# Blaizzy/mlx-audio-swift

Measured on NVIDIA H100. Metric: orpheus3b_tts_rtfx_batch8, higher is better.
Workload: dtype bf16

## Files before the change

### include/b200audio_internal.h

```cpp
#ifndef B200AUDIO_INTERNAL_H
#define B200AUDIO_INTERNAL_H

#include "b200audio.h"

#ifdef __cplusplus
extern "C" {
#endif

int32_t b2a_tts_create_random(int32_t device, const b2a_llama_config* cfg, float std, uint64_t seed,
                              b2a_snac* snac, b2a_tts** out);
int32_t b2a_stt_create_random(int32_t device, const b2a_whisper_config* cfg, float std, uint64_t seed, b2a_stt** out);
int32_t b2a_tts_set_bench_flags(b2a_tts* h, int32_t mask_eos, int32_t wrap_codes);
int32_t b2a_stt_set_bench_flags(b2a_stt* h, int32_t mask_eot);
int32_t b2a_tts_time_steps(b2a_tts* h, int32_t batch, int32_t ctx, int32_t iters, float* ms_per_step);
int32_t b2a_qwen3_talker_create_random(int32_t device, const b2a_qwen3_talker_config* cfg, float std, uint64_t seed, b2a_qwen3_talker** out);
int32_t b2a_qwen3_talker_set_bench_flags(b2a_qwen3_talker* h, int32_t mask_eos);

int32_t b2a_tts_debug_trace(b2a_tts* h, int32_t enable, int32_t batch, float* out);
int32_t b2a_debug_step_smem(int32_t gqa, int32_t* out);

int32_t b2a_speech_tokenizer_debug_layout(const float* w, int32_t out, int32_t k, int32_t in, int32_t stride, float* layout_out,
                                          int64_t capacity, int32_t* rows, int32_t* taps, int32_t* kpad);
int32_t b2a_speech_tokenizer_debug_stage(b2a_speech_tokenizer* h, int32_t stage, float* out, int64_t capacity, int64_t* n);
int32_t b2a_qwen3_sample_test(const float* logits, int32_t batch, int32_t vocab, float temperature, float top_p, int32_t top_k,
                              float min_p, float repetition_penalty, int32_t eos, int32_t suppress_lo, int32_t suppress_hi,
                              uint32_t* seen, int32_t track, uint64_t seed, int32_t step, int32_t* tokens_out, float* filtered_out);
int32_t b2a_implicit_conv_test(const float* w, int32_t M, int32_t taps, int32_t Cin, const float* x, int32_t B, int32_t Ttot, int32_t T,
                               int32_t dil, int32_t shift0, int32_t up, const float* bias, const float* gamma, int32_t gelu, int32_t add,
                               int32_t bias_twice_t0, const float* sa, const float* sb, int32_t Hout, int32_t fp16, float* xo, float* hl_out);
int32_t b2a_tc_gemm_epilogue_test(const void* W, const void* X, void* out, int32_t M, int32_t N, int32_t K, int32_t bn, int32_t epi,
                                  int32_t split, int32_t hilo, int32_t ctas, const float* bias, int32_t act, int32_t tile_rows,
                                  int32_t lo_rows, const float* rstd_ss, int32_t rstd_parts, float rstd_eps, int32_t stages, void* stream);
int32_t b2a_tc_gemm_test(const void* W, const void* X, void* out, int32_t M, int32_t N, int32_t K, int32_t bn, int32_t epi,
                         int32_t split, int32_t hilo, int32_t ctas, void* stream);
int32_t b2a_tc_gemm_splitk_test(const void* W, const void* X, float* h, const float* gain, void* xn, float* ss, int32_t M, int32_t N,
                                int32_t K, int32_t cluster, int32_t stages, void* stream);
int32_t b2a_mha_tc_test(const float* qkv, void* out, int32_t B, int32_t T, int32_t nh, void* stream);
int32_t b2a_conv_gemm_test(const float* w, int32_t M, int32_t K, const void* X, int32_t N, int32_t epi, const float* bias,
                           const float* alpha, const float* gamma, int32_t gelu, float* x, int32_t ldx, void* hl, int32_t ldh,
                           int32_t dual, int32_t T, int32_t Cout, int32_t stride, int32_t pad, int32_t Tin, const float* noise,
                           uint64_t seed, int32_t ctas, void* stream);
int32_t b2a_snac_unit_test(int32_t mode, int32_t C, int32_t dil, const float* x, float* y, int32_t B, int32_t T, const float* dw_w,
                           const float* dw_b, const float* a_in, const float* a_mid, const float* pw_w, const float* pw_bias,
                           const float* noise, uint64_t seed, void* hl, const float* a_next, int32_t ctas, void* stream);
int32_t b2a_snac_convt_test(const float* x, float* y, const float* alpha, const float* bias, const float* w, int32_t B, int32_t Tin,
                            int32_t stride, int32_t cout, int32_t ctas, void* stream);
int32_t b2a_snac_encode_latent_test(b2a_snac* h, const float* wave, int32_t batch, int64_t n_samples, float* z);

#ifdef __cplusplus
}
#endif
#endif
```

### mlx-audio-swift_b200/_ffi.py

```python
from __future__ import annotations

import ctypes as C
from pathlib import Path

import numpy as np

LIB_PATH = Path(__file__).resolve().parent / "lib" / "libb200audio.so"

(OK, ERR_MODEL_NOT_INITIALIZED, ERR_GENERATION_FAILED, ERR_INVALID_INPUT, ERR_AUDIO_DECODING_FAILED,
 ERR_AUDIO_ENCODING_FAILED, ERR_CANCELLED, ERR_CUDA) = range(8)
DTYPE_F32, DTYPE_BF16, DTYPE_I32 = 0, 1, 2


class AudioGenerationError(RuntimeError):
    CASES = {1: "modelNotInitialized", 2: "generationFailed", 3: "invalidInput", 4: "audioDecodingFailed",
             5: "audioEncodingFailed", 6: "cancelled", 7: "cudaError"}

    def __init__(self, code: int, message: str):
        super().__init__(f"{self.CASES.get(code, code)}: {message}")
        self.code, self.case, self.message = code, self.CASES.get(code, str(code)), message


class Tensor(C.Structure):
    _fields_ = [("name", C.c_char_p), ("dtype", C.c_int32), ("ndim", C.c_int32), ("shape", C.c_int64 * 4),
# ... 32 lines not shown
    _fields_ = [(n, C.c_int32) for n in ("input_channels", "dim", "intermediate_dim", "num_layers", "n_fft", "hop_length",
                                          "input_kernel_size", "dw_kernel_size", "adanorm_num_embeddings")]


class EncodecConfig(C.Structure):
    _fields_ = ([(n, C.c_int32) for n in ("audio_channels", "num_filters", "kernel_size", "num_residual_layers",
                                           "dilation_growth_rate", "codebook_size", "codebook_dim", "hidden_size",
                                           "num_lstm_layers", "residual_kernel_size", "use_causal_conv", "pad_mode_reflect",
                                           "norm_type", "last_kernel_size", "compress", "n_upsampling_ratios")]
                + [("upsampling_ratios", C.c_int32 * 8), ("sampling_rate", C.c_int32), ("use_conv_shortcut", C.c_int32),
                   ("trim_right_ratio", C.c_float), ("chunk_length_s", C.c_float), ("overlap", C.c_float)])


class SpeechTokenizerConfig(C.Structure):
    _fields_ = ([(n, C.c_int32) for n in ("codebook_size", "codebook_dim", "latent_dim", "decoder_dim", "hidden_size",
                                           "intermediate_size", "head_dim", "num_attention_heads", "num_key_value_heads",
                                           "num_hidden_layers", "num_quantizers", "num_semantic_quantizers")]
                + [("rms_norm_eps", C.c_float), ("rope_theta", C.c_float), ("attention_bias", C.c_int32),
                   ("num_upsample_rates", C.c_int32), ("upsample_rates", C.c_int32 * 8),
                   ("num_upsampling_ratios", C.c_int32), ("upsampling_ratios", C.c_int32 * 8),
                   ("max_batch", C.c_int32), ("max_cache_frames", C.c_int32)])


class Qwen3TalkerConfig(C.Structure):
    _fields_ = ([(n, C.c_int32) for n in ("vocab_size", "hidden_size", "intermediate_size", "num_hidden_layers", "num_attention_heads",
                                           "num_key_value_heads", "head_dim")]
                + [("rms_norm_eps", C.c_float), ("rope_theta", C.c_float)]
                + [(n, C.c_int32) for n in ("num_code_groups", "text_hidden_size", "text_vocab_size", "codec_eos_token_id", "cp_vocab_size",
                                             "cp_hidden_size", "cp_intermediate_size", "cp_num_hidden_layers", "cp_num_attention_heads",
                                             "cp_num_key_value_heads", "cp_head_dim")]
                + [("cp_rms_norm_eps", C.c_float), ("cp_rope_theta", C.c_float), ("max_batch", C.c_int32), ("max_context", C.c_int32)])


class Qwen3GenParams(C.Structure):
    _fields_ = [("max_tokens", C.c_int32), ("temperature", C.c_float), ("top_p", C.c_float), ("top_k", C.c_int32), ("min_p", C.c_float),
                ("repetition_penalty", C.c_float), ("seed", C.c_uint64)]


class WhisperConfig(C.Structure):
    _fields_ = [(n, C.c_int32) for n in ("vocab_size", "num_mel_bins", "d_model", "encoder_layers", "encoder_attention_heads",
                                          "encoder_ffn_dim", "max_source_positions", "decoder_layers", "decoder_attention_heads",
                                          "decoder_ffn_dim", "max_target_positions", "max_batch")]


class SttParams(C.Structure):
    _fields_ = [("max_tokens", C.c_int32), ("temperature", C.c_float), ("prompt_ids", C.c_void_p), ("n_prompt", C.c_int32),
                ("begin_suppress", C.c_void_p), ("n_begin_suppress", C.c_int32), ("suppress", C.c_void_p),
                ("n_suppress", C.c_int32), ("timestamp_begin", C.c_int32), ("eot", C.c_int32), ("seed", C.c_uint64)]


class SttInfo(C.Structure):
    _fields_ = [("prompt_tokens", C.c_int32), ("generation_tokens", C.c_int32), ("decode_steps", C.c_int32),
                ("encode_time", C.c_double), ("decode_time", C.c_double), ("total_time", C.c_double)]


TOKEN_CB = C.CFUNCTYPE(None, C.c_void_p, C.c_int32, C.c_int32, C.c_int32)
AUDIO_CB = C.CFUNCTYPE(None, C.c_void_p, C.c_int32, C.POINTER(C.c_float), C.c_int64, C.c_int32)
STT_DECODE_CB = C.CFUNCTYPE(C.c_int32, C.c_void_p, C.POINTER(C.c_float), C.c_int64, C.POINTER(C.c_int32), C.c_int32, C.POINTER(C.c_int32),
                            C.c_int32, C.POINTER(C.c_int32))


class SttStreamConfig(C.Structure):
    _fields_ = [("decode_interval_s", C.c_double), ("window_s", C.c_double), ("window_overlap_s", C.c_double), ("delay_ms", C.c_int32),
                ("min_agreement_passes", C.c_int32), ("max_tokens_per_pass", C.c_int32), ("sample_rate", C.c_int32)]


class SttStreamUpdate(C.Structure):
    _fields_ = [("kind", C.c_int32), ("promoted", C.c_int32), ("completed_windows", C.c_int32), ("n_confirmed", C.c_int32),
                ("n_provisional", C.c_int32), ("total_audio_s", C.c_double), ("pass_encode_time", C.c_double), ("pass_decode_time", C.c_double)]


_P = C.c_void_p
SIGNATURES = {
    "b2a_last_error": (C.c_char_p, []),
    "b2a_version": (C.c_char_p, []),
    "b2a_device_count": (C.c_int32, []),
    "b2a_launch_count": (C.c_int64, []),
    "b2a_hanning_window": (C.c_int32, [C.c_int32, C.c_int32, _P]),
    "b2a_hamming_window": (C.c_int32, [C.c_int32, C.c_int32, _P]),
    "b2a_power_to_db": (C.c_int32, [_P, C.c_int64, C.c_float, C.c_float, _P]),
    "b2a_mel_filters": (C.c_int32, [C.c_int32, C.c_int32, C.c_int32, C.c_float, C.c_float, C.c_int32, C.c_int32, _P]),
    "b2a_mel_create": (C.c_int32, [C.c_int32, C.c_int32, C.c_int32, C.c_int32, C.c_int32, C.POINTER(_P)]),
    "b2a_mel_max_frames": (C.c_int64, [_P, C.c_int64]),
    "b2a_mel_process": (C.c_int32, [_P, _P, C.c_int64, _P, C.c_int64, C.POINTER(C.c_int64)]),
    "b2a_mel_flush": (C.c_int32, [_P, _P, C.c_int64, C.POINTER(C.c_int64)]),
    "b2a_mel_reset": (C.c_int32, [_P]),
    "b2a_mel_total_frames": (C.c_int64, [_P]),
    "b2a_mel_destroy": (None, [_P]),
    "b2a_logmel_create": (C.c_int32, [C.c_int32, C.c_int32, C.c_int32, C.c_int32, C.c_int32, C.c_int32, C.POINTER(_P)]),
    "b2a_logmel_frames": (C.c_int64, [_P, C.c_int64]),
    "b2a_logmel_compute": (C.c_int32, [_P, _P, C.c_int32, C.c_int64, _P]),
    "b2a_logmel_compute_dev": (C.c_int32, [_P, _P, C.c_int32, C.c_int64, _P, _P]),
    "b2a_logmel_destroy": (None, [_P]),
    "b2a_snac_create": (C.c_int32, [C.c_int32, C.POINTER(SnacConfig), C.POINTER(Tensor), C.c_int32, C.POINTER(_P)]),
    "b2a_snac_hop_length": (C.c_int64, [_P]),
    "b2a_snac_decode": (C.c_int32, [_P, C.POINTER(_P), C.c_int32, C.c_int64, C.POINTER(_P), C.c_int32, C.c_uint64, _P]),
    "b2a_snac_decode_dev": (C.c_int32, [_P, C.POINTER(_P), C.c_int32, C.c_int64, C.POINTER(_P), C.c_int32, C.c_uint64, _P, _P]),
    "b2a_snac_quantize": (C.c_int32, [_P, _P, C.c_int32, C.c_int64, C.POINTER(_P), _P]),
    "b2a_snac_encoded_length": (C.c_int64, [_P, C.c_int64]),
    "b2a_snac_encode": (C.c_int32, [_P, _P, C.c_int32, C.c_int64, C.POINTER(_P)]),
    "b2a_snac_encode_dev": (C.c_int32, [_P, _P, C.c_int32, C.c_int64, C.POINTER(_P), _P]),
    "b2a_snac_encode_latent_test": (C.c_int32, [_P, _P, C.c_int32, C.c_int64, _P]),
    "b2a_snac_destroy": (None, [_P]),
    "b2a_tts_create": (C.c_int32, [C.c_int32, C.POINTER(LlamaConfig), C.POINTER(Tensor), C.c_int32, _P, C.POINTER(_P)]),
    "b2a_tts_debug_trace": (C.c_int32, [_P, C.c_int32, C.c_int32, _P]),
    "b2a_debug_step_smem": (C.c_int32, [C.c_int32, C.POINTER(C.c_int32)]),
    "b2a_tts_create_random": (C.c_int32, [C.c_int32, C.POINTER(LlamaConfig), C.c_float, C.c_uint64, _P, C.POINTER(_P)]),
    "b2a_tts_stream": (C.c_void_p, [_P]),
    "b2a_tts_set_bench_flags": (C.c_int32, [_P, C.c_int32, C.c_int32]),
    "b2a_stt_set_bench_flags": (C.c_int32, [_P, C.c_int32]),
    "b2a_tts_time_steps": (C.c_int32, [_P, C.c_int32, C.c_int32, C.c_int32, C.POINTER(C.c_float)]),
    "b2a_snac_stream": (C.c_void_p, [_P]),
    "b2a_tts_prepare_input_ids": (C.c_int32, [C.POINTER(_P), _P, C.c_int32, _P, C.POINTER(C.c_int32)]),
    "b2a_tts_prepare_input_ids_ref": (C.c_int32, [C.POINTER(_P), _P, C.c_int32, _P, C.c_int32, _P, C.c_int32, _P, C.POINTER(C.c_int32)]),
    "b2a_tts_forward_logits": (C.c_int32, [_P, _P, C.c_int32, C.c_int32, C.c_int32, _P]),
    "b2a_tts_generate": (C.c_int32, [_P, _P, C.c_int32, C.c_int32, C.POINTER(GenParams), _P, _P, _P, C.c_int64, _P,
                                     C.POINTER(GenInfo), TOKEN_CB, _P]),
    "b2a_tts_generate_stream": (C.c_int32, [_P, _P, C.c_int32, C.c_int32, C.POINTER(GenParams), C.c_int32, C.c_int32, _P, _P,
                                            C.POINTER(GenInfo), TOKEN_CB, AUDIO_CB, _P]),
    "b2a_tts_generate_dev": (C.c_int32, [_P, _P, C.c_int32, C.c_int32, C.POINTER(GenParams), _P, C.c_int64, _P,
                                         C.POINTER(GenInfo)]),
    "b2a_tts_cancel": (C.c_int32, [_P]),
    "b2a_tts_parse_output": (C.c_int32, [_P, C.c_int32, C.c_int32, _P, _P]),
    "b2a_tts_deinterleave": (C.c_int32, [_P, C.c_int32, _P, _P, _P, C.POINTER(C.c_int32)]),
    "b2a_tts_interleave": (C.c_int32, [_P, _P, _P, C.c_int32, _P]),
    "b2a_tts_destroy": (None, [_P]),
    "b2a_vocos_create": (C.c_int32, [C.c_int32, C.POINTER(VocosConfig), C.POINTER(Tensor), C.c_int32, C.POINTER(_P)]),
    "b2a_vocos_output_length": (C.c_int64, [_P, C.c_int32]),
    "b2a_vocos_stream": (C.c_void_p, [_P]),
    "b2a_vocos_decode": (C.c_int32, [_P, _P, C.c_int32, C.c_int32, _P]),
    "b2a_vocos_decode_dev": (C.c_int32, [_P, _P, C.c_int32, C.c_int32, _P, _P]),
    "b2a_vocos_decode_cond": (C.c_int32, [_P, _P, _P, C.c_int32, C.c_int32, _P]),
    "b2a_vocos_destroy": (None, [_P]),
    "b2a_speech_tokenizer_create": (C.c_int32, [C.c_int32, C.POINTER(SpeechTokenizerConfig), C.POINTER(Tensor), C.c_int32, C.POINTER(_P)]),
    "b2a_speech_tokenizer_total_upsample": (C.c_int32, [_P]),
    "b2a_speech_tokenizer_stream": (C.c_void_p, [_P]),
    "b2a_speech_tokenizer_reset": (C.c_int32, [_P]),
    "b2a_speech_tokenizer_streaming_step": (C.c_int32, [_P, _P, C.c_int32, C.c_int32, C.c_int32, _P]),
    "b2a_speech_tokenizer_streaming_step_dev": (C.c_int32, [_P, _P, C.c_int32, C.c_int32, C.c_int32, _P, _P]),
    "b2a_speech_tokenizer_streaming_decode": (C.c_int32, [_P, _P, C.c_int32, C.c_int32, C.c_int32, C.c_int32, _P]),
    "b2a_speech_tokenizer_chunked_decode": (C.c_int32, [_P, _P, C.c_int32, C.c_int32, C.c_int32, C.c_int32, C.c_int32, _P]),
    "b2a_speech_tokenizer_destroy": (None, [_P]),
    "b2a_weights_sanitize_speech_tokenizer": (C.c_int32, [_P]),
    "b2a_speech_tokenizer_config_from_json": (C.c_int32, [C.c_char_p, C.c_int32, C.c_int32, C.POINTER(SpeechTokenizerConfig), C.POINTER(C.c_int32)]),
    "b2a_speech_tokenizer_create_from_directory": (C.c_int32, [C.c_char_p, C.c_int32, C.c_int32, C.c_int32, C.POINTER(_P), C.POINTER(C.c_int32)]),
    "b2a_qwen3_sample_test": (C.c_int32, [_P, C.c_int32, C.c_int32, C.c_float, C.c_float, C.c_int32, C.c_float, C.c_float, C.c_int32, C.c_int32,
                                         C.c_int32, _P, C.c_int32, C.c_uint64, C.c_int32, _P, _P]),
    "b2a_implicit_conv_test": (C.c_int32, [_P, C.c_int32, C.c_int32, C.c_int32, _P, C.c_int32, C.c_int32, C.c_int32, C.c_int32, C.c_int32, C.c_int32,
                                          _P, _P, C.c_int32, C.c_int32, C.c_int32, _P, _P, C.c_int32, C.c_int32, _P, _P]),
    "b2a_tc_gemm_test": (C.c_int32, [_P, _P, _P] + [C.c_int32] * 8 + [_P]),
    "b2a_tc_gemm_epilogue_test": (C.c_int32, [_P, _P, _P] + [C.c_int32] * 8 + [_P, C.c_int32, C.c_int32, C.c_int32, _P, C.c_int32,
                                                                             C.c_float, C.c_int32, _P]),
    "b2a_tc_gemm_splitk_test": (C.c_int32, [_P, _P, _P, _P, _P, _P] + [C.c_int32] * 5 + [_P]),
    "b2a_mha_tc_test": (C.c_int32, [_P, _P, C.c_int32, C.c_int32, C.c_int32, _P]),
    "b2a_conv_gemm_test": (C.c_int32, [_P, C.c_int32, C.c_int32, _P, C.c_int32, C.c_int32, _P, _P, _P, C.c_int32, _P, C.c_int32, _P,
                                       C.c_int32] + [C.c_int32] * 6 + [_P, C.c_uint64, C.c_int32, _P]),
    "b2a_snac_unit_test": (C.c_int32, [C.c_int32] * 3 + [_P, _P, C.c_int32, C.c_int32] + [_P] * 6 + [_P, C.c_uint64, _P, _P, C.c_int32, _P]),
    "b2a_snac_convt_test": (C.c_int32, [_P] * 5 + [C.c_int32] * 5 + [_P]),
    "b2a_speech_tokenizer_debug_stage": (C.c_int32, [_P, C.c_int32, _P, C.c_int64, _P]),
    "b2a_speech_tokenizer_debug_layout": (C.c_int32, [_P, C.c_int32, C.c_int32, C.c_int32, C.c_int32, _P, C.c_int64, _P, _P, _P]),
    "b2a_encodec_create": (C.c_int32, [C.c_int32, C.POINTER(EncodecConfig), C.POINTER(Tensor), C.c_int32, C.POINTER(_P)]),
    "b2a_encodec_output_length": (C.c_int64, [_P, C.c_int32, C.c_int32]),
    "b2a_encodec_num_codebooks": (C.c_int32, [_P]),
    "b2a_encodec_stream": (C.c_void_p, [_P]),
    "b2a_encodec_decode": (C.c_int32, [_P, _P, C.c_int32, C.c_int32, C.c_int32, C.c_int32, _P, _P]),
    "b2a_encodec_decode_dev": (C.c_int32, [_P, _P, C.c_int32, C.c_int32, C.c_int32, C.c_int32, _P, _P, _P]),
    "b2a_encodec_destroy": (None, [_P]),
    "b2a_weights_load": (C.c_int32, [C.c_char_p, C.POINTER(_P)]),
    "b2a_weights_count": (C.c_int32, [_P]),
    "b2a_weights_get": (C.c_int32, [_P, C.c_int32, C.POINTER(Tensor)]),
    "b2a_weights_sanitize_whisper": (C.c_int32, [_P, C.POINTER(C.c_int32)]),
    "b2a_weights_sanitize_llama": (C.c_int32, [_P, C.c_int32, C.c_int32, C.c_int32]),
    "b2a_weights_sanitize_llama_config": (C.c_int32, [_P, C.c_char_p]),
    "b2a_weights_dequantize": (C.c_int32, [_P, C.c_int32, C.c_int32]),
    "b2a_weights_free": (None, [_P]),
    "b2a_tts_config_from_json": (C.c_int32, [C.c_char_p, C.c_int32, C.c_int32, C.POINTER(LlamaConfig), C.POINTER(C.c_int32), C.POINTER(C.c_int32)]),
    "b2a_tts_create_from_directory": (C.c_int32, [C.c_char_p, C.c_int32, C.c_int32, C.c_int32, _P, C.POINTER(_P)]),
    "b2a_stt_create": (C.c_int32, [C.c_int32, C.POINTER(WhisperConfig), C.POINTER(Tensor), C.c_int32, C.POINTER(_P)]),
    "b2a_stt_create_random": (C.c_int32, [C.c_int32, C.POINTER(WhisperConfig), C.c_float, C.c_uint64, C.POINTER(_P)]),
    "b2a_stt_stream": (C.c_void_p, [_P]),
    "b2a_stt_encode": (C.c_int32, [_P, _P, C.c_int32, C.c_int64, _P]),
    "b2a_stt_decoder_logits": (C.c_int32, [_P, _P, C.c_int32, C.c_int32, _P]),
    "b2a_stt_transcribe": (C.c_int32, [_P, _P, C.c_int32, C.c_int64, C.POINTER(SttParams), _P, _P, C.POINTER(SttInfo)]),
    "b2a_stt_transcribe_dev": (C.c_int32, [_P, _P, C.c_int32, C.c_int64, C.POINTER(SttParams), _P, _P, C.POINTER(SttInfo)]),
    "b2a_stt_transcribe_long": (C.c_int32, [_P, _P, C.c_int64, C.POINTER(SttParams), C.c_int32, _P, _P, _P, C.POINTER(C.c_int32), C.POINTER(SttInfo)]),
    "b2a_qwen3_talker_create": (C.c_int32, [C.c_int32, C.POINTER(Qwen3TalkerConfig), C.POINTER(Tensor), C.c_int32, C.POINTER(_P)]),
    "b2a_qwen3_talker_create_random": (C.c_int32, [C.c_int32, C.POINTER(Qwen3TalkerConfig), C.c_float, C.c_uint64, C.POINTER(_P)]),
    "b2a_qwen3_talker_set_bench_flags": (C.c_int32, [_P, C.c_int32]),
    "b2a_qwen3_talker_stream": (C.c_void_p, [_P]),
    "b2a_qwen3_talker_embed_text": (C.c_int32, [_P, _P, C.c_int32, _P]),
    "b2a_qwen3_talker_embed_codec": (C.c_int32, [_P, _P, C.c_int32, _P]),
    "b2a_qwen3_talker_forward": (C.c_int32, [_P, _P, C.c_int32, C.c_int32, _P, _P]),
    "b2a_qwen3_talker_generate": (C.c_int32, [_P, _P, C.c_int32, C.c_int32, _P, _P, C.c_int32, _P, C.POINTER(Qwen3GenParams), _P, _P,
                                              C.POINTER(GenInfo), _P, _P]),
    "b2a_qwen3_talker_config_from_json": (C.c_int32, [C.c_char_p, C.c_int32, C.c_int32, C.POINTER(Qwen3TalkerConfig)]),
    "b2a_weights_sanitize_qwen3_talker": (C.c_int32, [_P, C.c_char_p]),
    "b2a_qwen3_talker_create_from_directory": (C.c_int32, [C.c_char_p, C.c_int32, C.c_int32, C.c_int32, C.POINTER(_P)]),
    "b2a_qwen3_talker_cancel": (C.c_int32, [_P]),
    "b2a_qwen3_talker_destroy": (None, [_P]),
    "b2a_stt_session_create": (C.c_int32, [_P, C.POINTER(SttParams), C.POINTER(SttStreamConfig), C.POINTER(_P)]),
    "b2a_stt_session_create_with_decoder": (C.c_int32, [STT_DECODE_CB, _P, C.POINTER(SttStreamConfig), C.POINTER(_P)]),
    "b2a_stt_session_feed": (C.c_int32, [_P, _P, C.c_int64, C.c_double, C.POINTER(SttStreamUpdate)]),
    "b2a_stt_session_stop": (C.c_int32, [_P, C.c_double, C.POINTER(SttStreamUpdate)]),
    "b2a_stt_session_tokens": (C.c_int32, [_P, C.c_int32, C.c_int32, _P, C.c_int32, C.POINTER(C.c_int32)]),
    "b2a_stt_session_destroy": (None, [_P]),
    "b2a_stt_cancel": (C.c_int32, [_P]),
    "b2a_stt_destroy": (None, [_P]),
}

_lib = None


def lib() -> C.CDLL:
    global _lib
    if _lib is None:
        if not LIB_PATH.exists():
            raise ImportError(f"{LIB_PATH} is missing: build it with `python -c 'import __graft_entry__ as g; g.build()'`"
                              " -- there is no CPU fallback")
        _lib = C.CDLL(str(LIB_PATH))
        for name, (res, args) in SIGNATURES.items():
            fn = getattr(_lib, name)
            fn.restype, fn.argtypes = res, args
    return _lib


def check(status: int) -> None:
    if status != OK:
        raise AudioGenerationError(status, lib().b2a_last_error().decode("utf-8", "replace"))


def ptr(a) -> C.c_void_p:
    if a is None:
        return C.c_void_p(None)
    if isinstance(a, np.ndarray):
        assert a.flags["C_CONTIGUOUS"]
        return C.c_void_p(a.ctypes.data)
    return C.c_void_p(a.data_ptr())


def make_tensor_table(weights: dict):
    import torch
    arr = (Tensor * len(weights))()
    keep = []
    for i, (name, w) in enumerate(weights.items()):
        if isinstance(w, torch.Tensor):
            w = w.detach().contiguous().cpu()
            if w.dtype == torch.bfloat16:
                dt = DTYPE_BF16
            elif w.dtype == torch.float32:
                dt = DTYPE_F32
            else:
                w = w.to(torch.float32); dt = DTYPE_F32
            data, shape = w.data_ptr(), tuple(w.shape)
        else:
            w = np.ascontiguousarray(w)
            if w.dtype == np.int32:
                dt = DTYPE_I32
            else:
                if w.dtype != np.float32:
                    w = w.astype(np.float32)
                dt = DTYPE_F32
            data, shape = w.ctypes.data, w.shape
        assert len(shape) <= 4, name
        nm = name.encode()
        keep += [w, nm]
        arr[i].name, arr[i].dtype, arr[i].ndim, arr[i].data = nm, dt, len(shape), data
        for j, s in enumerate(shape):
            arr[i].shape[j] = s
    return arr, keep
```

### mlx-audio-swift_b200/csrc/llama.cu

```cuda
#include "common.cuh"
#include <cooperative_groups.h>
#include "tc_gemm.cuh"
#include "qwen3_sampler.cuh"

#include <algorithm>
#include <cstdlib>
#include <cstring>
#include <chrono>
#include <cmath>

namespace b2a {

typedef __nv_bfloat16 bf16;

constexpr int TOK_START_OF_HUMAN = 128259, TOK_END_OF_HUMAN = 128260, TOK_END_OF_TEXT = 128009;
constexpr int TOK_START_OF_SPEECH = 128257, TOK_END_OF_SPEECH = 128258, TOK_PAD = 128263;
constexpr int TOK_AUDIO_OFFSET = 128266;
constexpr int TOK_AUDIO_START = 128261, TOK_AUDIO_END = 128262;

__device__ __forceinline__ float bf16_round(float x) { return __bfloat162float(__float2bfloat16_rn(x)); }
__device__ __forceinline__ float bf_lo(unsigned u) { return __uint_as_float(u << 16); }
__device__ __forceinline__ float bf_hi(unsigned u) { return __uint_as_float(u & 0xffff0000u); }

__device__ __forceinline__ uint4 ldg_stream(const uint4* p) {
// ... 14 lines not shown
        x[(long long)b * H + i] = __bfloat162float(embed[(long long)tok * H + i]);
        y[(long long)b * H + i] = 0.f;
    }
}

__global__ void ext_embed_kernel(const float* __restrict__ src, float* __restrict__ x, float* __restrict__ y, int H) {
    const int b = blockIdx.x;
    pdl_trigger();
    pdl_wait();
    for (int i = threadIdx.x; i < H; i += blockDim.x) {
        x[(long long)b * H + i] = src[(long long)b * H + i];
        y[(long long)b * H + i] = 0.f;
    }
}

__global__ void finalize_norm_kernel(const float* __restrict__ x, const float* __restrict__ w, const float* __restrict__ ss, int parts,
                                     float* __restrict__ out, int H, float eps) {
    const int b = blockIdx.x;
    pdl_trigger();
    pdl_wait();
    float t = 0.f;
    for (int p = 0; p < parts; ++p) t += ss[p * 8 + b];
    const float r = rsqrtf(t / (float)H + eps);
    for (int i = threadIdx.x; i < H; i += blockDim.x) out[(long long)b * H + i] = x[(long long)b * H + i] * r * w[i];
}

constexpr int LO_ROW = 8;

constexpr int RN_THREADS = 1024, RN_MAXV = 8;
__global__ void __launch_bounds__(RN_THREADS)
add_rmsnorm_kernel(float* __restrict__ x, float* __restrict__ delta, const float* __restrict__ w,
                   bf16* __restrict__ xn, int H, float eps, float* __restrict__ trace, float* __restrict__ zero_ptr,
                   int zero_n, int half, float* __restrict__ normed = nullptr, float* __restrict__ ss_out = nullptr,
                   int ss_parts = 0) {
    __shared__ float red[RN_THREADS / 32];
    const int b = blockIdx.x, tid = threadIdx.x;
    pdl_trigger();
    pdl_wait();
    float* xr = x + (long long)b * H;
    float v[RN_MAXV];
    float ss = 0.f;
#pragma unroll
    for (int j = 0; j < RN_MAXV; ++j) {
        const int i = tid + j * RN_THREADS;
        float val = 0.f;
        if (i < H) {
            val = xr[i];
            if (delta) { val += delta[(long long)b * H + i]; xr[i] = val; delta[(long long)b * H + i] = 0.f; }
            if (trace) trace[(long long)b * H + i] = val;
        }
        v[j] = val;
        ss += val * val;
    }
    ss = warp_sum(ss);
    if ((tid & 31) == 0) red[tid >> 5] = ss;
    __syncthreads();
    float tot = 0.f;
#pragma unroll
    for (int i = 0; i < RN_THREADS / 32; ++i) tot += red[i];
    const float r = ss_out ? 1.0f : rsqrtf(tot / (float)H + eps);
    if (ss_out && tid < ss_parts) ss_out[tid * 8 + b] = tid == 0 ? tot : 0.f;
#pragma unroll
    for (int j = 0; j < RN_MAXV; ++j) {
        const int i = tid + j * RN_THREADS;
        if (i < H) {
            const float o = v[j] * r * w[i];
            tc::store_hilo(xn, H, b, i, o, half);
            if (normed) normed[(long long)b * H + i] = o;
        }
    }
    if (zero_ptr)
        for (int i = tid; i < zero_n; i += RN_THREADS) zero_ptr[(long long)b * zero_n + i] = 0.f;
}

constexpr int GV_MAX_THREADS = 256;
enum : int { GV_F32 = 0, GV_SWIGLU = 1, GV_F32_ATOMIC = 2 };

template <int NB, int ROWS, int EPI>
__global__ void __launch_bounds__(GV_MAX_THREADS)
gemv_bf16_kernel(const bf16* __restrict__ W, const bf16* __restrict__ xin, float* __restrict__ y,
                 bf16* __restrict__ act, int N, int K) {
    extern __shared__ uint4 sx[];
    pdl_trigger();
    pdl_wait();
    const int K8 = K >> 3;
    const int Kc8 = K8 / gridDim.y, kbase = blockIdx.y * Kc8;
    for (int i = threadIdx.x; i < 2 * NB * Kc8; i += blockDim.x) {
        const int r = i / Kc8, k = i - r * Kc8;
        const int grow = r < NB ? r : LO_ROW + (r - NB);
        sx[i] = reinterpret_cast<const uint4*>(xin)[(long long)grow * K8 + kbase + k];
    }
    __syncthreads();
    const int warp = threadIdx.x >> 5, lane = threadIdx.x & 31;
    const int row0 = (blockIdx.x * (blockDim.x >> 5) + warp) * ROWS;
    if (row0 >= N) return;
    const uint4* Wr[ROWS];
#pragma unroll
    for (int r = 0; r < ROWS; ++r)
        Wr[r] = reinterpret_cast<const uint4*>(W) + (long long)min(row0 + r, N - 1) * K8 + kbase;

    float acc[ROWS][2 * NB];
#pragma unroll
    for (int r = 0; r < ROWS; ++r)
#pragma unroll
        for (int b = 0; b < 2 * NB; ++b) acc[r][b] = 0.f;

    for (int k8 = lane; k8 < Kc8; k8 += 32) {
        float wf[ROWS][8];
#pragma unroll
        for (int r = 0; r < ROWS; ++r) {
            const uint4 wv = ldg_stream(Wr[r] + k8);
            wf[r][0] = bf_lo(wv.x); wf[r][1] = bf_hi(wv.x); wf[r][2] = bf_lo(wv.y); wf[r][3] = bf_hi(wv.y);
            wf[r][4] = bf_lo(wv.z); wf[r][5] = bf_hi(wv.z); wf[r][6] = bf_lo(wv.w); wf[r][7] = bf_hi(wv.w);
        }
#pragma unroll
        for (int b = 0; b < 2 * NB; ++b) {
            const uint4 xv = sx[b * Kc8 + k8];
            const float xf[8] = {bf_lo(xv.x), bf_hi(xv.x), bf_lo(xv.y), bf_hi(xv.y),
                                 bf_lo(xv.z), bf_hi(xv.z), bf_lo(xv.w), bf_hi(xv.w)};
#pragma unroll
            for (int r = 0; r < ROWS; ++r)
#pragma unroll
                for (int j = 0; j < 8; ++j) acc[r][b] = fmaf(wf[r][j], xf[j], acc[r][b]);
        }
    }
#pragma unroll
    for (int r = 0; r < ROWS; ++r)
#pragma unroll
        for (int b = 0; b < NB; ++b) acc[r][b] = warp_sum(acc[r][b] + acc[r][NB + b]);
    if (lane == 0) {
        if (EPI == GV_F32 || EPI == GV_F32_ATOMIC) {
#pragma unroll
            for (int r = 0; r < ROWS; ++r)
                if (row0 + r < N)
#pragma unroll
                    for (int b = 0; b < NB; ++b) {
                        if (EPI == GV_F32) y[(long long)b * N + row0 + r] = acc[r][b];
                        else atomicAdd(&y[(long long)b * N + row0 + r], acc[r][b]);
                    }
        } else {
#pragma unroll
            for (int r = 0; r < ROWS; r += 2)
                if (row0 + r + 1 < N)
#pragma unroll
                    for (int b = 0; b < NB; ++b) {
                        const float g = acc[r][b], u = acc[r + 1][b];
                        tc::store_hilo(act, N / 2, b, (row0 + r) / 2, g / (1.0f + __expf(-g)) * u, LO_ROW);
                    }
        }
    }
}

constexpr int HD = 128, AT_THREADS = 256, MAXG = 8, AT_CAP = 64;
constexpr int AT_SLOTS = 3;
constexpr size_t attn_smem_bytes(int G) {
    return ((size_t)AT_SLOTS * AT_CAP * HD + (size_t)G * HD + 2 * HD + (size_t)G * HD + 2 * MAXG) * sizeof(float) + 64;
}
static_assert((AT_THREADS / 32) * MAXG * HD <= AT_CAP * HD, "the warp-partial outputs must fit in one ring slot");

struct AttnArgs {
    const float* qkv;
    const int* pos;
    const float* freqs;
    float* kcache;
    float* vcache;
    bf16* out;
    int nq, nkv, max_ctx;
    float scale;
    const float* qnorm;
    const float* knorm;
    float qk_eps;
    int zero_qkv;
};

template <int G>
__global__ void __cluster_dims__(1, 1, 2) __launch_bounds__(AT_THREADS)
attn_decode_cluster_kernel(const __grid_constant__ AttnArgs a) {
    namespace cgr = cooperative_groups;
    cgr::cluster_group cluster = cgr::this_cluster();
    const int rank = (int)cluster.block_rank();
    extern __shared__ __align__(16) uint8_t at_smem[];
    float* sKV = reinterpret_cast<float*>(at_smem);
    float* wpo = sKV;
    float* sq = sKV + (size_t)AT_SLOTS * AT_CAP * HD;
    float* snew = sq + G * HD;
    float* xo = snew + 2 * HD;
    float* xml = xo + G * HD;
    uint64_t* bars = reinterpret_cast<uint64_t*>(xml + 2 * MAXG);
    __shared__ float red_m[AT_THREADS / 32][MAXG], red_l[AT_THREADS / 32][MAXG];

    const int h = blockIdx.x, b = blockIdx.y, tid = threadIdx.x;
    pdl_trigger();
    const int p = a.pos[b];
    if (!(p >= 0 && p < a.max_ctx)) { pdl_wait(); return; }
    const int nch = p / AT_CAP + 1;
    const int n_my = nch > rank ? (nch - rank + 1) / 2 : 0;
    const bool owner = ((nch - 1) & 1) == rank;
    const int qkv_ld = (a.nq + 2 * a.nkv) * HD;
    const float* row = a.qkv + (long long)b * qkv_ld;
    float* kc = a.kcache + (((long long)b * a.nkv + h) * a.max_ctx) * HD;
    float* vc = a.vcache + (((long long)b * a.nkv + h) * a.max_ctx) * HD;
    const int n_mat = 2 * n_my;
    auto issue = [&](int j) {
        const int slot = j % AT_SLOTS, c = rank + 2 * (j >> 1);
        const int n_load = (c < nch - 1) ? AT_CAP : p - c * AT_CAP;
        if (n_load > 0) {
            const uint32_t bytes = (uint32_t)n_load * HD * 4;
            tc::mbar_arrive_expect_tx(&bars[slot], bytes);
            asm volatile("cp.async.bulk.shared::cluster.global.mbarrier::complete_tx::bytes [%0], [%1], %2, [%3];"
                         ::"r"(tc::smem_u32(sKV + (size_t)slot * AT_CAP * HD)), "l"(((j & 1) ? vc : kc) + (long long)c * AT_CAP * HD), "r"(bytes),
                           "r"(tc::smem_u32(&bars[slot])) : "memory");
        } else {
            tc::mbar_arrive(&bars[slot]);
        }
    };
    if (tid == 0) {
        for (int i = 0; i < AT_SLOTS; ++i) tc::mbar_init(&bars[i], 1);
        tc::fence_barrier_init();
        asm volatile("fence.proxy.async.shared::cta;" ::: "memory");
        for (int j = 0; j < min(n_mat, AT_SLOTS); ++j) issue(j);
    }
    float sn = 0.f, cs = 1.f;
    if (tid < HD / 2) sincosf((float)p / a.freqs[tid], &sn, &cs);
    pdl_wait();
    const float* qsrc = row + (long long)h * G * HD;
    const float* ksrc = row + (a.nq + h) * HD;
    if (a.qnorm) {
        for (int vec = tid >> 5; vec < G + 1; vec += AT_THREADS / 32) {
            const float* src = vec < G ? qsrc + vec * HD : ksrc;
            const float* w = vec < G ? a.qnorm : a.knorm;
            const float4 x = reinterpret_cast<const float4*>(src)[tid & 31];
            const float ss = warp_sum(x.x * x.x + x.y * x.y + x.z * x.z + x.w * x.w);
            const float r = rsqrtf(ss * (1.0f / HD) + a.qk_eps);
            const float4 g4 = reinterpret_cast<const float4*>(w)[tid & 31];
            reinterpret_cast<float4*>(vec < G ? sq + vec * HD : snew)[tid & 31] =
                make_float4(x.x * r * g4.x, x.y * r * g4.y, x.z * r * g4.z, x.w * r * g4.w);
        }
        __syncthreads();
        qsrc = sq;
        ksrc = snew;
    }
    if (tid < HD / 2) {
        const int d = tid;
        _Pragma("unroll") for (int g = 0; g < G; ++g) {
            const float* q = qsrc + g * HD;
            const float x1 = q[d], x2 = q[d + HD / 2];
            sq[g * HD + d] = x1 * cs - x2 * sn;
            sq[g * HD + d + HD / 2] = x2 * cs + x1 * sn;
        }
        const float* k = ksrc;
        const float x1 = k[d], x2 = k[d + HD / 2];
        const float k1 = x1 * cs - x2 * sn, k2 = x2 * cs + x1 * sn;
        if (owner) { kc[(long long)p * HD + d] = k1; kc[(long long)p * HD + d + HD / 2] = k2; }
        snew[d] = k1;
        snew[d + HD / 2] = k2;
    } else if (tid >= 128) {
        const int d = tid - 128;
        const float v = row[(a.nq + a.nkv + h) * HD + d];
        if (owner) vc[(long long)p * HD + d] = v;
        snew[HD + d] = v;
    }
    __syncthreads();

    const int lane = tid & 31, warp = tid >> 5;
    const int kslot = warp * 8 + (lane >> 2), part = lane & 3;
    float m_run[G], l_run[G];
    float4 o4[G];
    _Pragma("unroll") for (int g = 0; g < G; ++g) { m_run[g] = -INFINITY; l_run[g] = 0.f; o4[g] = make_float4(0.f, 0.f, 0.f, 0.f); }

    for (int i = 0; i < n_my; ++i) {
        const int jk = 2 * i, jv = 2 * i + 1, c = rank + 2 * i;
        float* sK = sKV + (size_t)(jk % AT_SLOTS) * AT_CAP * HD;
        float* sV = sKV + (size_t)(jv % AT_SLOTS) * AT_CAP * HD;
        const int t0 = c * AT_CAP, nk = min(AT_CAP, p + 1 - t0);
        tc::mbar_wait(&bars[jk % AT_SLOTS], (uint32_t)((jk / AT_SLOTS) & 1));
        if (c == nch - 1) {
            if (tid < HD) sK[(p - t0) * HD + tid] = snew[tid];
            __syncthreads();
        }
        float sacc[G];
        _Pragma("unroll") for (int g = 0; g < G; ++g) sacc[g] = 0.f;
        if (kslot < nk) {
            const float4* kr = reinterpret_cast<const float4*>(sK + kslot * HD);
#pragma unroll
            for (int j = 0; j < 8; ++j) {
                const int d4 = part + 4 * ((j + kslot) & 7);
                const float4 kf = kr[d4];
                _Pragma("unroll") for (int g = 0; g < G; ++g) {
                    const float4 qf = reinterpret_cast<const float4*>(sq + g * HD)[d4];
                    sacc[g] = fmaf(qf.x, kf.x, sacc[g]); sacc[g] = fmaf(qf.y, kf.y, sacc[g]);
                    sacc[g] = fmaf(qf.z, kf.z, sacc[g]); sacc[g] = fmaf(qf.w, kf.w, sacc[g]);
                }
            }
        }
        if (jk + AT_SLOTS < n_mat) {
            __syncthreads();
            if (tid == 0) issue(jk + AT_SLOTS);
        }
        float pw[G];
        _Pragma("unroll") for (int g = 0; g < G; ++g) {
            float v = sacc[g];
            v += __shfl_xor_sync(0xffffffffu, v, 1);
            v += __shfl_xor_sync(0xffffffffu, v, 2);
            const float sv = kslot < nk ? v * a.scale : -INFINITY;
            float m = sv;
            m = fmaxf(m, __shfl_xor_sync(0xffffffffu, m, 4));
            m = fmaxf(m, __shfl_xor_sync(0xffffffffu, m, 8));
            m = fmaxf(m, __shfl_xor_sync(0xffffffffu, m, 16));
            const float m_new = fmaxf(m_run[g], m);
            const float rescale = (m_run[g] == -INFINITY) ? 0.f : __expf(m_run[g] - m_new);
            const float e = (sv == -INFINITY) ? 0.f : __expf(sv - m_new);
            float l = part == 0 ? e : 0.f;
            l = warp_sum(l);
            l_run[g] = l_run[g] * rescale + l;
            m_run[g] = m_new;
            o4[g].x *= rescale; o4[g].y *= rescale; o4[g].z *= rescale; o4[g].w *= rescale;
            pw[g] = e;
        }
        tc::mbar_wait(&bars[jv % AT_SLOTS], (uint32_t)((jv / AT_SLOTS) & 1));
        if (c == nch - 1) {
            if (tid >= HD) sV[(p - t0) * HD + tid - HD] = snew[tid];
            __syncthreads();
        }
#pragma unroll
        for (int kk = 0; kk < 8; ++kk) {
            const int t = warp * 8 + kk;
            if (t < nk) {
                const float4 v = reinterpret_cast<const float4*>(sV + t * HD)[lane];
                _Pragma("unroll") for (int g = 0; g < G; ++g) {
                    const float pk = __shfl_sync(0xffffffffu, pw[g], kk * 4);
                    o4[g].x = fmaf(pk, v.x, o4[g].x); o4[g].y = fmaf(pk, v.y, o4[g].y);
                    o4[g].z = fmaf(pk, v.z, o4[g].z); o4[g].w = fmaf(pk, v.w, o4[g].w);
                }
            }
        }
        if (jv + AT_SLOTS < n_mat) {
            __syncthreads();
            if (tid == 0) issue(jv + AT_SLOTS);
        }
    }
    __syncthreads();
    _Pragma("unroll") for (int g = 0; g < G; ++g) {
        reinterpret_cast<float4*>(wpo + (warp * G + g) * HD)[lane] = o4[g];
        if (lane == 0) { red_m[warp][g] = m_run[g]; red_l[warp][g] = l_run[g]; }
    }
    __syncthreads();
    float Ms[G], Ls[G], Os[G];
    if (tid < HD) {
        _Pragma("unroll") for (int g = 0; g < G; ++g) {
            float M = red_m[0][g];
#pragma unroll
            for (int w = 1; w < AT_THREADS / 32; ++w) M = fmaxf(M, red_m[w][g]);
            float L = 0.f, O = 0.f;
#pragma unroll
            for (int w = 0; w < AT_THREADS / 32; ++w) {
                const float sc_w = red_m[w][g] == -INFINITY ? 0.f : __expf(red_m[w][g] - M);
                L = fmaf(red_l[w][g], sc_w, L);
                O = fmaf(wpo[(w * G + g) * HD + tid], sc_w, O);
            }
            Ms[g] = M; Ls[g] = L; Os[g] = O;
        }
        if (rank == 1) {
            float* rxo = cluster.map_shared_rank(xo, 0);
            float* rxml = cluster.map_shared_rank(xml, 0);
            _Pragma("unroll") for (int g = 0; g < G; ++g) {
                rxo[g * HD + tid] = Os[g];
                if (tid == 0) { rxml[g] = Ms[g]; rxml[MAXG + g] = Ls[g]; }
            }
        }
    }
    cluster.sync();
    if (a.zero_qkv && rank == 0) {
        float* wrow = const_cast<float*>(row);
        for (int i = tid; i < G * HD; i += AT_THREADS) wrow[(long long)h * G * HD + i] = 0.f;
        if (tid < HD) { wrow[(a.nq + h) * HD + tid] = 0.f; wrow[(a.nq + a.nkv + h) * HD + tid] = 0.f; }
    }
    if (rank == 0 && tid < HD) {
        _Pragma("unroll") for (int g = 0; g < G; ++g) {
            const float M1 = xml[g], L1 = xml[MAXG + g], O1 = xo[g * HD + tid];
            const float M = fmaxf(Ms[g], M1);
            const float w0 = Ms[g] == -INFINITY ? 0.f : __expf(Ms[g] - M), w1 = M1 == -INFINITY ? 0.f : __expf(M1 - M);
            const float L = Ls[g] * w0 + L1 * w1, O = Os[g] * w0 + O1 * w1;
            tc::store_hilo(a.out, (long long)a.nq * HD, b, (h * G + g) * HD + tid, O / L, LO_ROW);
        }
    }
}

constexpr int PF_HALF = 64;
constexpr int PA_QT = 32, PA_THREADS = 256, PA_MAXL = 128;

__global__ void embed_rows_kernel(const int* __restrict__ ids, const bf16* __restrict__ embed, float* __restrict__ x,
                                  int H, int V) {
    const int t = blockIdx.x;
    int tok = ids[t];
    tok = min(max(tok, 0), V - 1);
    for (int i = threadIdx.x; i < H; i += blockDim.x) x[(long long)t * H + i] = __bfloat162float(embed[(long long)tok * H + i]);
}

__global__ void rope_table_kernel(const float* __restrict__ freqs, float2* __restrict__ tab, int L) {
    const int i = blockIdx.x * blockDim.x + threadIdx.x;
    if (i >= L * (HD / 2)) return;
    const int p = i / (HD / 2), d = i - p * (HD / 2);
    float s, c;
    sincosf((float)p / freqs[d], &s, &c);
    tab[i] = make_float2(c, s);
}

struct PrefillAttnArgs {
    const float* qkv;
    const float2* rope;
    float* kcache;
    float* vcache;
    bf16* out;
    int nq, nkv, max_ctx, L;
    float scale;
};

template <int G>
__global__ void __launch_bounds__(PA_THREADS)
prefill_attn_kernel(PrefillAttnArgs a) {
    extern __shared__ __align__(16) uint8_t pa_smem[];
    const int h = blockIdx.x, b = blockIdx.y, q0 = blockIdx.z * PA_QT;
    const int nqt = min(PA_QT, a.L - q0), kmax = q0 + nqt;
    float* sK = reinterpret_cast<float*>(pa_smem);
    float* sV = sK + (size_t)a.L * HD;
    float* sQ = sV + (size_t)a.L * HD;
    const int tid = threadIdx.x, lane = tid & 31, warp = tid >> 5;
    const int ld = (a.nq + 2 * a.nkv) * HD;
    const float* base = a.qkv + (long long)b * a.L * ld;
    float* kc = a.kcache + (((long long)b * a.nkv + h) * a.max_ctx) * HD;
    float* vc = a.vcache + (((long long)b * a.nkv + h) * a.max_ctx) * HD;

    for (int i = tid; i < kmax * (HD / 2); i += PA_THREADS) {
        const int t = i / (HD / 2), d = i - t * (HD / 2);
        const float2 cs = a.rope[t * (HD / 2) + d];
        const float* k = base + (long long)t * ld + (a.nq + h) * HD;
        const float x1 = k[d], x2 = k[d + HD / 2];
        const float k1 = x1 * cs.x - x2 * cs.y, k2 = x2 * cs.x + x1 * cs.y;
        sK[t * HD + d] = k1; sK[t * HD + d + HD / 2] = k2;
        if (t >= q0) { kc[(long long)t * HD + d] = k1; kc[(long long)t * HD + d + HD / 2] = k2; }
    }
    for (int i = tid; i < kmax * HD; i += PA_THREADS) {
        const int t = i / HD, d = i - t * HD;
        const float v = base[(long long)t * ld + (a.nq + a.nkv + h) * HD + d];
        sV[i] = v;
        if (t >= q0) vc[(long long)t * HD + d] = v;
    }
    for (int i = tid; i < G * nqt * (HD / 2); i += PA_THREADS) {
        const int g = i / (nqt * (HD / 2)), r = i - g * nqt * (HD / 2), qi = r / (HD / 2), d = r - qi * (HD / 2);
        const float2 cs = a.rope[(q0 + qi) * (HD / 2) + d];
        const float* q = base + (long long)(q0 + qi) * ld + (h * G + g) * HD;
        const float x1 = q[d], x2 = q[d + HD / 2];
        sQ[(g * PA_QT + qi) * HD + d] = x1 * cs.x - x2 * cs.y;
        sQ[(g * PA_QT + qi) * HD + d + HD / 2] = x2 * cs.x + x1 * cs.y;
    }
    __syncthreads();

    constexpr int KJ = PA_MAXL / 32;
    for (int r = warp; r < G * nqt; r += PA_THREADS / 32) {
        const int g = r / nqt, qi = r - g * nqt, qpos = q0 + qi;
        const float4* q4 = reinterpret_cast<const float4*>(sQ + (g * PA_QT + qi) * HD);
        float sc[KJ];
        float mx = -INFINITY;
#pragma unroll
        for (int j = 0; j < KJ; ++j) {
            const int t = j * 32 + lane;
            float acc = -INFINITY;
            if (t <= qpos) {
                const float4* k4 = reinterpret_cast<const float4*>(sK + t * HD);
                acc = 0.f;
#pragma unroll 8
                for (int i = 0; i < HD / 4; ++i) {
                    const int d4 = (i + lane) & (HD / 4 - 1);
                    const float4 kf = k4[d4], qf = q4[d4];
                    acc = fmaf(qf.x, kf.x, acc); acc = fmaf(qf.y, kf.y, acc);
                    acc = fmaf(qf.z, kf.z, acc); acc = fmaf(qf.w, kf.w, acc);
                }
                acc *= a.scale;
            }
            sc[j] = acc;
            mx = fmaxf(mx, acc);
        }
        for (int o = 16; o; o >>= 1) mx = fmaxf(mx, __shfl_xor_sync(0xffffffffu, mx, o));
        float sum = 0.f;
#pragma unroll
        for (int j = 0; j < KJ; ++j) { sc[j] = sc[j] == -INFINITY ? 0.f : __expf(sc[j] - mx); sum += sc[j]; }
        sum = warp_sum(sum);
        float4 o = make_float4(0.f, 0.f, 0.f, 0.f);
#pragma unroll
        for (int j = 0; j < KJ; ++j) {
            if (j * 32 > qpos) break;
            for (int l = 0; l < 32; ++l) {
                const int t = j * 32 + l;
                if (t > qpos) break;
                const float p = __shfl_sync(0xffffffffu, sc[j], l);
                const float4 v = reinterpret_cast<const float4*>(sV + t * HD)[lane];
                o.x = fmaf(p, v.x, o.x); o.y = fmaf(p, v.y, o.y); o.z = fmaf(p, v.z, o.z); o.w = fmaf(p, v.w, o.w);
            }
        }
        const float inv = 1.0f / sum;
        const int tok = b * a.L + qpos;
        const long long col = (long long)(h * G + g) * HD + lane * 4;
        const long long ldo = (long long)a.nq * HD;
        tc::store_hilo(a.out, ldo, tok, col + 0, o.x * inv, PF_HALF);
        tc::store_hilo(a.out, ldo, tok, col + 1, o.y * inv, PF_HALF);
        tc::store_hilo(a.out, ldo, tok, col + 2, o.z * inv, PF_HALF);
        tc::store_hilo(a.out, ldo, tok, col + 3, o.w * inv, PF_HALF);
    }
}

__global__ void gather_last_kernel(const float* __restrict__ xp, const float* __restrict__ yp, float* __restrict__ x,
                                   float* __restrict__ y, int* __restrict__ pos, int L, int H) {
    const int b = blockIdx.x;
    const long long src = ((long long)b * L + L - 1) * H;
    for (int i = threadIdx.x; i < H; i += blockDim.x) {
        x[(long long)b * H + i] = xp[src + i];
        y[(long long)b * H + i] = yp[src + i];
    }
    if (threadIdx.x == 0) pos[b] = L - 1;
}

constexpr int SM_THREADS = 1024, SM_WARPS = SM_THREADS / 32, SM_MAX_ATTEMPTS = 12;

struct SampleArgs {
    float* logits;
    float* probs;
    int* tokens;
    int* pos;
    int* recent;
    int* recent_n;
    int* out_tokens;
    int* n_gen;
    int* done;
    int* n_active;
    const int* forced;
    int V, R, max_tokens;
    float temperature, top_p, rep_penalty;
    unsigned long long seed;
// ... 92 lines not shown
                return l * inv_t - __logf(-__logf(u));
            };
            float z = 0.f, gv = -INFINITY;
            int gi = 0x7fffffff;
            for (int i = i0 + t; i < i1; i += SM_THREADS) {
                const float l = lg[i];
                z += __expf((l - mx) * inv_t);
                const float k = l == -INFINITY ? -INFINITY : gumbel_key(i, l, 0);
                if (k > gv) { gv = k; gi = i; }
            }
            exchange(gv, gi, z);
            const float Z = z;
            int cand = gi;
            bool accepted = a.top_p >= 1.0f;
            for (int att = 0; !accepted; ++att) {
                const float lc = lg[cand];
                float gm = 0.f, dv = -INFINITY;
                int di = 0x7fffffff;
                for (int i = i0 + t; i < i1; i += SM_THREADS) { const float l = lg[i]; if (l > lc) gm += __expf((l - mx) * inv_t); }
                exchange(dv, di, gm);
                if (gm < a.top_p * Z) { accepted = true; break; }
                if (att + 1 >= SM_MAX_ATTEMPTS) { cand = tok_final; break; }
                gv = -INFINITY; gi = 0x7fffffff;
                float ds = 0.f;
                for (int i = i0 + t; i < i1; i += SM_THREADS) {
                    const float l = lg[i];
                    const float k = l == -INFINITY ? -INFINITY : gumbel_key(i, l, att + 1);
                    if (k > gv) { gv = k; gi = i; }
                }
                exchange(gv, gi, ds);
                cand = gi;
            }
            if (cand >= 0 && cand < a.V) tok_final = cand;
        }
    } else {
        tok_final = a.forced[b];
    }

    if (rank == 0 && t == 0) {
        const int tok = tok_final;
        a.tokens[b] = tok;
        a.pos[b] += 1;
        const int rn = a.recent_n[b];
        if (a.R > 0) {
            if (rn < a.R) a.recent[b * a.R + rn] = tok;
            else {
                for (int j = 1; j < a.R; ++j) a.recent[b * a.R + j - 1] = a.recent[b * a.R + j];
                a.recent[b * a.R + a.R - 1] = tok;
            }
            a.recent_n[b] = rn + 1;
        }
        if (a.forced == nullptr && !a.done[b]) {
            if (tok == TOK_END_OF_SPEECH) {
                a.done[b] = 1;
                atomicSub(a.n_active, 1);
            } else {
                const int n = a.n_gen[b];
                if (n < a.max_tokens) a.out_tokens[b * a.max_tokens + n] = tok;
                a.n_gen[b] = n + 1;
                if (n + 1 >= a.max_tokens) { a.done[b] = 1; atomicSub(a.n_active, 1); }
            }
        }
    }
}

__global__ void prefill_advance_kernel(const int* __restrict__ ids, int L, int* tokens, int* pos, int B) {
    const int b = threadIdx.x;
    pdl_wait();
    if (b >= B) return;
    const int p = pos[b] + 1;
    pos[b] = p;
    if (p < L) tokens[b] = ids[b * L + p];
}

__global__ void init_rows_kernel(const int* __restrict__ ids, int L, int B, int R, int* tokens, int* pos, int* recent,
                                 int* recent_n, int* n_gen, int* done, int* n_active, int start_pos) {
    const int b = threadIdx.x;
    if (b == 0) *n_active = B;
    if (b >= B) return;
    tokens[b] = ids[b * L];
    pos[b] = start_pos;
    n_gen[b] = 0;
    done[b] = 0;
    const int n = min(R, L);
    for (int j = 0; j < n; ++j) recent[b * R + j] = ids[b * L + L - n + j];
    recent_n[b] = n;
}

__global__ void random_bf16_kernel(bf16* __restrict__ w, long long n, float std, unsigned long long seed) {
    for (long long i = (long long)blockIdx.x * blockDim.x + threadIdx.x; i < n; i += (long long)gridDim.x * blockDim.x) {
        unsigned long long z = seed + 0x9E3779B97F4A7C15ull * (unsigned long long)(i + 1);
        z = (z ^ (z >> 30)) * 0xBF58476D1CE4E5B9ull;
        z = (z ^ (z >> 27)) * 0x94D049BB133111EBull;
        z ^= z >> 31;
        const float u1 = ((unsigned)(z >> 40) + 1.0f) * (1.0f / 16777217.0f);
        const float u2 = (unsigned)((z >> 8) & 0xFFFFFF) * (1.0f / 16777216.0f);
        w[i] = __float2bfloat16_rn(std * sqrtf(-2.0f * __logf(u1)) * cospif(2.0f * u2));
    }
}
__global__ void fill_f32_kernel(float* p, int n, float v) {
    const int i = blockIdx.x * blockDim.x + threadIdx.x;
    if (i < n) p[i] = v;
}

static std::vector<float> llama3_freqs(const b2a_llama_config& c) {
    const int d = c.head_dim;
    std::vector<float> f(d / 2);
    const float low_wl = c.rope_old_context_len / c.rope_low_freq_factor;
    const float high_wl = c.rope_old_context_len / c.rope_high_freq_factor;
    for (int i = 0; i < d / 2; ++i) {
        float fr = powf(c.rope_theta, (float)(2 * i) / (float)d);
        const float wl = 2.0f * (float)M_PI * fr;
        const float base = fr;
        if (wl > low_wl) fr = fr * c.rope_factor;
        const bool med = wl > high_wl && wl < low_wl;
        if (med) {
            const float smooth = (c.rope_old_context_len / wl - c.rope_low_freq_factor) /
                                 (c.rope_high_freq_factor - c.rope_low_freq_factor);
            fr = base / ((1.0f - smooth) / c.rope_factor + smooth);
        }
        f[i] = fr;
    }
    return f;
}

struct LayerW {
    DBuf<bf16> wqkv, wo, wgu, wdown;
    DBuf<float> ln1, ln2;
    DBuf<float> qnorm, knorm;
};

struct StackSpec {
    std::string prefix = "model.";
    bool qk_norm = false;
    bool has_embed = true;
    std::string head;
    bool has_head = true;
};

}

using namespace b2a;

struct b2a_tts {
    int device;
    b2a_llama_config cfg;
    b2a_snac* snac;
    cudaStream_t stream = nullptr;
    std::vector<LayerW> layers;
    DBuf<bf16> embed, lm_head_w;
    const bf16* lm_head = nullptr;
    DBuf<float> final_ln, freqs;
    DBuf<float> kcache, vcache;
    DBuf<float> x, y, qkv, logits, probs;
    DBuf<bf16> xn, attn, act;
    DBuf<float> sk_ws;
    DBuf<unsigned> sk_cnt;
    int sk_slots = 0;
    bool use_tc = true;
    int num_sms = 132;
    std::vector<CUtensorMap> tm_qkv, tm_o, tm_gu, tm_down;
    static int pick_tile_rows(int M, int sms) {
        if (cdiv(M, tc::BM) * 4 >= sms * 3) return tc::BM;
        return std::max(8, std::min(tc::BM, cdiv(cdiv(M, sms), 8) * 8));
    }
    int lm_tile_rows = 128, head_rows_now = 0;
    std::vector<CUtensorMap> tm_gu_dec;
    int gu_tile_rows = 0;
    CUtensorMap tm_lm{}, tmx_xn{}, tmx_attn{}, tmx_act{};
    DBuf<float> xp, yp, qkvp;
    DBuf<bf16> xnp, attnp, actp;
    DBuf<float2> rope_tab;
    CUtensorMap tmp_xn{}, tmp_attn{}, tmp_act{};
    int pf_tokens_cap = 0;
    bool use_batched_prefill = true;
    DBuf<int> tokens, pos, recent, recent_n, out_tokens, n_gen, done, n_active, ids, forced;
    HBuf<int> h_flag;
    cudaEvent_t ev_poll[2] = {nullptr, nullptr};
    bool fused = false;
    static constexpr int fused_cluster = 5;
    static constexpr int gemm_stages = 6, splitk_stages = 5;
    int fused_parts = 0;
    DBuf<float> ss_a, ss_b;
    StackSpec spec;
    const float* x_ext = nullptr;
    float* normed_out = nullptr;
    std::atomic<int> cancel{0};
    int bench_mask_eos = 0, bench_wrap_codes = 0;
    int nb_pad = 0;
    bool trace_on = false;
    DBuf<float> trace;
    cudaGraphExec_t g_step = nullptr, g_prefill = nullptr;
    SampleArgs g_args{};
    int g_nb = 0;
    DBuf<int> d_codes[3];
    DBuf<float> d_wave;

    ~b2a_tts() {
        if (g_step) cudaGraphExecDestroy(g_step);
        if (g_prefill) cudaGraphExecDestroy(g_prefill);
        for (auto& e : ev_poll) if (e) cudaEventDestroy(e);
        if (stream) cudaStreamDestroy(stream);
    }

    static void upload_bf16(const TensorTable& tt, const std::string& name, int64_t expect, DBuf<bf16>& dst, size_t offset_elems,
                            size_t total_elems) {
        const b2a_tensor& t = tt.get(name);
        B2A_CHECK(t.dtype == B2A_DTYPE_BF16 || t.dtype == B2A_DTYPE_F32, B2A_ERR_MODEL_NOT_INITIALIZED, "tensor must be bf16 or f32: " + name);
        B2A_CHECK(TensorTable::numel(t) == expect, B2A_ERR_MODEL_NOT_INITIALIZED, "bad shape for tensor: " + name);
        dst.alloc(total_elems);
        if (t.dtype == B2A_DTYPE_BF16) {
            B2A_CUDA(cudaMemcpy(dst.p + offset_elems, t.data, expect * sizeof(bf16), cudaMemcpyHostToDevice));
        } else {
            std::vector<bf16> tmp((size_t)expect);
            const float* src = (const float*)t.data;
            for (int64_t i = 0; i < expect; ++i) tmp[i] = __float2bfloat16_rn(src[i]);
            B2A_CUDA(cudaMemcpy(dst.p + offset_elems, tmp.data(), expect * sizeof(bf16), cudaMemcpyHostToDevice));
        }
    }

    template <int G>
    static void attn_cluster_attr() {
        B2A_CUDA(cudaFuncSetAttribute(attn_decode_cluster_kernel<G>, cudaFuncAttributeMaxDynamicSharedMemorySize, (int)attn_smem_bytes(G)));
        B2A_CUDA(cudaFuncSetAttribute(attn_decode_cluster_kernel<G>, cudaFuncAttributePreferredSharedMemoryCarveout, cudaSharedmemCarveoutMaxShared));
    }
    void attn_launch(const AttnArgs& aa, int B, cudaStream_t s) {
        const int G = aa.nq / aa.nkv;
        const size_t sm = attn_smem_bytes(G);
        const dim3 g3(aa.nkv, B, 2);
        switch (G) {
            case 1: launch_pdl(attn_decode_cluster_kernel<1>, g3, dim3(AT_THREADS), sm, s, aa); break;
            case 2: launch_pdl(attn_decode_cluster_kernel<2>, g3, dim3(AT_THREADS), sm, s, aa); break;
            case 3: launch_pdl(attn_decode_cluster_kernel<3>, g3, dim3(AT_THREADS), sm, s, aa); break;
            case 4: launch_pdl(attn_decode_cluster_kernel<4>, g3, dim3(AT_THREADS), sm, s, aa); break;
            case 6: launch_pdl(attn_decode_cluster_kernel<6>, g3, dim3(AT_THREADS), sm, s, aa); break;
            default: launch_pdl(attn_decode_cluster_kernel<8>, g3, dim3(AT_THREADS), sm, s, aa); break;
        }
    }

    void check_config() {
        const b2a_llama_config& c = cfg;
        B2A_CHECK(c.head_dim == HD, B2A_ERR_INVALID_INPUT, "llama: head_dim must be 128");
        B2A_CHECK(c.hidden_size % 8 == 0 && c.intermediate_size % 8 == 0, B2A_ERR_INVALID_INPUT, "llama: sizes must be multiples of 8");
        {
            const int g = c.num_key_value_heads > 0 && c.num_attention_heads % c.num_key_value_heads == 0
                              ? c.num_attention_heads / c.num_key_value_heads : 0;
            B2A_CHECK(g == 1 || g == 2 || g == 3 || g == 4 || g == 6 || g == 8, B2A_ERR_INVALID_INPUT,
                      "llama: unsupported GQA ratio (q heads per kv head must be 1, 2, 3, 4, 6 or 8)");
        }
        B2A_CHECK(c.max_batch >= 1 && c.max_batch <= 8, B2A_ERR_INVALID_INPUT, "llama: max_batch must be in 1..8");
        B2A_CHECK(c.max_context >= 8, B2A_ERR_INVALID_INPUT, "llama: max_context too small");
        require_device(device);
        B2A_CUDA(cudaStreamCreateWithFlags(&stream, cudaStreamNonBlocking));
    }

    void alloc_state() {
        const b2a_llama_config& c = cfg;
        const int H = c.hidden_size, I = c.intermediate_size, nq = c.num_attention_heads, nkv = c.num_key_value_heads;
        const int NQ = nq * HD, NKV = nkv * HD;
        B2A_CHECK(H <= RN_THREADS * RN_MAXV, B2A_ERR_INVALID_INPUT, "llama: hidden_size above 8192 is not supported");
        std::vector<float> fr = llama3_freqs(c);
        freqs.upload(fr.data(), fr.size());
        const size_t kv = (size_t)c.num_hidden_layers * c.max_batch * nkv * c.max_context * HD;
        kcache.alloc(kv);
        vcache.alloc(kv);
        B2A_CUDA(cudaMemset(kcache.p, 0, kv * sizeof(float)));
        B2A_CUDA(cudaMemset(vcache.p, 0, kv * sizeof(float)));
        const int B = 8, R16 = 16;
        x.alloc((size_t)B * H); y.alloc((size_t)B * H); qkv.alloc((size_t)B * (NQ + 2 * NKV));
        logits.alloc((size_t)B * c.vocab_size); probs.alloc((size_t)B * c.vocab_size);
        xn.alloc((size_t)R16 * H); attn.alloc((size_t)R16 * NQ); act.alloc((size_t)R16 * I);
        B2A_CUDA(cudaMemset(xn.p, 0, (size_t)R16 * H * sizeof(bf16)));
        B2A_CUDA(cudaMemset(attn.p, 0, (size_t)R16 * NQ * sizeof(bf16)));
        B2A_CUDA(cudaMemset(act.p, 0, (size_t)R16 * I * sizeof(bf16)));
        B2A_CUDA(cudaMemset(x.p, 0, (size_t)B * H * sizeof(float)));
        B2A_CUDA(cudaMemset(y.p, 0, (size_t)B * H * sizeof(float)));
        B2A_CUDA(cudaMemset(qkv.p, 0, (size_t)B * (NQ + 2 * NKV) * sizeof(float)));
        tokens.alloc(B); pos.alloc(B); recent.alloc(B * 64); recent_n.alloc(B); n_gen.alloc(B); done.alloc(B);
        n_active.alloc(1); forced.alloc(B);
        B2A_CUDA(cudaMemset(tokens.p, 0, B * sizeof(int)));
        B2A_CUDA(cudaMemset(pos.p, 0, B * sizeof(int)));
        h_flag.alloc(16);
        gemv_attrs<1>(); gemv_attrs<2>(); gemv_attrs<4>(); gemv_attrs<8>();
        attn_cluster_attr<1>(); attn_cluster_attr<2>(); attn_cluster_attr<3>(); attn_cluster_attr<4>(); attn_cluster_attr<6>(); attn_cluster_attr<8>();
        const char* env = getenv("B2A_GEMM");
        use_tc = !(env && std::string(env) == "simt") && H % tc::BK == 0 && NQ % tc::BK == 0 && I % tc::BK == 0;
        fused_parts = H / tc::BM;
        fused = use_tc && H % tc::BM == 0 && fused_parts <= 64;
        ss_a.alloc((size_t)64 * 8); ss_b.alloc((size_t)64 * 8);
        B2A_CUDA(cudaMemset(ss_a.p, 0, 64 * 8 * sizeof(float)));
        B2A_CUDA(cudaMemset(ss_b.p, 0, 64 * 8 * sizeof(float)));
        B2A_CUDA(cudaDeviceGetAttribute(&num_sms, cudaDevAttrMultiProcessorCount, device));
        {
            const int ops[3][2] = {{NQ + 2 * NKV, H}, {H, NQ}, {H, I}};
            int mt_max = 0;
            for (const auto& op : ops) {
                const int mt = cdiv(op[0], tc::BM), kb = op[1] / tc::BK;
                if (kb == 0) continue;
                const int ctas = (int)std::min<long long>(num_sms, (long long)mt * kb);
                sk_slots = std::max(sk_slots, tc::stream_k_slots(mt, kb, ctas));
                mt_max = std::max(mt_max, mt);
            }
            sk_ws.alloc((size_t)std::max(1, mt_max) * std::max(1, sk_slots) * 16 * tc::BM);
            sk_cnt.alloc((size_t)std::max(1, mt_max));
            B2A_CUDA(cudaMemset(sk_cnt.p, 0, (size_t)std::max(1, mt_max) * sizeof(unsigned)));
        }
        const char* envp = getenv("B2A_PREFILL");
        use_batched_prefill = !(envp && std::string(envp) == "step");
        if (use_tc) {
            tc::set_attributes();
            for (auto& L : layers) {
                tm_qkv.push_back(tc::make_tmap_bf16(L.wqkv.p, NQ + 2 * NKV, H, tc::BM));
                tm_o.push_back(tc::make_tmap_bf16(L.wo.p, H, NQ, tc::BM));
                tm_gu.push_back(tc::make_tmap_bf16(L.wgu.p, 2 * I, H, tc::BM));
                {
                    gu_tile_rows = pick_tile_rows(2 * I, num_sms);
                    tm_gu_dec.push_back(tc::make_tmap_bf16(L.wgu.p, 2 * I, H, gu_tile_rows));
                }
                tm_down.push_back(tc::make_tmap_bf16(L.wdown.p, H, I, tc::BM));
            }
            lm_tile_rows = pick_tile_rows(c.vocab_size, num_sms);
            if (lm_head) tm_lm = tc::make_tmap_bf16(lm_head, c.vocab_size, H, lm_tile_rows);
            tmx_xn = tc::make_tmap_bf16(xn.p, R16, H, 16);
            tmx_attn = tc::make_tmap_bf16(attn.p, R16, NQ, 16);
            tmx_act = tc::make_tmap_bf16(act.p, R16, I, 16);
        }
        B2A_CUDA(cudaDeviceSynchronize());
    }

    b2a_tts(int dev, const b2a_llama_config& c, const TensorTable& tt, b2a_snac* sn, const StackSpec& sp = StackSpec())
        : device(dev), cfg(c), snac(sn), spec(sp) {
        check_config();
        const int H = c.hidden_size, I = c.intermediate_size, nq = c.num_attention_heads, nkv = c.num_key_value_heads;
        const int NQ = nq * HD, NKV = nkv * HD;
        if (sp.has_embed) upload_bf16(tt, sp.prefix + "embed_tokens.weight", (int64_t)c.vocab_size * H, embed, 0, (size_t)c.vocab_size * H);
        if (sp.has_head) {
            if (sp.head.empty() && c.tie_word_embeddings) {
                B2A_CHECK(sp.has_embed, B2A_ERR_MODEL_NOT_INITIALIZED, "a tied head needs the embedding");
                lm_head = embed.p;
            } else {
                upload_bf16(tt, sp.head.empty() ? std::string("lm_head.weight") : sp.head, (int64_t)c.vocab_size * H, lm_head_w, 0, (size_t)c.vocab_size * H);
                lm_head = lm_head_w.p;
            }
        }
        layers.resize(c.num_hidden_layers);
        std::vector<bf16> tmp;
        for (int l = 0; l < c.num_hidden_layers; ++l) {
            const std::string p = sp.prefix + "layers." + std::to_string(l) + ".";
            if (sp.qk_norm) {
                std::vector<float> qn = tt.f32(p + "self_attn.q_norm.weight", HD), kn = tt.f32(p + "self_attn.k_norm.weight", HD);
                layers[l].qnorm.upload(qn.data(), HD);
                layers[l].knorm.upload(kn.data(), HD);
            }
            LayerW& L = layers[l];
            const size_t qkv_n = (size_t)(NQ + 2 * NKV) * H;
            upload_bf16(tt, p + "self_attn.q_proj.weight", (int64_t)NQ * H, L.wqkv, 0, qkv_n);
            upload_bf16(tt, p + "self_attn.k_proj.weight", (int64_t)NKV * H, L.wqkv, (size_t)NQ * H, qkv_n);
            upload_bf16(tt, p + "self_attn.v_proj.weight", (int64_t)NKV * H, L.wqkv, (size_t)(NQ + NKV) * H, qkv_n);
            upload_bf16(tt, p + "self_attn.o_proj.weight", (int64_t)H * NQ, L.wo, 0, (size_t)H * NQ);
            upload_bf16(tt, p + "mlp.down_proj.weight", (int64_t)H * I, L.wdown, 0, (size_t)H * I);
            const b2a_tensor& tg = tt.get(p + "mlp.gate_proj.weight");
            const b2a_tensor& tu = tt.get(p + "mlp.up_proj.weight");
            B2A_CHECK(tg.dtype == tu.dtype && (tg.dtype == B2A_DTYPE_BF16 || tg.dtype == B2A_DTYPE_F32) &&
                          TensorTable::numel(tg) == (int64_t)I * H && TensorTable::numel(tu) == (int64_t)I * H,
                      B2A_ERR_MODEL_NOT_INITIALIZED, "bad gate/up projection: " + p);
            tmp.resize((size_t)2 * I * H);
            for (int n = 0; n < I; ++n) {
                if (tg.dtype == B2A_DTYPE_BF16) {
                    memcpy(&tmp[(size_t)(2 * n) * H], (const bf16*)tg.data + (size_t)n * H, H * sizeof(bf16));
                    memcpy(&tmp[(size_t)(2 * n + 1) * H], (const bf16*)tu.data + (size_t)n * H, H * sizeof(bf16));
                } else {
                    for (int k = 0; k < H; ++k) {
                        tmp[(size_t)(2 * n) * H + k] = __float2bfloat16_rn(((const float*)tg.data)[(size_t)n * H + k]);
                        tmp[(size_t)(2 * n + 1) * H + k] = __float2bfloat16_rn(((const float*)tu.data)[(size_t)n * H + k]);
                    }
                }
            }
            L.wgu.alloc(tmp.size());
            B2A_CUDA(cudaMemcpy(L.wgu.p, tmp.data(), tmp.size() * sizeof(bf16), cudaMemcpyHostToDevice));
            std::vector<float> g1 = tt.f32(p + "input_layernorm.weight", H), g2 = tt.f32(p + "post_attention_layernorm.weight", H);
            L.ln1.upload(g1.data(), H);
            L.ln2.upload(g2.data(), H);
        }
        std::vector<float> gf = tt.f32(sp.prefix + "norm.weight", H);
        final_ln.upload(gf.data(), H);
        alloc_state();
    }

    b2a_tts(int dev, const b2a_llama_config& c, float std, unsigned long long seed, b2a_snac* sn, const StackSpec& sp = StackSpec())
        : device(dev), cfg(c), snac(sn), spec(sp) {
        check_config();
        const int H = c.hidden_size, I = c.intermediate_size, nq = c.num_attention_heads, nkv = c.num_key_value_heads;
        const int NQ = nq * HD, NKV = nkv * HD;
        unsigned long long sd = seed * 1000003ull + 17;
        auto rnd = [&](DBuf<bf16>& d, size_t n) {
            d.alloc(n);
            random_bf16_kernel<<<132 * 8, 256, 0, stream>>>(d.p, (long long)n, std, sd++);
            count_launch();
        };
        auto ones = [&](DBuf<float>& d, int n) {
            d.alloc(n);
            fill_f32_kernel<<<cdiv(n, 256), 256, 0, stream>>>(d.p, n, 1.0f);
            count_launch();
        };
        if (sp.has_embed) rnd(embed, (size_t)c.vocab_size * H);
        if (sp.has_head) {
            if (sp.head.empty() && c.tie_word_embeddings && sp.has_embed) lm_head = embed.p;
            else { rnd(lm_head_w, (size_t)c.vocab_size * H); lm_head = lm_head_w.p; }
        }
        layers.resize(c.num_hidden_layers);
        for (auto& L : layers) {
            if (sp.qk_norm) { ones(L.qnorm, HD); ones(L.knorm, HD); }
            rnd(L.wqkv, (size_t)(NQ + 2 * NKV) * H);
            rnd(L.wo, (size_t)H * NQ);
            rnd(L.wgu, (size_t)2 * I * H);
            rnd(L.wdown, (size_t)H * I);
            ones(L.ln1, H);
            ones(L.ln2, H);
        }
        ones(final_ln, H);
        B2A_CUDA(cudaStreamSynchronize(stream));
        B2A_CUDA(cudaGetLastError());
        alloc_state();
    }

    template <int NB, int ROWS, int EPI>
    void gemv_launch(const bf16* W, const bf16* xin, float* yout, bf16* actout, int N, int K, int warps, int ksplit,
                     cudaStream_t s) {
        const size_t sm = (size_t)2 * NB * (K / ksplit) * sizeof(bf16);
        dim3 grid(cdiv(N, warps * ROWS), ksplit);
        launch_pdl(gemv_bf16_kernel<NB, ROWS, EPI>, grid, dim3(warps * 32), sm, s, W, xin, yout, actout, N, K);
    }
    template <int NB, int ROWS, int EPI>
    static void gemv_attr() {
        B2A_CUDA(cudaFuncSetAttribute(gemv_bf16_kernel<NB, ROWS, EPI>, cudaFuncAttributeMaxDynamicSharedMemorySize, 200 * 1024));
    }
    template <int NB>
    static void gemv_attrs() {
        gemv_attr<NB, 2, GV_F32>(); gemv_attr<NB, 2, GV_SWIGLU>(); gemv_attr<NB, 2, GV_F32_ATOMIC>();
    }
    enum { OP_QKV, OP_O, OP_GU, OP_DOWN, OP_LM };
    template <int NB>
    void gemv_op(int op, const bf16* W, const bf16* xin, float* yout, bf16* actout, int N, int K, cudaStream_t s) {
        const bool split = (K / 8) % 2 == 0 && (size_t)2 * NB * K * sizeof(bf16) > 96 * 1024;
        switch (op) {
            case OP_GU: gemv_launch<NB, 2, GV_SWIGLU>(W, xin, yout, actout, N, K, 8, 1, s); break;
            case OP_DOWN:
            case OP_O:
                if (split) gemv_launch<NB, 2, GV_F32_ATOMIC>(W, xin, yout, actout, N, K, 4, 2, s);
                else gemv_launch<NB, 2, GV_F32>(W, xin, yout, actout, N, K, 4, 1, s);
                break;
            default: gemv_launch<NB, 2, GV_F32>(W, xin, yout, actout, N, K, 8, 1, s); break;
        }
    }
    void gemv_nb(int op, const bf16* W, const bf16* xin, float* yout, bf16* actout, int N, int K, cudaStream_t s) {
        B2A_CHECK((size_t)2 * nb_pad * K * sizeof(bf16) <= 200 * 1024 * ((op == OP_DOWN || op == OP_O) ? 2 : 1),
                  B2A_ERR_INVALID_INPUT, "llama: layer too wide for the shared-memory activation tile");
        switch (nb_pad) {
            case 1: gemv_op<1>(op, W, xin, yout, actout, N, K, s); break;
            case 2: gemv_op<2>(op, W, xin, yout, actout, N, K, s); break;
            case 4: gemv_op<4>(op, W, xin, yout, actout, N, K, s); break;
            default: gemv_op<8>(op, W, xin, yout, actout, N, K, s); break;
        }
    }

    void tc_gemm(const CUtensorMap& tmW, const CUtensorMap& tmX, int op, float* yout, bf16* actout, int B, int M, int K,
                 cudaStream_t s, const float* rstd_ss = nullptr) {
        tc::Args a{};
        a.rstd_ss = rstd_ss; a.rstd_parts = fused_parts; a.rstd_inv_h = 1.0f / (float)cfg.hidden_size; a.rstd_eps = cfg.rms_norm_eps;
        a.out_f32 = yout; a.out_bf16 = actout; a.M = M; a.N = B; a.K = K;
        a.m_tiles = cdiv(M, tc::BM); a.k_blocks = K / tc::BK;
        a.stages = gemm_stages;
        a.hilo = 1;
        int ctas = num_sms;
        if (op == OP_GU) {
            a.ldo = M / 2; a.epi_full = tc::EPI_SWIGLU; a.epi_partial = -1; a.lo_rows = LO_ROW;
            a.tile_rows = gu_tile_rows; a.m_tiles = cdiv(M, gu_tile_rows);
            ctas = std::min(num_sms, a.m_tiles);
        } else if (op == OP_LM) {
            a.ldo = M; a.epi_full = tc::EPI_STORE; a.epi_partial = -1; a.lo_rows = 0;
            a.tile_rows = head_rows_now > 0 ? head_rows_now : lm_tile_rows; a.m_tiles = cdiv(M, a.tile_rows);
            ctas = std::min(num_sms, a.m_tiles);
        } else {
            a.ldo = M; a.epi_full = tc::EPI_STORE; a.epi_partial = tc::EPI_PARTIAL; a.lo_rows = 0;
            ctas = (int)std::min<long long>(num_sms, (long long)a.m_tiles * a.k_blocks);
            a.part_ws = sk_ws.p; a.part_cnt = sk_cnt.p; a.part_slots = sk_slots;
        }
        tc::launch<16>(tmW, tmX, a, ctas, 1, s);
    }

    void gemm(int op, int layer, int B, cudaStream_t s) {
        const int H = cfg.hidden_size, I = cfg.intermediate_size, NQ = cfg.num_attention_heads * HD,
                  NKV = cfg.num_key_value_heads * HD;
        LayerW* L = layer >= 0 ? &layers[layer] : nullptr;
        switch (op) {
            case OP_QKV:
                if (use_tc) tc_gemm(tm_qkv[layer], tmx_xn, op, qkv.p, nullptr, B, NQ + 2 * NKV, H, s);
                else gemv_nb(op, L->wqkv.p, xn.p, qkv.p, nullptr, NQ + 2 * NKV, H, s);
                break;
            case OP_O:
                if (use_tc) tc_gemm(tm_o[layer], tmx_attn, op, y.p, nullptr, B, H, NQ, s);
                else gemv_nb(op, L->wo.p, attn.p, y.p, nullptr, H, NQ, s);
                break;
            case OP_GU:
                if (use_tc) tc_gemm(tm_gu_dec[layer], tmx_xn, op, nullptr, act.p, B, 2 * I, H, s);
                else gemv_nb(op, L->wgu.p, xn.p, nullptr, act.p, 2 * I, H, s);
                break;
            case OP_DOWN:
                if (use_tc) tc_gemm(tm_down[layer], tmx_act, op, y.p, nullptr, B, H, I, s);
                else gemv_nb(op, L->wdown.p, act.p, y.p, nullptr, H, I, s);
                break;
            default:
                if (use_tc) tc_gemm(tm_lm, tmx_xn, op, logits.p, nullptr, B, cfg.vocab_size, H, s);
                else gemv_nb(op, lm_head, xn.p, logits.p, nullptr, cfg.vocab_size, H, s);
                break;
        }
    }

    void splitk_gemm(const CUtensorMap& tmW, const CUtensorMap& tmX, int M, int K, const float* gain, float* ss, int B, cudaStream_t s) {
        tc::SplitArgs a{};
        a.M = M; a.N = B; a.K = K; a.k_blocks = K / tc::BK; a.stages = splitk_stages;
        a.h = x.p; a.gain = gain; a.xn = xn.p; a.ss = ss;
        a.rstd_ss = nullptr; a.rstd_parts = 0; a.rstd_inv_h = 0.f; a.rstd_eps = 0.f;
        tc::launch_splitk(tmW, tmX, a, cdiv(M, tc::BM), std::max(1, std::min(fused_cluster, a.k_blocks)), s);
    }
    void run_layers_fused(int B, cudaStream_t s) {
        const int H = cfg.hidden_size, I = cfg.intermediate_size, nq = cfg.num_attention_heads, nkv = cfg.num_key_value_heads;
        const int NQ = nq * HD, NKV = nkv * HD, L = cfg.num_hidden_layers;
        if (x_ext) launch_pdl(ext_embed_kernel, dim3(B), dim3(256), 0, s, x_ext, x.p, y.p, H);
        else launch_pdl(embed_kernel, dim3(B), dim3(256), 0, s, tokens.p, embed.p, x.p, y.p, H, cfg.vocab_size);
        launch_pdl(add_rmsnorm_kernel, dim3(B), dim3(RN_THREADS), 0, s, x.p, (float*)nullptr, layers[0].ln1.p, xn.p, H, cfg.rms_norm_eps,
                   (float*)nullptr, (float*)nullptr, 0, LO_ROW, (float*)nullptr, ss_b.p, fused_parts);
        const size_t kv_layer = (size_t)cfg.max_batch * nkv * cfg.max_context * HD;
        for (int l = 0; l < L; ++l) {
            LayerW& Lw = layers[l];
            tc_gemm(tm_qkv[l], tmx_xn, OP_QKV, qkv.p, nullptr, B, NQ + 2 * NKV, H, s, ss_b.p);
            AttnArgs aa{qkv.p, pos.p, freqs.p, kcache.p + l * kv_layer, vcache.p + l * kv_layer, attn.p, nq, nkv, cfg.max_context,
                        1.0f / sqrtf((float)HD), spec.qk_norm ? Lw.qnorm.p : nullptr, spec.qk_norm ? Lw.knorm.p : nullptr, cfg.rms_norm_eps, 1};
            attn_launch(aa, B, s);
            splitk_gemm(tm_o[l], tmx_attn, H, NQ, Lw.ln2.p, ss_a.p, B, s);
            tc_gemm(tm_gu_dec[l], tmx_xn, OP_GU, nullptr, act.p, B, 2 * I, H, s, ss_a.p);
            splitk_gemm(tm_down[l], tmx_act, H, I, l + 1 < L ? layers[l + 1].ln1.p : final_ln.p, ss_b.p, B, s);
        }
    }
    int launches_layers_fused() const { return 2 + cfg.num_hidden_layers * 5; }

    void run_layers(int B, cudaStream_t s) {
        if (fused && !trace_on) { run_layers_fused(B, s); return; }
        const int H = cfg.hidden_size, nq = cfg.num_attention_heads, nkv = cfg.num_key_value_heads;
        const int QKV_N = (nq + 2 * nkv) * HD, G = nq / nkv;
        if (x_ext) launch_pdl(ext_embed_kernel, dim3(B), dim3(256), 0, s, x_ext, x.p, y.p, H);
        else launch_pdl(embed_kernel, dim3(B), dim3(256), 0, s, tokens.p, embed.p, x.p, y.p, H, cfg.vocab_size);
        const size_t kv_layer = (size_t)cfg.max_batch * nkv * cfg.max_context * HD;
        for (int l = 0; l < cfg.num_hidden_layers; ++l) {
            LayerW& L = layers[l];
            launch_pdl(add_rmsnorm_kernel, dim3(B), dim3(RN_THREADS), 0, s, x.p, l == 0 ? (float*)nullptr : y.p, L.ln1.p, xn.p, H,
                       cfg.rms_norm_eps, trace_on ? trace.p + (size_t)(2 * l) * 8 * H : (float*)nullptr, (float*)nullptr, 0, LO_ROW,
                       (float*)nullptr, (float*)nullptr, 0);
            gemm(OP_QKV, l, B, s);
            AttnArgs aa{qkv.p, pos.p, freqs.p, kcache.p + l * kv_layer, vcache.p + l * kv_layer, attn.p, nq, nkv, cfg.max_context,
                        1.0f / sqrtf((float)HD), spec.qk_norm ? L.qnorm.p : nullptr, spec.qk_norm ? L.knorm.p : nullptr, cfg.rms_norm_eps, 0};
            attn_launch(aa, B, s);
            gemm(OP_O, l, B, s);
            launch_pdl(add_rmsnorm_kernel, dim3(B), dim3(RN_THREADS), 0, s, x.p, y.p, L.ln2.p, xn.p, H, cfg.rms_norm_eps,
                       trace_on ? trace.p + (size_t)(2 * l + 1) * 8 * H : (float*)nullptr, qkv.p, QKV_N, LO_ROW, (float*)nullptr, (float*)nullptr, 0);
            gemm(OP_GU, l, B, s);
            gemm(OP_DOWN, l, B, s);
        }
        (void)G;
    }

    void run_final_norm(int B, cudaStream_t s) {
        if (fused && !trace_on) {
            if (normed_out)
                launch_pdl(finalize_norm_kernel, dim3(B), dim3(256), 0, s, (const float*)x.p, (const float*)final_ln.p, (const float*)ss_b.p, fused_parts,
                           normed_out, cfg.hidden_size, cfg.rms_norm_eps);
            return;
        }
        launch_pdl(add_rmsnorm_kernel, dim3(B), dim3(RN_THREADS), 0, s, x.p, y.p, final_ln.p, xn.p, cfg.hidden_size, cfg.rms_norm_eps,
                   trace_on ? trace.p + (size_t)(2 * cfg.num_hidden_layers) * 8 * cfg.hidden_size : (float*)nullptr, (float*)nullptr, 0, LO_ROW,
                   normed_out, (float*)nullptr, 0);
    }
    void run_lm_head(int B, cudaStream_t s) {
        run_final_norm(B, s);
        if (fused && !trace_on) tc_gemm(tm_lm, tmx_xn, OP_LM, logits.p, nullptr, B, cfg.vocab_size, cfg.hidden_size, s, ss_b.p);
        else gemm(OP_LM, -1, B, s);
    }
    void run_lm_head_after_prefill(int B, cudaStream_t s) {
        launch_pdl(add_rmsnorm_kernel, dim3(B), dim3(RN_THREADS), 0, s, x.p, y.p, final_ln.p, xn.p, cfg.hidden_size, cfg.rms_norm_eps,
                   (float*)nullptr, (float*)nullptr, 0, LO_ROW, (float*)nullptr, (float*)nullptr, 0);
        gemm(OP_LM, -1, B, s);
    }
    void run_head(const CUtensorMap& tmW, const bf16* W, int M, float* logits_out, int B, cudaStream_t s, int tile_rows = 0) {
        head_rows_now = tile_rows;
        if (use_tc) tc_gemm(tmW, tmx_xn, OP_LM, logits_out, nullptr, B, M, cfg.hidden_size, s, (fused && !trace_on) ? ss_b.p : nullptr);
        else gemv_nb(OP_LM, W, xn.p, logits_out, nullptr, M, cfg.hidden_size, s);
        head_rows_now = 0;
    }

    template <int G>
    static void pattn_attr() {
        B2A_CUDA(cudaFuncSetAttribute(prefill_attn_kernel<G>, cudaFuncAttributeMaxDynamicSharedMemorySize, 220 * 1024));
    }
    size_t pattn_smem(int L) const {
        const int G = cfg.num_attention_heads / cfg.num_key_value_heads;
        return ((size_t)2 * L * HD + (size_t)G * PA_QT * HD) * sizeof(float);
    }
    bool can_batch_prefill(int L) const {
        return use_tc && use_batched_prefill && spec.has_embed && !spec.qk_norm && L >= 2 && L <= PA_MAXL && pattn_smem(L) <= 220 * 1024;
    }

    void pf_gemm(const CUtensorMap& tmW, const CUtensorMap& tmX, int epi, float* yout, bf16* actout, int T, int M, int K,
                 cudaStream_t s) {
        tc::Args a{};
        a.out_f32 = yout; a.out_bf16 = actout; a.M = M; a.N = T; a.K = K;
        a.m_tiles = cdiv(M, tc::BM); a.k_blocks = K / tc::BK;
        a.stages = tc::Smem<128>::max_stages(); a.hilo = 1; a.epi_full = epi; a.epi_partial = -1;
        a.ldo = epi == tc::EPI_SWIGLU ? M / 2 : M;
        a.lo_rows = epi == tc::EPI_SWIGLU ? PF_HALF : 0;
        const int n_tiles = cdiv(T, PF_HALF);
        const int ctas = std::max(1, std::min(a.m_tiles, num_sms / n_tiles));
        tc::launch<128>(tmW, tmX, a, ctas, n_tiles, s);
    }

    void prefill_batched(int B, int L, cudaStream_t s) {
        const int H = cfg.hidden_size, I = cfg.intermediate_size, nq = cfg.num_attention_heads, nkv = cfg.num_key_value_heads;
        const int NQ = nq * HD, QKV_N = (nq + 2 * nkv) * HD, T = B * L, G = nq / nkv;
        const int n_tiles = cdiv(T, PF_HALF), Tp = n_tiles * PF_HALF;
        if (Tp > pf_tokens_cap) {
            xp.alloc((size_t)Tp * H); yp.alloc((size_t)Tp * H); qkvp.alloc((size_t)Tp * QKV_N);
            xnp.alloc((size_t)2 * Tp * H); attnp.alloc((size_t)2 * Tp * NQ); actp.alloc((size_t)2 * Tp * I);
            pf_tokens_cap = Tp;
            tmp_xn = tc::make_tmap_bf16(xnp.p, 2 * Tp, H, 128);
            tmp_attn = tc::make_tmap_bf16(attnp.p, 2 * Tp, NQ, 128);
            tmp_act = tc::make_tmap_bf16(actp.p, 2 * Tp, I, 128);
            pattn_attr<1>(); pattn_attr<2>(); pattn_attr<3>(); pattn_attr<4>(); pattn_attr<6>(); pattn_attr<8>();
        }
        rope_tab.alloc((size_t)PA_MAXL * (HD / 2));
        B2A_CUDA(cudaMemsetAsync(xnp.p, 0, (size_t)2 * pf_tokens_cap * H * sizeof(bf16), s));
        B2A_CUDA(cudaMemsetAsync(attnp.p, 0, (size_t)2 * pf_tokens_cap * NQ * sizeof(bf16), s));
        B2A_CUDA(cudaMemsetAsync(actp.p, 0, (size_t)2 * pf_tokens_cap * I * sizeof(bf16), s));
        embed_rows_kernel<<<T, 256, 0, s>>>(ids.p, embed.p, xp.p, H, cfg.vocab_size);
        rope_table_kernel<<<cdiv(L * (HD / 2), 256), 256, 0, s>>>(freqs.p, rope_tab.p, L);
        count_launch(2);
        const size_t kv_layer = (size_t)cfg.max_batch * nkv * cfg.max_context * HD;
        for (int l = 0; l < cfg.num_hidden_layers; ++l) {
            LayerW& Lw = layers[l];
            launch_pdl(add_rmsnorm_kernel, dim3(T), dim3(RN_THREADS), 0, s, xp.p, l == 0 ? (float*)nullptr : yp.p, Lw.ln1.p, xnp.p, H,
                       cfg.rms_norm_eps, (float*)nullptr, (float*)nullptr, 0, PF_HALF, (float*)nullptr, (float*)nullptr, 0);
            pf_gemm(tm_qkv[l], tmp_xn, tc::EPI_STORE, qkvp.p, nullptr, T, QKV_N, H, s);
            PrefillAttnArgs pa{qkvp.p, rope_tab.p, kcache.p + l * kv_layer, vcache.p + l * kv_layer, attnp.p, nq, nkv,
                               cfg.max_context, L, 1.0f / sqrtf((float)HD)};
            const dim3 grid(nkv, B, cdiv(L, PA_QT));
            const size_t sm = pattn_smem(L);
            switch (G) {
                case 1: prefill_attn_kernel<1><<<grid, PA_THREADS, sm, s>>>(pa); break;
                case 2: prefill_attn_kernel<2><<<grid, PA_THREADS, sm, s>>>(pa); break;
                case 3: prefill_attn_kernel<3><<<grid, PA_THREADS, sm, s>>>(pa); break;
                case 4: prefill_attn_kernel<4><<<grid, PA_THREADS, sm, s>>>(pa); break;
                case 6: prefill_attn_kernel<6><<<grid, PA_THREADS, sm, s>>>(pa); break;
                default: prefill_attn_kernel<8><<<grid, PA_THREADS, sm, s>>>(pa); break;
            }
            count_launch();
            pf_gemm(tm_o[l], tmp_attn, tc::EPI_STORE, yp.p, nullptr, T, H, NQ, s);
            launch_pdl(add_rmsnorm_kernel, dim3(T), dim3(RN_THREADS), 0, s, xp.p, yp.p, Lw.ln2.p, xnp.p, H, cfg.rms_norm_eps,
                       (float*)nullptr, (float*)nullptr, 0, PF_HALF, (float*)nullptr, (float*)nullptr, 0);
            pf_gemm(tm_gu[l], tmp_xn, tc::EPI_SWIGLU, nullptr, actp.p, T, 2 * I, H, s);
            pf_gemm(tm_down[l], tmp_act, tc::EPI_STORE, yp.p, nullptr, T, H, I, s);
        }
        gather_last_kernel<<<B, 256, 0, s>>>(xp.p, yp.p, x.p, y.p, pos.p, L, H);
        count_launch();
        B2A_CUDA(cudaGetLastError());
    }

    void set_batch(int B) {
        nb_pad = B <= 1 ? 1 : B <= 2 ? 2 : B <= 4 ? 4 : 8;
    }

    void drop_graphs() {
        if (g_step) { cudaGraphExecDestroy(g_step); g_step = nullptr; }
        if (g_prefill) { cudaGraphExecDestroy(g_prefill); g_prefill = nullptr; }
    }

    static bool same_args(const SampleArgs& a, const SampleArgs& b) {
        return a.V == b.V && a.R == b.R && a.max_tokens == b.max_tokens && a.temperature == b.temperature &&
               a.top_p == b.top_p && a.rep_penalty == b.rep_penalty && a.seed == b.seed && a.mask_eos == b.mask_eos &&
               a.out_tokens == b.out_tokens;
    }

    void capture(int B, const SampleArgs& sa, int L) {
        if (g_step && g_nb == B && same_args(sa, g_args) && g_L == L) return;
        drop_graphs();
        cudaGraph_t g;
        B2A_CUDA(cudaStreamBeginCapture(stream, cudaStreamCaptureModeThreadLocal));
        run_layers(B, stream);
        run_lm_head(B, stream);
        launch_pdl(sample_kernel, dim3(B * SM_CLUSTER), dim3(SM_THREADS), 0, stream, sa);
        B2A_CUDA(cudaStreamEndCapture(stream, &g));
        B2A_CUDA(cudaGraphInstantiate(&g_step, g, 0));
        cudaGraphDestroy(g);
        B2A_CUDA(cudaStreamBeginCapture(stream, cudaStreamCaptureModeThreadLocal));
        run_layers(B, stream);
        launch_pdl(prefill_advance_kernel, dim3(1), dim3(32), 0, stream, ids.p, L, tokens.p, pos.p, B);
        B2A_CUDA(cudaStreamEndCapture(stream, &g));
        B2A_CUDA(cudaGraphInstantiate(&g_prefill, g, 0));
        cudaGraphDestroy(g);
        g_nb = B; g_args = sa; g_L = L;
        launches_step = fused ? launches_layers_fused() + 1 + 1 : 1 + cfg.num_hidden_layers * 7 + 2 + 1;
        launches_prefill = fused ? launches_layers_fused() + 1 : 1 + cfg.num_hidden_layers * 7 + 1;
    }
    int g_L = 0, launches_step = 0, launches_prefill = 0;
};

static std::vector<int> parse_row(const int* row, int n, int crop_after) {
    std::vector<int> r;
    for (int j = crop_after + 1; j < n; ++j)
        if (row[j] != TOK_END_OF_SPEECH) r.push_back(row[j]);
    r.resize((r.size() / 7) * 7);
    for (auto& t : r) t -= TOK_AUDIO_OFFSET;
    return r;
}

static void deinterleave(const int* cl, int n, std::vector<int>& l1, std::vector<int>& l2, std::vector<int>& l3) {
    const int groups = (n + 1) / 7;
    for (int i = 0; i < groups; ++i) {
        const int b = 7 * i;
        l1.push_back(cl[b]);
        l2.push_back(cl[b + 1] - 4096);
        l3.push_back(cl[b + 2] - 2 * 4096);
        l3.push_back(cl[b + 3] - 3 * 4096);
        l2.push_back(cl[b + 4] - 4 * 4096);
        l3.push_back(cl[b + 5] - 5 * 4096);
        l3.push_back(cl[b + 6] - 6 * 4096);
    }
}

static double now_s() {
    return std::chrono::duration<double>(std::chrono::steady_clock::now().time_since_epoch()).count();
}

struct StreamSpec {
    int frames_per_chunk = 0;
    int left_context = 0;
    b2a_audio_cb on_audio = nullptr;
};

static void tts_generate_impl(b2a_tts* h, const int32_t* input_ids, bool ids_on_device, int32_t B, int32_t L,
                              const b2a_gen_params* gp, int32_t* tokens_out, int32_t* n_tokens_out, float* wave_out,
                              bool wave_on_device, int64_t wave_cap, int64_t* wave_len, b2a_gen_info* info,
                              b2a_token_cb on_token, void* user, const StreamSpec& ss = StreamSpec()) {
    B2A_CHECK(h && input_ids && gp, B2A_ERR_INVALID_INPUT, "tts generate: null argument");
    B2A_CHECK(B >= 1 && B <= h->cfg.max_batch, B2A_ERR_INVALID_INPUT, "tts generate: batch exceeds max_batch");
    B2A_CHECK(L >= 1, B2A_ERR_INVALID_INPUT, "tts generate: empty prompt");
    B2A_CHECK(gp->max_tokens >= 1, B2A_ERR_INVALID_INPUT, "tts generate: max_tokens must be positive");
    B2A_CHECK(L + gp->max_tokens <= h->cfg.max_context, B2A_ERR_INVALID_INPUT, "tts generate: prompt + max_tokens exceeds max_context");
    B2A_CHECK(gp->repetition_context_size >= 0 && gp->repetition_context_size <= 64, B2A_ERR_INVALID_INPUT,
              "tts generate: repetition_context_size must be in 0..64");
    B2A_CHECK(gp->temperature >= 0.f && gp->top_p > 0.f, B2A_ERR_INVALID_INPUT, "tts generate: bad sampling parameters");
    if (wave_out) B2A_CHECK(h->snac, B2A_ERR_MODEL_NOT_INITIALIZED, "SNAC model not loaded");
    B2A_CUDA(cudaSetDevice(h->device));
    cudaStream_t s = h->stream;
    h->cancel.store(0);
    h->set_batch(B);
    if (h->trace_on) { h->trace_on = false; h->drop_graphs(); }
    const int MT = gp->max_tokens, R = std::max(1, gp->repetition_context_size);
    h->ids.alloc((size_t)B * L);
    h->out_tokens.alloc((size_t)B * MT);
    h->recent.alloc((size_t)8 * R);
    B2A_CUDA(cudaMemcpyAsync(h->ids.p, input_ids, (size_t)B * L * sizeof(int),
                             ids_on_device ? cudaMemcpyDeviceToDevice : cudaMemcpyHostToDevice, s));
    SampleArgs sa{};
    sa.logits = h->logits.p; sa.probs = h->probs.p; sa.tokens = h->tokens.p; sa.pos = h->pos.p; sa.recent = h->recent.p;
    sa.recent_n = h->recent_n.p; sa.out_tokens = h->out_tokens.p; sa.n_gen = h->n_gen.p; sa.done = h->done.p;
    sa.n_active = h->n_active.p; sa.forced = nullptr; sa.V = h->cfg.vocab_size; sa.R = gp->repetition_context_size > 0 ? R : 0;
    sa.max_tokens = MT; sa.temperature = gp->temperature; sa.top_p = gp->top_p;
    sa.rep_penalty = gp->repetition_context_size > 0 ? gp->repetition_penalty : 1.0f;
    sa.seed = gp->seed; sa.mask_eos = h->bench_mask_eos;
    if (sa.R == 0) { sa.R = 1; }
    h->capture(B, sa, L);

    const double t0 = now_s();
    init_rows_kernel<<<1, 32, 0, s>>>(h->ids.p, L, B, gp->repetition_context_size > 0 ? R : 0, h->tokens.p, h->pos.p, h->recent.p,
                                      h->recent_n.p, h->n_gen.p, h->done.p, h->n_active.p, 0);
    count_launch();
    int steps = 0;
    if (h->can_batch_prefill(L)) {
        h->prefill_batched(B, L, s);
        h->run_lm_head_after_prefill(B, s);
        launch_pdl(sample_kernel, dim3(B * SM_CLUSTER), dim3(SM_THREADS), 0, s, sa);
        steps = 1;
    } else {
        for (int p = 0; p < L - 1; ++p) {
            B2A_CUDA(cudaGraphLaunch(h->g_prefill, s));
            count_launch(h->launches_prefill);
        }
    }
    B2A_CUDA(cudaStreamSynchronize(s));
    const double t1 = now_s();
    bool cancelled = false;
    int streamed = 0;
    std::vector<int> h_tok;
    const bool streaming = ss.frames_per_chunk > 0 && ss.on_audio;
    if (streaming) B2A_CHECK(h->snac && !ids_on_device, B2A_ERR_MODEL_NOT_INITIALIZED, "SNAC model not loaded");
    std::vector<int> emitted(B, 0), s_prompt, s_tok, s_ng(B);
    std::vector<float> s_wave;
    double codec_stream_t = 0;
    if (streaming) { s_prompt.assign(input_ids, input_ids + (size_t)B * L); s_tok.resize((size_t)B * MT); }
    auto emit_audio = [&](bool final_call) {
        const double c0 = now_s();
        B2A_CUDA(cudaMemcpy(s_ng.data(), h->n_gen.p, B * sizeof(int), cudaMemcpyDeviceToHost));
        B2A_CUDA(cudaMemcpy(s_tok.data(), h->out_tokens.p, (size_t)B * MT * sizeof(int), cudaMemcpyDeviceToHost));
        const int64_t hop = b2a_snac_hop_length(h->snac);
        for (int b = 0; b < B; ++b) {
            const int ng = std::min(s_ng[b], MT);
            std::vector<int> all(s_prompt.begin() + (size_t)b * L, s_prompt.begin() + (size_t)(b + 1) * L);
            all.insert(all.end(), s_tok.begin() + (size_t)b * MT, s_tok.begin() + (size_t)b * MT + ng);
            int last = -1;
            for (int j = 0; j < (int)all.size(); ++j) if (all[j] == TOK_START_OF_SPEECH) last = j;
            std::vector<int> cl = parse_row(all.data(), (int)all.size(), last);
            if (h->bench_wrap_codes)
                for (size_t i = 0; i < cl.size(); ++i) cl[i] = ((cl[i] % 4096) + 4096) % 4096 + 4096 * (int)(i % 7);
            const int total = (int)cl.size() / 7;
            while (total - emitted[b] >= ss.frames_per_chunk || (final_call && total > emitted[b])) {
                const int f1 = final_call ? total : emitted[b] + ss.frames_per_chunk;
                const int f0 = std::max(0, emitted[b] - ss.left_context);
                std::vector<int> l1, l2, l3;
                deinterleave(cl.data() + (size_t)f0 * 7, (f1 - f0) * 7, l1, l2, l3);
                const int F = f1 - f0;
                h->d_codes[0].upload(l1.data(), l1.size(), s);
                h->d_codes[1].upload(l2.data(), l2.size(), s);
                h->d_codes[2].upload(l3.data(), l3.size(), s);
                const int64_t T = 4ll * F, wl = T * hop;
                h->d_wave.alloc((size_t)wl);
                const int* dc[3] = {h->d_codes[0].p, h->d_codes[1].p, h->d_codes[2].p};
                B2A_CUDA(cudaStreamSynchronize(s));
                const int32_t st = b2a_snac_decode_dev(h->snac, dc, 1, T, nullptr, 0, gp->seed + (uint64_t)b, h->d_wave.p, s);
                B2A_CHECK(st == B2A_OK, B2A_ERR_AUDIO_DECODING_FAILED, std::string("SNAC decode failed: ") + b2a_last_error());
                const int64_t skip = (int64_t)(emitted[b] - f0) * 4 * hop, n_new = wl - skip;
                s_wave.resize((size_t)n_new);
                B2A_CUDA(cudaMemcpyAsync(s_wave.data(), h->d_wave.p + skip, (size_t)n_new * sizeof(float), cudaMemcpyDeviceToHost, s));
                B2A_CUDA(cudaStreamSynchronize(s));
                emitted[b] = f1;
                ss.on_audio(user, b, s_wave.data(), n_new, (final_call && f1 == total) ? 1 : 0);
            }
        }
        codec_stream_t += now_s() - c0;
    };
    auto stream_tokens = [&]() {
        h_tok.resize((size_t)B * MT);
        std::vector<int> ng(B);
        B2A_CUDA(cudaMemcpy(ng.data(), h->n_gen.p, B * sizeof(int), cudaMemcpyDeviceToHost));
        B2A_CUDA(cudaMemcpy(h_tok.data(), h->out_tokens.p, (size_t)B * MT * sizeof(int), cudaMemcpyDeviceToHost));
        for (int b = 0; b < B; ++b)
            if (ng[b] > streamed) on_token(user, b, streamed, h_tok[(size_t)b * MT + streamed]);
        ++streamed;
    };
    if (steps == 1) {
        if (on_token) stream_tokens();
        B2A_CUDA(cudaMemcpyAsync(h->h_flag.p, h->n_active.p, sizeof(int), cudaMemcpyDeviceToHost, s));
        B2A_CUDA(cudaStreamSynchronize(s));
    }
    const bool pipelined = !on_token && !streaming;
// ... 101 lines not shown
        info->codec_time = codec_t + codec_stream_t;
        size_t fr = 0, tot = 0;
        cudaMemGetInfo(&fr, &tot);
        info->peak_memory_gb = (double)(tot - fr) / 1e9;
    }
}

extern "C" {

int32_t b2a_tts_generate_stream(b2a_tts* h, const int32_t* input_ids, int32_t B, int32_t L, const b2a_gen_params* gp,
                                int32_t frames_per_chunk, int32_t left_context_frames, int32_t* tokens_out, int32_t* n_tokens_out,
                                b2a_gen_info* info, b2a_token_cb on_token, b2a_audio_cb on_audio, void* user) {
    return guarded([&] {
        B2A_CHECK(on_audio && frames_per_chunk >= 1 && left_context_frames >= 0, B2A_ERR_INVALID_INPUT,
                  "b2a_tts_generate_stream: needs on_audio, frames_per_chunk >= 1, left_context_frames >= 0");
        StreamSpec ss;
        ss.frames_per_chunk = frames_per_chunk; ss.left_context = left_context_frames; ss.on_audio = on_audio;
        tts_generate_impl(h, input_ids, false, B, L, gp, tokens_out, n_tokens_out, nullptr, false, 0, nullptr, info, on_token, user, ss);
    });
}

int32_t b2a_tts_create(int32_t device, const b2a_llama_config* cfg, const b2a_tensor* tensors, int32_t n, b2a_snac* snac,
                       b2a_tts** out) {
    return guarded([&] {
        B2A_CHECK(out, B2A_ERR_INVALID_INPUT, "b2a_tts_create: null out");
        *out = nullptr;
        B2A_CHECK(cfg && tensors && n > 0, B2A_ERR_MODEL_NOT_INITIALIZED, "b2a_tts_create: missing config or weights");
        TensorTable tt(tensors, n);
        *out = new b2a_tts(device, *cfg, tt, snac);
    });
}

int32_t b2a_tts_create_random(int32_t device, const b2a_llama_config* cfg, float std, uint64_t seed, b2a_snac* snac,
                              b2a_tts** out) {
    return guarded([&] {
        B2A_CHECK(out, B2A_ERR_INVALID_INPUT, "b2a_tts_create_random: null out");
        *out = nullptr;
        B2A_CHECK(cfg && std > 0.f, B2A_ERR_MODEL_NOT_INITIALIZED, "b2a_tts_create_random: missing config");
        *out = new b2a_tts(device, *cfg, std, seed, snac);
    });
}

void* b2a_tts_stream(b2a_tts* h) { return h ? (void*)h->stream : nullptr; }

int32_t b2a_tts_time_steps(b2a_tts* h, int32_t B, int32_t ctx, int32_t iters, float* ms_per_step) {
    return guarded([&] {
        B2A_CHECK(h && ms_per_step && iters > 0, B2A_ERR_INVALID_INPUT, "b2a_tts_time_steps: bad argument");
        B2A_CHECK(B >= 1 && B <= h->cfg.max_batch && ctx >= 0 && ctx + iters < h->cfg.max_context, B2A_ERR_INVALID_INPUT,
                  "b2a_tts_time_steps: batch / context out of range");
        B2A_CUDA(cudaSetDevice(h->device));
        cudaStream_t s = h->stream;
        h->set_batch(B);
        const int MT = iters + 8;
        h->ids.alloc((size_t)B * 1);
        h->out_tokens.alloc((size_t)B * MT);
        h->recent.alloc(8);
        SampleArgs sa{};
        sa.logits = h->logits.p; sa.probs = h->probs.p; sa.tokens = h->tokens.p; sa.pos = h->pos.p; sa.recent = h->recent.p;
        sa.recent_n = h->recent_n.p; sa.out_tokens = h->out_tokens.p; sa.n_gen = h->n_gen.p; sa.done = h->done.p;
        sa.n_active = h->n_active.p; sa.forced = nullptr; sa.V = h->cfg.vocab_size; sa.R = 1; sa.max_tokens = MT;
        sa.temperature = 0.f; sa.top_p = 1.f; sa.rep_penalty = 1.f; sa.seed = 0; sa.mask_eos = 1;
        h->capture(B, sa, 1);
        B2A_CUDA(cudaMemsetAsync(h->ids.p, 0, (size_t)B * sizeof(int), s));
        init_rows_kernel<<<1, 32, 0, s>>>(h->ids.p, 1, B, 0, h->tokens.p, h->pos.p, h->recent.p, h->recent_n.p, h->n_gen.p,
                                          h->done.p, h->n_active.p, ctx);
        count_launch();
        cudaEvent_t e0, e1;
        B2A_CUDA(cudaEventCreate(&e0));
        B2A_CUDA(cudaEventCreate(&e1));
        B2A_CUDA(cudaGraphLaunch(h->g_step, s));
        B2A_CUDA(cudaEventRecord(e0, s));
        for (int i = 0; i < iters - 1; ++i) B2A_CUDA(cudaGraphLaunch(h->g_step, s));
        B2A_CUDA(cudaEventRecord(e1, s));
        B2A_CUDA(cudaStreamSynchronize(s));
        count_launch(h->launches_step * iters);
        float ms = 0.f;
        B2A_CUDA(cudaEventElapsedTime(&ms, e0, e1));
        cudaEventDestroy(e0);
        cudaEventDestroy(e1);
        *ms_per_step = ms / (float)std::max(1, iters - 1);
    });
}

int32_t b2a_tts_prepare_input_ids(const int32_t* const* prompt_ids, const int32_t* lens, int32_t batch, int32_t* out,
                                  int32_t* out_len) {
    return guarded([&] {
        B2A_CHECK(prompt_ids && lens && out_len && batch > 0, B2A_ERR_INVALID_INPUT, "b2a_tts_prepare_input_ids: null argument");
        int mx = 0;
        for (int b = 0; b < batch; ++b) mx = std::max(mx, lens[b]);
        *out_len = mx + 3;
        if (!out) return;
        for (int b = 0; b < batch; ++b) {
            int32_t* r = out + (size_t)b * (mx + 3);
            int j = 0;
            for (; j < mx - lens[b]; ++j) r[j] = TOK_PAD;
            r[j++] = TOK_START_OF_HUMAN;
            for (int i = 0; i < lens[b]; ++i) r[j++] = prompt_ids[b][i];
            r[j++] = TOK_END_OF_TEXT;
            r[j++] = TOK_END_OF_HUMAN;
        }
    });
}

int32_t b2a_tts_prepare_input_ids_ref(const int32_t* const* prompt_ids, const int32_t* lens, int32_t batch, const int32_t* ref_text_ids,
                                      int32_t ref_text_len, const int32_t* ref_code_list, int32_t ref_code_len, int32_t* out,
                                      int32_t* out_len) {
    return guarded([&] {
        B2A_CHECK(prompt_ids && lens && out_len && batch > 0 && ref_text_len >= 0 && ref_code_len >= 0 && (ref_text_ids || ref_text_len == 0) &&
                      (ref_code_list || ref_code_len == 0),
                  B2A_ERR_INVALID_INPUT, "b2a_tts_prepare_input_ids_ref: null argument");
        B2A_CHECK(ref_code_len % 7 == 0, B2A_ERR_INVALID_INPUT, "b2a_tts_prepare_input_ids_ref: ref_code_len must be a multiple of 7");
        for (int i = 0; i < ref_code_len; ++i)
            B2A_CHECK(ref_code_list[i] >= 0 && ref_code_list[i] < 7 * 4096, B2A_ERR_INVALID_INPUT,
                      "b2a_tts_prepare_input_ids_ref: reference code out of range [0, 7 * 4096)");
        int mx = 0;
        for (int b = 0; b < batch; ++b) {
            B2A_CHECK(lens[b] >= 0 && (prompt_ids[b] || lens[b] == 0), B2A_ERR_INVALID_INPUT, "b2a_tts_prepare_input_ids_ref: bad prompt");
            mx = std::max(mx, lens[b]);
        }
        const int ref = 1 + ref_text_len + 2 + 2 + ref_code_len + 2;
        *out_len = mx + ref + 3;
        if (!out) return;
        for (int b = 0; b < batch; ++b) {
            int32_t* r = out + (size_t)b * (mx + ref + 3);
            int j = 0;
            for (; j < mx - lens[b]; ++j) r[j] = TOK_PAD;
            r[j++] = TOK_START_OF_HUMAN;
            for (int i = 0; i < ref_text_len; ++i) r[j++] = ref_text_ids[i];
            r[j++] = TOK_END_OF_TEXT;
            r[j++] = TOK_END_OF_HUMAN;
            r[j++] = TOK_AUDIO_START;
            r[j++] = TOK_START_OF_SPEECH;
            for (int i = 0; i < ref_code_len; ++i) r[j++] = ref_code_list[i] + TOK_AUDIO_OFFSET;
            r[j++] = TOK_END_OF_SPEECH;
            r[j++] = TOK_AUDIO_END;
            r[j++] = TOK_START_OF_HUMAN;
            for (int i = 0; i < lens[b]; ++i) r[j++] = prompt_ids[b][i];
            r[j++] = TOK_END_OF_TEXT;
            r[j++] = TOK_END_OF_HUMAN;
        }
    });
}

int32_t b2a_debug_step_smem(int32_t gqa, int32_t* out) {
    return guarded([&] {
        B2A_CHECK(out && (gqa == 1 || gqa == 2 || gqa == 3 || gqa == 4 || gqa == 6 || gqa == 8), B2A_ERR_INVALID_INPUT,
                  "b2a_debug_step_smem: q heads per kv head must be 1, 2, 3, 4, 6 or 8");
        out[0] = (int32_t)tc::Smem<16>::bytes(b2a_tts::gemm_stages);
        out[1] = (int32_t)tc::SmemSplit::bytes(b2a_tts::splitk_stages, b2a_tts::fused_cluster);
        out[2] = (int32_t)attn_smem_bytes(gqa);
    });
}

int32_t b2a_tts_debug_trace(b2a_tts* h, int32_t enable, int32_t batch, float* out) {
    return guarded([&] {
        B2A_CHECK(h, B2A_ERR_INVALID_INPUT, "b2a_tts_debug_trace: null handle");
        B2A_CUDA(cudaSetDevice(h->device));
        const int H = h->cfg.hidden_size, n = 2 * h->cfg.num_hidden_layers + 1;
        if (out) {
            B2A_CHECK(h->trace.p && batch >= 1 && batch <= 8, B2A_ERR_INVALID_INPUT, "b2a_tts_debug_trace: nothing traced");
            B2A_CUDA(cudaStreamSynchronize(h->stream));
            for (int i = 0; i < n; ++i)
                B2A_CUDA(cudaMemcpy(out + (size_t)i * batch * H, h->trace.p + (size_t)i * 8 * H, (size_t)batch * H * sizeof(float),
                                    cudaMemcpyDeviceToHost));
        }
        h->trace_on = enable != 0;
        if (h->trace_on) { h->trace.alloc((size_t)n * 8 * H); h->drop_graphs(); }
    });
}

int32_t b2a_tts_forward_logits(b2a_tts* h, const int32_t* ids, int32_t B, int32_t L, int32_t reset_cache, float* logits_out) {
    return guarded([&] {
        B2A_CHECK(h && ids && logits_out, B2A_ERR_INVALID_INPUT, "b2a_tts_forward_logits: null argument");
        B2A_CHECK(B >= 1 && B <= h->cfg.max_batch && L >= 1, B2A_ERR_INVALID_INPUT, "b2a_tts_forward_logits: bad batch / length");
        B2A_CUDA(cudaSetDevice(h->device));
        cudaStream_t s = h->stream;
        h->set_batch(B);
        h->drop_graphs();
        std::vector<int> hp(8, 0);
        if (!reset_cache) B2A_CUDA(cudaMemcpy(hp.data(), h->pos.p, 8 * sizeof(int), cudaMemcpyDeviceToHost));
        const int start = reset_cache ? 0 : hp[0];
        B2A_CHECK(start + L <= h->cfg.max_context, B2A_ERR_INVALID_INPUT, "b2a_tts_forward_logits: context overflow");
        h->ids.alloc((size_t)B * L);
        B2A_CUDA(cudaMemcpyAsync(h->ids.p, ids, (size_t)B * L * sizeof(int), cudaMemcpyHostToDevice, s));
        const int V = h->cfg.vocab_size;
        std::vector<int> tk(8, 0), ps(8, -1);
        for (int p = 0; p < L; ++p) {
            for (int b = 0; b < B; ++b) { tk[b] = ids[(size_t)b * L + p]; ps[b] = start + p; }
            B2A_CUDA(cudaMemcpyAsync(h->tokens.p, tk.data(), 8 * sizeof(int), cudaMemcpyHostToDevice, s));
            B2A_CUDA(cudaMemcpyAsync(h->pos.p, ps.data(), 8 * sizeof(int), cudaMemcpyHostToDevice, s));
            h->run_layers(B, s);
            h->run_lm_head(B, s);
            for (int b = 0; b < B; ++b)
                B2A_CUDA(cudaMemcpyAsync(logits_out + ((size_t)b * L + p) * V, h->logits.p + (size_t)b * V, V * sizeof(float),
                                         cudaMemcpyDeviceToHost, s));
            B2A_CUDA(cudaStreamSynchronize(s));
        }
        for (int b = 0; b < B; ++b) ps[b] = start + L;
        B2A_CUDA(cudaMemcpy(h->pos.p, ps.data(), 8 * sizeof(int), cudaMemcpyHostToDevice));
        B2A_CUDA(cudaGetLastError());
    });
}

int32_t b2a_tts_generate(b2a_tts* h, const int32_t* input_ids, int32_t B, int32_t L, const b2a_gen_params* gp,
                         int32_t* tokens_out, int32_t* n_tokens_out, float* wave_out, int64_t wave_cap, int64_t* wave_len,
                         b2a_gen_info* info, b2a_token_cb on_token, void* user) {
    return guarded([&] {
        tts_generate_impl(h, input_ids, false, B, L, gp, tokens_out, n_tokens_out, wave_out, false, wave_cap, wave_len, info,
                          on_token, user);
    });
}

int32_t b2a_tts_generate_dev(b2a_tts* h, const int32_t* d_input_ids, int32_t B, int32_t L, const b2a_gen_params* gp,
                             float* d_wave_out, int64_t wave_cap, int64_t* wave_len, b2a_gen_info* info) {
    return guarded([&] {
        tts_generate_impl(h, d_input_ids, true, B, L, gp, nullptr, nullptr, d_wave_out, true, wave_cap, wave_len, info, nullptr,
                          nullptr);
    });
}

int32_t b2a_tts_set_bench_flags(b2a_tts* h, int32_t mask_eos, int32_t wrap_codes) {
    if (!h) return B2A_ERR_INVALID_INPUT;
    h->bench_mask_eos = mask_eos != 0;
    h->bench_wrap_codes = wrap_codes != 0;
    return B2A_OK;
}

int32_t b2a_tts_cancel(b2a_tts* h) {
    if (!h) return B2A_ERR_INVALID_INPUT;
    h->cancel.store(1);
    return B2A_OK;
}

int32_t b2a_tts_parse_output(const int32_t* tokens, int32_t batch, int32_t n, int32_t* code_lists_out, int32_t* code_lens) {
    return guarded([&] {
        B2A_CHECK(tokens && code_lists_out && code_lens && batch > 0 && n >= 0, B2A_ERR_INVALID_INPUT, "b2a_tts_parse_output: bad argument");
        int last = -1;
        for (int i = 0; i < batch; ++i)
            for (int j = 0; j < n; ++j)
                if (tokens[(size_t)i * n + j] == TOK_START_OF_SPEECH) last = j;
        for (int i = 0; i < batch; ++i) {
            std::vector<int> r = parse_row(tokens + (size_t)i * n, n, last);
            code_lens[i] = (int)r.size();
            memcpy(code_lists_out + (size_t)i * n, r.data(), r.size() * sizeof(int));
        }
    });
}

int32_t b2a_tts_deinterleave(const int32_t* code_list, int32_t n, int32_t* c0, int32_t* c1, int32_t* c2, int32_t* n_frames) {
    return guarded([&] {
        B2A_CHECK(code_list && c0 && c1 && c2 && n_frames && n >= 0, B2A_ERR_INVALID_INPUT, "b2a_tts_deinterleave: bad argument");
        const int groups = (n + 1) / 7;
        B2A_CHECK(groups * 7 <= n, B2A_ERR_INVALID_INPUT, "b2a_tts_deinterleave: code list must hold whole 7-token frames");
        std::vector<int> l1, l2, l3;
        deinterleave(code_list, n, l1, l2, l3);
        memcpy(c0, l1.data(), l1.size() * sizeof(int));
        memcpy(c1, l2.data(), l2.size() * sizeof(int));
        memcpy(c2, l3.data(), l3.size() * sizeof(int));
        *n_frames = groups;
    });
}

int32_t b2a_tts_interleave(const int32_t* c0, const int32_t* c1, const int32_t* c2, int32_t n_frames, int32_t* cl) {
    return guarded([&] {
        B2A_CHECK(c0 && c1 && c2 && cl && n_frames >= 0, B2A_ERR_INVALID_INPUT, "b2a_tts_interleave: bad argument");
        for (int i = 0; i < n_frames; ++i) {
            int32_t* o = cl + 7 * i;
            o[0] = c0[i];
            o[1] = c1[2 * i] + 4096;
            o[2] = c2[4 * i] + 2 * 4096;
            o[3] = c2[4 * i + 1] + 3 * 4096;
            o[4] = c1[2 * i + 1] + 4 * 4096;
            o[5] = c2[4 * i + 2] + 5 * 4096;
            o[6] = c2[4 * i + 3] + 6 * 4096;
        }
    });
}

void b2a_tts_destroy(b2a_tts* h) { delete h; }

}

namespace b2a {

__global__ void q3_gather_kernel(const bf16* __restrict__ table, int rows, const int* __restrict__ ids, int id_stride, int id_col,
                                 float* __restrict__ dst, int H, int* pos, int pos_value) {
    const int b = blockIdx.x;
    if (!pos) pdl_trigger();
    pdl_wait();
    int t = ids[b * id_stride + id_col];
    t = min(max(t, 0), rows - 1);
    for (int i = threadIdx.x; i < H; i += blockDim.x) dst[(long long)b * H + i] = __bfloat162float(table[(long long)t * H + i]);
    if (pos && threadIdx.x == 0) pos[b] = pos_value;
}
__global__ void q3_copy_rows_kernel(const float* __restrict__ src, long long src_stride, float* __restrict__ dst, int H, int* pos, int pos_value) {
    const int b = blockIdx.x;
    if (!(pos && pos_value >= 0)) pdl_trigger();
    pdl_wait();
    for (int i = threadIdx.x; i < H; i += blockDim.x) dst[(long long)b * H + i] = src[(long long)b * src_stride + i];
    if (pos && pos_value >= 0 && threadIdx.x == 0) pos[b] = pos_value;
}
__global__ void q3_linear_kernel(const bf16* __restrict__ W, const float* __restrict__ bias, const float* __restrict__ x, float* __restrict__ y,
                                 int O, int K, int silu) {
    const int o = blockIdx.x * (blockDim.x >> 5) + (threadIdx.x >> 5), t = blockIdx.y, lane = threadIdx.x & 31;
    if (o >= O) return;
    float acc = 0.f;
// ... 428 lines not shown
```

### mlx-audio-swift_b200/csrc/tc_gemm.cu

```cuda
#define B2A_TC_GEMM_IMPL
#include "common.cuh"
#include "tc_gemm.cuh"

namespace b2a {
namespace tc {

typedef CUresult (*EncodeTiledFn)(CUtensorMap*, CUtensorMapDataType, cuuint32_t, void*, const cuuint64_t*, const cuuint64_t*,
                                  const cuuint32_t*, const cuuint32_t*, CUtensorMapInterleave, CUtensorMapSwizzle,
                                  CUtensorMapL2promotion, CUtensorMapFloatOOBfill);

static EncodeTiledFn encode_fn() {
    static EncodeTiledFn fn = nullptr;
    if (!fn) {
        void* p = nullptr;
        cudaDriverEntryPointQueryResult q;
        B2A_CUDA(cudaGetDriverEntryPoint("cuTensorMapEncodeTiled", &p, cudaEnableDefault, &q));
        B2A_CHECK(p && q == cudaDriverEntryPointSuccess, B2A_ERR_CUDA, "cuTensorMapEncodeTiled is not available in this driver");
        fn = (EncodeTiledFn)p;
    }
    return fn;
}

static CUtensorMapDataType type16(int f16) { return f16 ? CU_TENSOR_MAP_DATA_TYPE_FLOAT16 : CU_TENSOR_MAP_DATA_TYPE_BFLOAT16; }

CUtensorMap make_tmap_bf16(const void* base, long long rows, long long cols, int box_rows, int f16) {
    B2A_CHECK(cols % 8 == 0 && ((uintptr_t)base & 15) == 0, B2A_ERR_INVALID_INPUT, "TMA: tensor must be 16-byte aligned with cols % 8 == 0");
    CUtensorMap m;
    const cuuint64_t dims[2] = {(cuuint64_t)cols, (cuuint64_t)rows};
    const cuuint64_t strides[1] = {(cuuint64_t)cols * 2};
    const cuuint32_t box[2] = {(cuuint32_t)BK, (cuuint32_t)box_rows};
    const cuuint32_t estr[2] = {1, 1};
    const CUresult r = encode_fn()(&m, type16(f16), 2, const_cast<void*>(base), dims, strides, box, estr,
                                   CU_TENSOR_MAP_INTERLEAVE_NONE, CU_TENSOR_MAP_SWIZZLE_128B, CU_TENSOR_MAP_L2_PROMOTION_L2_256B,
                                   CU_TENSOR_MAP_FLOAT_OOB_FILL_NONE);
    B2A_CHECK(r == CUDA_SUCCESS, B2A_ERR_CUDA, "cuTensorMapEncodeTiled failed (" + std::to_string((int)r) + ")");
    return m;
}

CUtensorMap make_tmap_f16_3d(const void* base, long long d0, long long d1, long long d2, int b0, int b1) {
    B2A_CHECK(b0 * 2 == 128 && d0 % 8 == 0 && ((uintptr_t)base & 15) == 0, B2A_ERR_INVALID_INPUT, "TMA: bad 3-D fp16 tensor");
    CUtensorMap m;
    const cuuint64_t dims[3] = {(cuuint64_t)d0, (cuuint64_t)d1, (cuuint64_t)d2};
    const cuuint64_t strides[2] = {(cuuint64_t)d0 * 2, (cuuint64_t)d0 * (cuuint64_t)d1 * 2};
    const cuuint32_t box[3] = {(cuuint32_t)b0, (cuuint32_t)b1, 1};
    const cuuint32_t estr[3] = {1, 1, 1};
    const CUresult r = encode_fn()(&m, CU_TENSOR_MAP_DATA_TYPE_FLOAT16, 3, const_cast<void*>(base), dims, strides, box, estr,
                                   CU_TENSOR_MAP_INTERLEAVE_NONE, CU_TENSOR_MAP_SWIZZLE_128B, CU_TENSOR_MAP_L2_PROMOTION_L2_256B,
                                   CU_TENSOR_MAP_FLOAT_OOB_FILL_NONE);
    B2A_CHECK(r == CUDA_SUCCESS, B2A_ERR_CUDA, "cuTensorMapEncodeTiled (3-D fp16) failed (" + std::to_string((int)r) + ")");
    return m;
}

CUtensorMap make_tmap_planes(const void* base, int C, long long Ttot, int B, int box_frames, int f16) {
    B2A_CHECK(C % 8 == 0 && ((uintptr_t)base & 15) == 0 && Ttot >= 1 && B >= 1, B2A_ERR_INVALID_INPUT,
              "TMA: activation planes must be 16-byte aligned with channels % 8 == 0");
    CUtensorMap m;
    const cuuint64_t dims[4] = {(cuuint64_t)C, (cuuint64_t)Ttot, (cuuint64_t)B, 2};
    const cuuint64_t strides[3] = {(cuuint64_t)C * 2, (cuuint64_t)Ttot * C * 2, (cuuint64_t)B * Ttot * C * 2};
    const cuuint32_t box[4] = {(cuuint32_t)BK, (cuuint32_t)box_frames, 1, 2};
    const cuuint32_t estr[4] = {1, 1, 1, 1};
    const CUresult r = encode_fn()(&m, type16(f16), 4, const_cast<void*>(base), dims, strides, box, estr,
                                   CU_TENSOR_MAP_INTERLEAVE_NONE, CU_TENSOR_MAP_SWIZZLE_128B, CU_TENSOR_MAP_L2_PROMOTION_L2_256B,
                                   CU_TENSOR_MAP_FLOAT_OOB_FILL_NONE);
    B2A_CHECK(r == CUDA_SUCCESS, B2A_ERR_CUDA, "cuTensorMapEncodeTiled (rank 4) failed (" + std::to_string((int)r) + ")");
    return m;
}

template <int BN>
void launch(const CUtensorMap& tmA, const CUtensorMap& tmB, const Args& a, int ctas, int n_tiles, cudaStream_t s) {
    B2A_CHECK(a.stages >= 1 && a.stages <= Smem<BN>::max_stages(), B2A_ERR_INVALID_INPUT, "tc_gemm: ring depth does not fit in shared memory");
    B2A_CHECK(a.epi_partial < 0 || (a.part_ws && a.part_cnt && a.part_slots >= stream_k_slots(a.m_tiles, a.k_blocks, ctas)),
              B2A_ERR_INVALID_INPUT, "tc_gemm: stream-K workspace missing or too small");
    launch_pdl(tc_gemm_kernel<BN>, dim3(ctas, n_tiles), dim3(Cfg<BN>::NTHREADS), Smem<BN>::bytes(a.stages), s, tmA, tmB, a);
}
template void launch<16>(const CUtensorMap&, const CUtensorMap&, const Args&, int, int, cudaStream_t);
template void launch<32>(const CUtensorMap&, const CUtensorMap&, const Args&, int, int, cudaStream_t);
template void launch<128>(const CUtensorMap&, const CUtensorMap&, const Args&, int, int, cudaStream_t);

void launch_splitk(const CUtensorMap& tmA, const CUtensorMap& tmB, const SplitArgs& a, int m_tiles, int cluster, cudaStream_t s) {
    B2A_CHECK(SmemSplit::bytes(a.stages, cluster) <= 227 * 1024, B2A_ERR_INVALID_INPUT, "tc_gemm: split-K ring does not fit in shared memory");
    cudaLaunchConfig_t cfg{};
    cfg.gridDim = dim3((unsigned)(m_tiles * cluster)); cfg.blockDim = dim3(THREADS);
    cfg.dynamicSmemBytes = SmemSplit::bytes(a.stages, cluster); cfg.stream = s;
    cudaLaunchAttribute at[2];
    at[0].id = cudaLaunchAttributeProgrammaticStreamSerialization;
    at[0].val.programmaticStreamSerializationAllowed = pdl_enabled() ? 1 : 0;
    at[1].id = cudaLaunchAttributeClusterDimension;
    at[1].val.clusterDim.x = (unsigned)cluster; at[1].val.clusterDim.y = 1; at[1].val.clusterDim.z = 1;
    cfg.attrs = at; cfg.numAttrs = 2;
    B2A_CUDA(cudaLaunchKernelEx(&cfg, tc_gemm_splitk_kernel, tmA, tmB, a));
    count_launch();
}

void set_attributes() {
    B2A_CUDA(cudaFuncSetAttribute(tc_gemm_splitk_kernel, cudaFuncAttributeMaxDynamicSharedMemorySize, 227 * 1024));
    B2A_CUDA(cudaFuncSetAttribute(tc_gemm_kernel<16>, cudaFuncAttributeMaxDynamicSharedMemorySize, 227 * 1024));
    B2A_CUDA(cudaFuncSetAttribute(tc_gemm_splitk_kernel, cudaFuncAttributePreferredSharedMemoryCarveout, cudaSharedmemCarveoutMaxShared));
    B2A_CUDA(cudaFuncSetAttribute(tc_gemm_kernel<16>, cudaFuncAttributePreferredSharedMemoryCarveout, cudaSharedmemCarveoutMaxShared));
    B2A_CUDA(cudaFuncSetAttribute(tc_gemm_kernel<32>, cudaFuncAttributeMaxDynamicSharedMemorySize, 227 * 1024));
    B2A_CUDA(cudaFuncSetAttribute(tc_gemm_kernel<128>, cudaFuncAttributeMaxDynamicSharedMemorySize, 227 * 1024));
}

}
}


extern "C" int32_t b2a_tc_gemm_epilogue_test(const void* W, const void* X, void* out, int32_t M, int32_t N, int32_t K, int32_t bn,
                                             int32_t epi, int32_t split, int32_t hilo, int32_t ctas, const float* bias, int32_t act,
                                             int32_t tile_rows, int32_t lo_rows, const float* rstd_ss, int32_t rstd_parts,
                                             float rstd_eps, int32_t stages, void* stream) {
    using namespace b2a;
    using namespace b2a::tc;
    return guarded([&] {
        B2A_CHECK(W && X && out && (bn == 16 || bn == 32 || bn == 128) && K % BK == 0 && M > 0 && N > 0 && ctas > 0, B2A_ERR_INVALID_INPUT,
                  "b2a_tc_gemm_epilogue_test: bad argument");
        B2A_CHECK(epi == EPI_STORE || epi == EPI_SWIGLU || epi == EPI_STORE_BF16 || epi == EPI_ADD, B2A_ERR_INVALID_INPUT,
                  "b2a_tc_gemm_epilogue_test: unknown epilogue");
        B2A_CHECK(act == ACT_NONE || act == ACT_GELU, B2A_ERR_INVALID_INPUT, "b2a_tc_gemm_epilogue_test: unknown activation");
        B2A_CHECK(!split || epi == EPI_STORE || epi == EPI_ADD, B2A_ERR_INVALID_INPUT,
                  "b2a_tc_gemm_epilogue_test: stream-K partial tiles are summed into fp32 outputs only");
        B2A_CHECK(!split || act == ACT_NONE, B2A_ERR_INVALID_INPUT, "b2a_tc_gemm_epilogue_test: GELU of a partial K range is not the GELU of the sum");
        B2A_CHECK(!split || tile_rows == 0, B2A_ERR_INVALID_INPUT, "b2a_tc_gemm_epilogue_test: tile_rows is a whole-tile option");
        B2A_CHECK(tile_rows == 0 || (tile_rows % 8 == 0 && tile_rows >= 8 && tile_rows <= BM), B2A_ERR_INVALID_INPUT,
                  "b2a_tc_gemm_epilogue_test: tile_rows must be a multiple of 8 in [8, 128]");
        B2A_CHECK(!lo_rows || (hilo && (epi == EPI_SWIGLU || epi == EPI_STORE_BF16)), B2A_ERR_INVALID_INPUT,
                  "b2a_tc_gemm_epilogue_test: hi/lo outputs need hi/lo inputs and a bf16 epilogue");
        B2A_CHECK(epi != EPI_SWIGLU || M % 2 == 0, B2A_ERR_INVALID_INPUT, "b2a_tc_gemm_epilogue_test: SwiGLU needs (gate, up) row pairs");
        B2A_CHECK(!rstd_ss || (bn == 16 && hilo && N <= 8 && rstd_parts >= 1), B2A_ERR_INVALID_INPUT,
                  "b2a_tc_gemm_epilogue_test: the fused RMSNorm scale is a BN = 16 hi/lo option");
        require_device(0);
        set_attributes();
        const int n_tiles = hilo ? cdiv(N, bn / 2) : cdiv(N, bn);
        B2A_CHECK(n_tiles <= 65535, B2A_ERR_INVALID_INPUT, "b2a_tc_gemm_epilogue_test: too many tokens");
        const int x_rows = hilo ? n_tiles * bn : N;
        const int TR = tile_rows > 0 ? tile_rows : BM;
        CUtensorMap ta = make_tmap_bf16(W, M, K, TR), tb = make_tmap_bf16(X, x_rows, K, bn);
        Args a{};
        a.out_f32 = (float*)out; a.out_bf16 = (__nv_bfloat16*)out; a.M = M; a.N = N; a.K = K;
        a.ldo = epi == EPI_SWIGLU ? M / 2 : M;
        a.tile_rows = tile_rows; a.m_tiles = cdiv(M, TR); a.k_blocks = K / BK;
        const int max_st = bn == 16 ? Smem<16>::max_stages() : bn == 32 ? Smem<32>::max_stages() : Smem<128>::max_stages();
        a.stages = stages > 0 ? stages : max_st;
        a.epi_full = epi; a.epi_partial = split ? EPI_PARTIAL : -1; a.hilo = hilo;
        a.bias = bias; a.act = act;
        a.lo_rows = lo_rows ? bn / 2 : 0;
        a.rstd_ss = rstd_ss; a.rstd_parts = rstd_parts; a.rstd_inv_h = 1.0f / (float)K; a.rstd_eps = rstd_eps;
        DBuf<float> ws;
        DBuf<unsigned> cnt;
        if (split) {
            a.part_slots = stream_k_slots(a.m_tiles, a.k_blocks, ctas);
            ws.alloc((size_t)n_tiles * a.m_tiles * a.part_slots * bn * BM);
            cnt.alloc((size_t)n_tiles * a.m_tiles);
            B2A_CUDA(cudaMemset(cnt.p, 0, (size_t)n_tiles * a.m_tiles * sizeof(unsigned)));
            a.part_ws = ws.p; a.part_cnt = cnt.p;
        }
        if (bn == 16) launch<16>(ta, tb, a, ctas, n_tiles, (cudaStream_t)stream);
        else if (bn == 32) launch<32>(ta, tb, a, ctas, n_tiles, (cudaStream_t)stream);
        else launch<128>(ta, tb, a, ctas, n_tiles, (cudaStream_t)stream);
        B2A_CUDA(cudaGetLastError());
        B2A_CUDA(cudaStreamSynchronize((cudaStream_t)stream));
    });
}

extern "C" int32_t b2a_tc_gemm_test(const void* W, const void* X, void* out, int32_t M, int32_t N, int32_t K, int32_t bn,
                                    int32_t epi, int32_t split, int32_t hilo, int32_t ctas, void* stream) {
    const int32_t lo_rows = hilo && (epi == b2a::tc::EPI_SWIGLU || epi == b2a::tc::EPI_STORE_BF16);
    return b2a_tc_gemm_epilogue_test(W, X, out, M, N, K, bn, epi, split, hilo, ctas, nullptr, b2a::tc::ACT_NONE, 0, lo_rows, nullptr, 0,
                                     0.f, 0, stream);
}

extern "C" int32_t b2a_tc_gemm_splitk_test(const void* W, const void* X, float* h, const float* gain, void* xn, float* ss, int32_t M,
                                           int32_t N, int32_t K, int32_t cluster, int32_t stages, void* stream) {
    using namespace b2a;
    using namespace b2a::tc;
    return guarded([&] {
        B2A_CHECK(W && X && h && gain && xn && ss && M > 0 && M % 8 == 0 && K > 0 && K % BK == 0 && N >= 1 && N <= 8 && stages >= 1,
                  B2A_ERR_INVALID_INPUT, "b2a_tc_gemm_splitk_test: bad argument");
        B2A_CHECK(cluster >= 1 && cluster <= SPLIT_MAX_CLUSTER && cluster <= K / BK, B2A_ERR_INVALID_INPUT,
                  "b2a_tc_gemm_splitk_test: cluster must be in [1, min(8, K / 64)]");
        require_device(0);
        set_attributes();
        CUtensorMap ta = make_tmap_bf16(W, M, K, BM), tb = make_tmap_bf16(X, 16, K, 16);
        SplitArgs a{};
        a.M = M; a.N = N; a.K = K; a.k_blocks = K / BK; a.stages = stages;
        a.h = h; a.gain = gain; a.xn = (__nv_bfloat16*)xn; a.ss = ss;
        launch_splitk(ta, tb, a, cdiv(M, BM), cluster, (cudaStream_t)stream);
        B2A_CUDA(cudaGetLastError());
        B2A_CUDA(cudaStreamSynchronize((cudaStream_t)stream));
    });
}
```

### mlx-audio-swift_b200/csrc/tc_gemm.cuh

```cuda
#pragma once
#include <cuda.h>
#include <cuda_bf16.h>
#include <cuda_runtime.h>
#include <stdint.h>

namespace b2a {
namespace tc {

constexpr int BM = 128, BK = 64, UMMA_K = 16;
constexpr int THREADS = 160;
enum : int { EPI_STORE = 0, EPI_PARTIAL = 1, EPI_SWIGLU = 2, EPI_STORE_BF16 = 3, EPI_ADD = 4 };
enum : int { ACT_NONE = 0, ACT_GELU = 1 };

struct Args {
    float* out_f32;
    __nv_bfloat16* out_bf16;
    int M, N, K;
    int ldo;
    int m_tiles, k_blocks;
    int stages;
    int epi_full;
    int epi_partial;
    int hilo;
    const float* bias;
    int act;
    int tile_rows;
    const float* rstd_ss;
    int rstd_parts;
    float rstd_inv_h, rstd_eps;
    int lo_rows;
    float* part_ws;
    unsigned* part_cnt;
    int part_slots;
};

__host__ __device__ __forceinline__ int stream_k_owner(long long u, long long units, int ctas) {
    return (int)(((u + 1) * ctas + units - 1) / units) - 1;
}
inline int stream_k_slots(int m_tiles, int k_blocks, int ctas) {
    const long long units = (long long)m_tiles * k_blocks;
    int n = 1;
    for (int mt = 0; mt < m_tiles; ++mt)
        n = n > stream_k_owner((long long)(mt + 1) * k_blocks - 1, units, ctas) - stream_k_owner((long long)mt * k_blocks, units, ctas) + 1
                ? n : stream_k_owner((long long)(mt + 1) * k_blocks - 1, units, ctas) - stream_k_owner((long long)mt * k_blocks, units, ctas) + 1;
    return n;
}

__device__ __forceinline__ uint32_t smem_u32(const void* p) { return (uint32_t)__cvta_generic_to_shared(p); }

__device__ __forceinline__ void mbar_init(uint64_t* bar, uint32_t count) {
    asm volatile("mbarrier.init.shared::cta.b64 [%0], %1;" ::"r"(smem_u32(bar)), "r"(count));
}
__device__ __forceinline__ void fence_barrier_init() { asm volatile("fence.mbarrier_init.release.cluster;" ::: "memory"); }
__device__ __forceinline__ void mbar_arrive_expect_tx(uint64_t* bar, uint32_t bytes) {
    asm volatile("mbarrier.arrive.expect_tx.shared::cta.b64 _, [%0], %1;" ::"r"(smem_u32(bar)), "r"(bytes) : "memory");
}
__device__ __forceinline__ void mbar_arrive(uint64_t* bar) {
    asm volatile("mbarrier.arrive.shared::cta.b64 _, [%0];" ::"r"(smem_u32(bar)) : "memory");
}
__device__ __forceinline__ bool mbar_try_wait(uint64_t* bar, uint32_t parity) {
    uint32_t ok;
    asm volatile(
        "{\n\t"
        ".reg .pred p;\n\t"
        "mbarrier.try_wait.parity.shared::cta.b64 p, [%1], %2;\n\t"
        "selp.u32 %0, 1, 0, p;\n\t"
        "}\n"
        : "=r"(ok)
        : "r"(smem_u32(bar)), "r"(parity)
        : "memory");
    return ok != 0;
}
__device__ __forceinline__ void mbar_wait(uint64_t* bar, uint32_t parity) {
    for (uint32_t spins = 0; !mbar_try_wait(bar, parity); ++spins)
        if (spins > (1u << 28)) __trap();
}
__device__ __forceinline__ void tma_load_2d(void* dst, const CUtensorMap* map, uint64_t* bar, int c0, int c1) {
    asm volatile(
        "cp.async.bulk.tensor.2d.shared::cluster.global.tile.mbarrier::complete_tx::bytes [%0], [%1, {%3, %4}], [%2];"
        ::"r"(smem_u32(dst)), "l"(map), "r"(smem_u32(bar)), "r"(c0), "r"(c1)
        : "memory");
}
__device__ __forceinline__ void tma_prefetch_desc(const CUtensorMap* map) {
    asm volatile("prefetch.tensormap [%0];" ::"l"(map) : "memory");
}
__device__ __forceinline__ void wg_fence() { asm volatile("wgmma.fence.sync.aligned;" ::: "memory"); }
__device__ __forceinline__ void wg_commit() { asm volatile("wgmma.commit_group.sync.aligned;" ::: "memory"); }
__device__ __forceinline__ void wg_wait0() { asm volatile("wgmma.wait_group.sync.aligned 0;" ::: "memory"); }
template <int R>
__device__ __forceinline__ void wg_fence_operand(float (&d)[R]) {
#pragma unroll
    for (int i = 0; i < R; ++i) asm volatile("" : "+f"(d[i])::"memory");
}
__device__ __forceinline__ void wgmma_bf16_n16(float (&d)[8], uint64_t da, uint64_t db, uint32_t scale_d) {
    asm volatile(
        "{\n\t.reg .pred p;\n\tsetp.ne.b32 p, %10, 0;\n\t"
        "wgmma.mma_async.sync.aligned.m64n16k16.f32.bf16.bf16 {%0,%1,%2,%3,%4,%5,%6,%7}, %8, %9, p, 1, 1, 0, 0;\n\t}\n"
        : "+f"(d[0]), "+f"(d[1]), "+f"(d[2]), "+f"(d[3]), "+f"(d[4]), "+f"(d[5]), "+f"(d[6]), "+f"(d[7])
        : "l"(da), "l"(db), "r"(scale_d));
}
__device__ __forceinline__ void wgmma_bf16_n32(float (&d)[16], uint64_t da, uint64_t db, uint32_t scale_d) {
    asm volatile(
        "{\n\t.reg .pred p;\n\tsetp.ne.b32 p, %18, 0;\n\t"
        "wgmma.mma_async.sync.aligned.m64n32k16.f32.bf16.bf16 {%0,%1,%2,%3,%4,%5,%6,%7,%8,%9,%10,%11,%12,%13,%14,%15}, %16, %17, p, 1, 1, 0, 0;\n\t}\n"
        : "+f"(d[0]), "+f"(d[1]), "+f"(d[2]), "+f"(d[3]), "+f"(d[4]), "+f"(d[5]), "+f"(d[6]), "+f"(d[7]), "+f"(d[8]), "+f"(d[9]), "+f"(d[10]), "+f"(d[11]), "+f"(d[12]), "+f"(d[13]), "+f"(d[14]), "+f"(d[15])
        : "l"(da), "l"(db), "r"(scale_d));
}
__device__ __forceinline__ void wgmma_bf16_n64(float (&d)[32], uint64_t da, uint64_t db, uint32_t scale_d) {
    asm volatile(
        "{\n\t.reg .pred p;\n\tsetp.ne.b32 p, %34, 0;\n\t"
        "wgmma.mma_async.sync.aligned.m64n64k16.f32.bf16.bf16 {%0,%1,%2,%3,%4,%5,%6,%7,%8,%9,%10,%11,%12,%13,%14,%15,%16,%17,%18,%19,%20,%21,%22,%23,%24,%25,%26,%27,%28,%29,%30,%31}, %32, %33, p, 1, 1, 0, 0;\n\t}\n"
        : "+f"(d[0]), "+f"(d[1]), "+f"(d[2]), "+f"(d[3]), "+f"(d[4]), "+f"(d[5]), "+f"(d[6]), "+f"(d[7]), "+f"(d[8]), "+f"(d[9]), "+f"(d[10]), "+f"(d[11]), "+f"(d[12]), "+f"(d[13]), "+f"(d[14]), "+f"(d[15]), "+f"(d[16]), "+f"(d[17]), "+f"(d[18]), "+f"(d[19]), "+f"(d[20]), "+f"(d[21]), "+f"(d[22]), "+f"(d[23]), "+f"(d[24]), "+f"(d[25]), "+f"(d[26]), "+f"(d[27]), "+f"(d[28]), "+f"(d[29]), "+f"(d[30]), "+f"(d[31])
        : "l"(da), "l"(db), "r"(scale_d));
}
__device__ __forceinline__ void wgmma_bf16_n128(float (&d)[64], uint64_t da, uint64_t db, uint32_t scale_d) {
    asm volatile(
        "{\n\t.reg .pred p;\n\tsetp.ne.b32 p, %66, 0;\n\t"
        "wgmma.mma_async.sync.aligned.m64n128k16.f32.bf16.bf16 {%0,%1,%2,%3,%4,%5,%6,%7,%8,%9,%10,%11,%12,%13,%14,%15,%16,%17,%18,%19,%20,%21,%22,%23,%24,%25,%26,%27,%28,%29,%30,%31,%32,%33,%34,%35,%36,%37,%38,%39,%40,%41,%42,%43,%44,%45,%46,%47,%48,%49,%50,%51,%52,%53,%54,%55,%56,%57,%58,%59,%60,%61,%62,%63}, %64, %65, p, 1, 1, 0, 0;\n\t}\n"
        : "+f"(d[0]), "+f"(d[1]), "+f"(d[2]), "+f"(d[3]), "+f"(d[4]), "+f"(d[5]), "+f"(d[6]), "+f"(d[7]), "+f"(d[8]), "+f"(d[9]), "+f"(d[10]), "+f"(d[11]), "+f"(d[12]), "+f"(d[13]), "+f"(d[14]), "+f"(d[15]), "+f"(d[16]), "+f"(d[17]), "+f"(d[18]), "+f"(d[19]), "+f"(d[20]), "+f"(d[21]), "+f"(d[22]), "+f"(d[23]), "+f"(d[24]), "+f"(d[25]), "+f"(d[26]), "+f"(d[27]), "+f"(d[28]), "+f"(d[29]), "+f"(d[30]), "+f"(d[31]), "+f"(d[32]), "+f"(d[33]), "+f"(d[34]), "+f"(d[35]), "+f"(d[36]), "+f"(d[37]), "+f"(d[38]), "+f"(d[39]), "+f"(d[40]), "+f"(d[41]), "+f"(d[42]), "+f"(d[43]), "+f"(d[44]), "+f"(d[45]), "+f"(d[46]), "+f"(d[47]), "+f"(d[48]), "+f"(d[49]), "+f"(d[50]), "+f"(d[51]), "+f"(d[52]), "+f"(d[53]), "+f"(d[54]), "+f"(d[55]), "+f"(d[56]), "+f"(d[57]), "+f"(d[58]), "+f"(d[59]), "+f"(d[60]), "+f"(d[61]), "+f"(d[62]), "+f"(d[63])
        : "l"(da), "l"(db), "r"(scale_d));
}
__device__ __forceinline__ void wgmma_f16_n64(float (&d)[32], uint64_t da, uint64_t db, uint32_t scale_d) {
    asm volatile(
        "{\n\t.reg .pred p;\n\tsetp.ne.b32 p, %34, 0;\n\t"
        "wgmma.mma_async.sync.aligned.m64n64k16.f32.f16.f16 {%0,%1,%2,%3,%4,%5,%6,%7,%8,%9,%10,%11,%12,%13,%14,%15,%16,%17,%18,%19,%20,%21,%22,%23,%24,%25,%26,%27,%28,%29,%30,%31}, %32, %33, p, 1, 1, 0, 0;\n\t}\n"
        : "+f"(d[0]), "+f"(d[1]), "+f"(d[2]), "+f"(d[3]), "+f"(d[4]), "+f"(d[5]), "+f"(d[6]), "+f"(d[7]), "+f"(d[8]), "+f"(d[9]), "+f"(d[10]), "+f"(d[11]), "+f"(d[12]), "+f"(d[13]), "+f"(d[14]), "+f"(d[15]), "+f"(d[16]), "+f"(d[17]), "+f"(d[18]), "+f"(d[19]), "+f"(d[20]), "+f"(d[21]), "+f"(d[22]), "+f"(d[23]), "+f"(d[24]), "+f"(d[25]), "+f"(d[26]), "+f"(d[27]), "+f"(d[28]), "+f"(d[29]), "+f"(d[30]), "+f"(d[31])
        : "l"(da), "l"(db), "r"(scale_d));
}
__device__ __forceinline__ void wgmma_f16_n128(float (&d)[64], uint64_t da, uint64_t db, uint32_t scale_d) {
    asm volatile(
        "{\n\t.reg .pred p;\n\tsetp.ne.b32 p, %66, 0;\n\t"
        "wgmma.mma_async.sync.aligned.m64n128k16.f32.f16.f16 {%0,%1,%2,%3,%4,%5,%6,%7,%8,%9,%10,%11,%12,%13,%14,%15,%16,%17,%18,%19,%20,%21,%22,%23,%24,%25,%26,%27,%28,%29,%30,%31,%32,%33,%34,%35,%36,%37,%38,%39,%40,%41,%42,%43,%44,%45,%46,%47,%48,%49,%50,%51,%52,%53,%54,%55,%56,%57,%58,%59,%60,%61,%62,%63}, %64, %65, p, 1, 1, 0, 0;\n\t}\n"
        : "+f"(d[0]), "+f"(d[1]), "+f"(d[2]), "+f"(d[3]), "+f"(d[4]), "+f"(d[5]), "+f"(d[6]), "+f"(d[7]), "+f"(d[8]), "+f"(d[9]), "+f"(d[10]), "+f"(d[11]), "+f"(d[12]), "+f"(d[13]), "+f"(d[14]), "+f"(d[15]), "+f"(d[16]), "+f"(d[17]), "+f"(d[18]), "+f"(d[19]), "+f"(d[20]), "+f"(d[21]), "+f"(d[22]), "+f"(d[23]), "+f"(d[24]), "+f"(d[25]), "+f"(d[26]), "+f"(d[27]), "+f"(d[28]), "+f"(d[29]), "+f"(d[30]), "+f"(d[31]), "+f"(d[32]), "+f"(d[33]), "+f"(d[34]), "+f"(d[35]), "+f"(d[36]), "+f"(d[37]), "+f"(d[38]), "+f"(d[39]), "+f"(d[40]), "+f"(d[41]), "+f"(d[42]), "+f"(d[43]), "+f"(d[44]), "+f"(d[45]), "+f"(d[46]), "+f"(d[47]), "+f"(d[48]), "+f"(d[49]), "+f"(d[50]), "+f"(d[51]), "+f"(d[52]), "+f"(d[53]), "+f"(d[54]), "+f"(d[55]), "+f"(d[56]), "+f"(d[57]), "+f"(d[58]), "+f"(d[59]), "+f"(d[60]), "+f"(d[61]), "+f"(d[62]), "+f"(d[63])
        : "l"(da), "l"(db), "r"(scale_d));
}
__device__ __forceinline__ void wgmma_f16_rs_n64(float (&d)[32], const uint32_t (&a)[4], uint64_t db, uint32_t scale_d) {
    asm volatile(
        "{\n\t.reg .pred p;\n\tsetp.ne.b32 p, %37, 0;\n\t"
        "wgmma.mma_async.sync.aligned.m64n64k16.f32.f16.f16 {%0,%1,%2,%3,%4,%5,%6,%7,%8,%9,%10,%11,%12,%13,%14,%15,%16,%17,%18,%19,%20,%21,%22,%23,%24,%25,%26,%27,%28,%29,%30,%31}, {%32,%33,%34,%35}, %36, p, 1, 1, 0;\n\t}\n"
        : "+f"(d[0]), "+f"(d[1]), "+f"(d[2]), "+f"(d[3]), "+f"(d[4]), "+f"(d[5]), "+f"(d[6]), "+f"(d[7]), "+f"(d[8]), "+f"(d[9]), "+f"(d[10]), "+f"(d[11]), "+f"(d[12]), "+f"(d[13]), "+f"(d[14]), "+f"(d[15]), "+f"(d[16]), "+f"(d[17]), "+f"(d[18]), "+f"(d[19]), "+f"(d[20]), "+f"(d[21]), "+f"(d[22]), "+f"(d[23]), "+f"(d[24]), "+f"(d[25]), "+f"(d[26]), "+f"(d[27]), "+f"(d[28]), "+f"(d[29]), "+f"(d[30]), "+f"(d[31])
        : "r"(a[0]), "r"(a[1]), "r"(a[2]), "r"(a[3]), "l"(db), "r"(scale_d));
}

template <int N>
__device__ __forceinline__ void wgmma_bf16(float (&d)[N / 2], uint64_t da, uint64_t db, uint32_t scale_d) {
    if constexpr (N == 16) wgmma_bf16_n16(d, da, db, scale_d);
    else if constexpr (N == 32) wgmma_bf16_n32(d, da, db, scale_d);
    else if constexpr (N == 64) wgmma_bf16_n64(d, da, db, scale_d);
    else wgmma_bf16_n128(d, da, db, scale_d);
}

__device__ __forceinline__ uint64_t make_smem_desc(uint32_t saddr) {
    return (uint64_t)((saddr & 0x3FFFF) >> 4) | ((uint64_t)1 << 16) | ((uint64_t)(1024 >> 4) << 32) | ((uint64_t)1 << 62);
}

template <int N>
__device__ __forceinline__ void store_frag(float* s, int ld, const float (&d)[N / 2], int r0, int c0) {
    const int t = threadIdx.x & 127, r = r0 + (t >> 5) * 16 + ((t & 31) >> 2), c = c0 + 2 * (t & 3);
#pragma unroll
    for (int i = 0; i < N / 8; ++i) {
        *reinterpret_cast<float2*>(s + (size_t)r * ld + c + 8 * i) = make_float2(d[4 * i], d[4 * i + 1]);
        *reinterpret_cast<float2*>(s + (size_t)(r + 8) * ld + c + 8 * i) = make_float2(d[4 * i + 2], d[4 * i + 3]);
    }
}
__device__ __forceinline__ void ld_acc16(const float* p, float* v) {
#pragma unroll
    for (int i = 0; i < 4; ++i) {
        const float4 f = reinterpret_cast<const float4*>(p)[i];
        v[4 * i] = f.x; v[4 * i + 1] = f.y; v[4 * i + 2] = f.z; v[4 * i + 3] = f.w;
    }
}
__device__ __forceinline__ void named_sync(int id, int threads) { asm volatile("bar.sync %0, %1;" ::"r"(id), "r"(threads) : "memory"); }

template <class I>
__device__ __forceinline__ void store_hilo(__nv_bfloat16* base, long long ld, I t, long long col, float v, int half) {
    const __nv_bfloat16 hi = __float2bfloat16_rn(v);
    const long long r = (long long)(t / half) * 2 * half + (t % half);
    base[r * ld + col] = hi;
    base[(r + half) * ld + col] = __float2bfloat16_rn(v - __bfloat162float(hi));
}

template <int BN>
struct Cfg {
    static constexpr int EPI_WARPS = BN >= 128 ? 16 : 4;
    static constexpr int WG = EPI_WARPS / 4;
    static constexpr int RB = WG == 1 ? 2 : 1;
    static constexpr int WN = WG == 1 ? BN : BN * 2 / WG;
    static constexpr int LD = BN + 4;
    static constexpr int NTHREADS = 32 * EPI_WARPS + 32;
};

template <int BN>
struct Smem {
    static constexpr int A_BYTES = BM * BK * 2, B_BYTES = BN * BK * 2, STAGE = A_BYTES + B_BYTES;
    static constexpr int ACC_BYTES = BM * Cfg<BN>::LD * 4;
    static int max_stages() { return (226 * 1024 - 256 - ACC_BYTES) / STAGE; }
    static size_t bytes(int stages) { return (size_t)stages * STAGE + ACC_BYTES + 256; }
};
__device__ __forceinline__ void check_smem_base(const void* base) {
    if (threadIdx.x == 0 && (smem_u32(base) & 1023u)) __trap();
}

template <int BN>
__global__ void __launch_bounds__(Cfg<BN>::NTHREADS, Cfg<BN>::EPI_WARPS > 4 ? 1 : 2)
tc_gemm_kernel(const __grid_constant__ CUtensorMap tmA, const __grid_constant__ CUtensorMap tmB, const __grid_constant__ Args a) {
    using S = Smem<BN>;
    using C = Cfg<BN>;
    extern __shared__ __align__(1024) uint8_t smem[];
    float* sacc = reinterpret_cast<float*>(smem + (size_t)a.stages * S::STAGE);
    uint64_t* full = reinterpret_cast<uint64_t*>(smem + (size_t)a.stages * S::STAGE + S::ACC_BYTES);
    uint64_t* empty = full + a.stages;
    int* s_reduce = reinterpret_cast<int*>(empty + a.stages);

    const int warp = threadIdx.x >> 5, lane = threadIdx.x & 31;
    const int n0 = blockIdx.y * BN;
    const int TR = a.tile_rows > 0 ? a.tile_rows : BM;
    const uint32_t stage_tx = (uint32_t)(TR * BK * 2 + S::B_BYTES);
    asm volatile("griddepcontrol.launch_dependents;" ::: "memory");

    check_smem_base(smem);
    if (threadIdx.x == 0) {
        tma_prefetch_desc(&tmA);
        tma_prefetch_desc(&tmB);
        for (int i = 0; i < a.stages; ++i) { mbar_init(&full[i], 1); mbar_init(&empty[i], C::EPI_WARPS); }
        fence_barrier_init();
    }
    __syncthreads();

    const long long units = (long long)a.m_tiles * a.k_blocks;
    long long u0, u1;
    if (a.epi_partial >= 0) {
        u0 = units * blockIdx.x / gridDim.x;
        u1 = units * (blockIdx.x + 1) / gridDim.x;
    } else {
        u0 = ((long long)a.m_tiles * blockIdx.x / gridDim.x) * a.k_blocks;
        u1 = ((long long)a.m_tiles * (blockIdx.x + 1) / gridDim.x) * a.k_blocks;
    }

    if (warp == C::EPI_WARPS) {
        if (lane == 0) {
            const int npre = (int)min((long long)a.stages, u1 - u0);
            for (int i = 0; i < npre; ++i) {
                const long long u = u0 + i;
                const int mt = (int)(u / a.k_blocks), kb = (int)(u - (long long)mt * a.k_blocks);
                mbar_arrive_expect_tx(&full[i], stage_tx);
                tma_load_2d(smem + (size_t)i * S::STAGE, &tmA, &full[i], kb * BK, mt * TR);
            }
            asm volatile("griddepcontrol.wait;" ::: "memory");
            for (int i = 0; i < npre; ++i) {
                const long long u = u0 + i;
                const int mt = (int)(u / a.k_blocks), kb = (int)(u - (long long)mt * a.k_blocks);
                tma_load_2d(smem + (size_t)i * S::STAGE + S::A_BYTES, &tmB, &full[i], kb * BK, n0);
            }
            int stage = npre == a.stages ? 0 : npre;
            uint32_t phase = npre == a.stages ? 1 : 0;
            for (long long u = u0 + npre; u < u1; ++u) {
                const int mt = (int)(u / a.k_blocks), kb = (int)(u - (long long)mt * a.k_blocks);
                mbar_wait(&empty[stage], phase ^ 1);
                uint8_t* sa = smem + (size_t)stage * S::STAGE;
                mbar_arrive_expect_tx(&full[stage], stage_tx);
                tma_load_2d(sa, &tmA, &full[stage], kb * BK, mt * TR);
                tma_load_2d(sa + S::A_BYTES, &tmB, &full[stage], kb * BK, n0);
                if (++stage == a.stages) { stage = 0; phase ^= 1; }
            }
        }
    } else {
        const int q = warp & 3;
        constexpr int NCG = C::EPI_WARPS / 4;
        const int cg = warp >> 2, wg = warp >> 2;
        const int row_blk = C::WG == 1 ? 0 : (wg & 1), col_blk = C::WG == 1 ? 0 : (wg >> 1);
        int stage = 0; uint32_t phase = 0;
        float acc[C::RB][C::WN / 2];
#pragma unroll
        for (int rb = 0; rb < C::RB; ++rb)
#pragma unroll
            for (int i = 0; i < C::WN / 2; ++i) acc[rb][i] = 0.f;
        long long u = u0;
        float rstd[8];
        bool have_rstd = false;
        if (BN == 16 && a.rstd_ss) {
            asm volatile("griddepcontrol.wait;" ::: "memory");
            float t = 0.f;
            for (int p0 = 0; p0 < a.rstd_parts; p0 += 4) {
                const int p = p0 + (lane >> 3);
                if (p < a.rstd_parts) t += a.rstd_ss[p * 8 + (lane & 7)];
            }
            t += __shfl_xor_sync(0xffffffffu, t, 8);
            t += __shfl_xor_sync(0xffffffffu, t, 16);
            const float rs = rsqrtf(t * a.rstd_inv_h + a.rstd_eps);
#pragma unroll
            for (int j = 0; j < 8; ++j) rstd[j] = __shfl_sync(0xffffffffu, rs, j);
            have_rstd = true;
        }
        while (u < u1) {
            const int mt = (int)(u / a.k_blocks);
            const long long seg_begin = u;
            const long long seg_end = min(u1, (long long)(mt + 1) * a.k_blocks);
            u = seg_end;
            const bool whole = (seg_begin == (long long)mt * a.k_blocks) && (seg_end == (long long)(mt + 1) * a.k_blocks);
            const int epi = whole ? a.epi_full : a.epi_partial;
            for (long long uu = seg_begin; uu < seg_end; ++uu) {
                mbar_wait(&full[stage], phase);
                const uint32_t sa = smem_u32(smem + (size_t)stage * S::STAGE);
                wg_fence();
#pragma unroll
                for (int k = 0; k < BK / UMMA_K; ++k) {
#pragma unroll
                    for (int rb = 0; rb < C::RB; ++rb) {
                        const uint64_t ad = make_smem_desc(sa + (uint32_t)((row_blk + rb) * 64 * 128)) + (uint64_t)(2 * k);
                        const uint64_t bd = make_smem_desc(sa + S::A_BYTES + (uint32_t)(col_blk * C::WN * 128)) + (uint64_t)(2 * k);
                        wgmma_bf16<C::WN>(acc[rb], ad, bd, (uu == seg_begin && k == 0) ? 0u : 1u);
                    }
                }
                wg_commit();
                wg_wait0();
                __syncwarp();
                if (lane == 0) mbar_arrive(&empty[stage]);
                if (++stage == a.stages) { stage = 0; phase ^= 1; }
            }
#pragma unroll
            for (int rb = 0; rb < C::RB; ++rb) wg_fence_operand(acc[rb]);
            named_sync(1, 32 * C::EPI_WARPS);
#pragma unroll
            for (int rb = 0; rb < C::RB; ++rb) store_frag<C::WN>(sacc, C::LD, acc[rb], (row_blk + rb) * 64, col_blk * C::WN);
            named_sync(1, 32 * C::EPI_WARPS);
            const int m = mt * TR + q * 32 + lane;
            const float* arow = sacc + (size_t)(q * 32 + lane) * C::LD;
            const long long units = (long long)a.m_tiles * a.k_blocks;
            const int first_owner = stream_k_owner((long long)mt * a.k_blocks, units, gridDim.x);
            const size_t tile_id = (size_t)blockIdx.y * a.m_tiles + mt;
            float* ws_tile = whole ? nullptr : a.part_ws + (tile_id * a.part_slots + (blockIdx.x - first_owner)) * BN * BM;
            constexpr int HALF = BN / 2;
            constexpr int CH = (BN == 16) ? 8 : 16;
            const int n_cols = a.hilo ? HALF : BN;
            const int ntok0 = a.hilo ? (int)blockIdx.y * HALF : n0;
            const bool m_ok = m < a.M && q * 32 + lane < TR;
            const int cstep = (BN == 16 && !a.hilo) ? 16 : CH;
            for (int c0 = cg * cstep; c0 < n_cols; c0 += cstep * NCG) {
                float v[16];
                if (BN == 16) {
                    ld_acc16(arow, v);
                    if (a.hilo) {
#pragma unroll
                        for (int j = 0; j < 8; ++j) v[j] += v[j + 8];
                    }
                    if (have_rstd) {
#pragma unroll
                        for (int j = 0; j < 8; ++j) v[j] *= rstd[j];
                    }
                } else {
                    ld_acc16(arow + c0, v);
                    if (a.hilo) {
                        float w[16];
                        ld_acc16(arow + c0 + HALF, w);
#pragma unroll
                        for (int j = 0; j < 16; ++j) v[j] += w[j];
                    }
                }
                const int jn = (BN == 16 && !a.hilo) ? 16 : CH;
                if (a.bias || a.act) {
                    const float bv = (a.bias && m_ok && (whole || seg_begin == (long long)mt * a.k_blocks)) ? a.bias[m] : 0.f;
#pragma unroll
                    for (int j = 0; j < 16; ++j) {
                        float t = v[j] + bv;
                        if (a.act == ACT_GELU) t = 0.5f * t * (1.0f + erff(t * 0.70710678118654752f));
                        v[j] = t;
                    }
                }
                const int nt = ntok0 + c0;
                const int nvalid = min(jn, a.N - nt);
                if (epi == EPI_SWIGLU) {
                    const long long hrow = a.lo_rows ? (long long)(nt / HALF) * BN + (nt % HALF) : nt;
                    __nv_bfloat16* ph = a.out_bf16 + hrow * a.ldo + (m >> 1);
                    const long long lo_off = (long long)HALF * a.ldo;
#pragma unroll
                    for (int j = 0; j < 16; ++j) {
                        if (j >= jn) break;
                        const float other = __shfl_xor_sync(0xffffffffu, v[j], 1);
                        if (j < nvalid && m_ok && (lane & 1) == 0) {
                            const float r = v[j] / (1.0f + __expf(-v[j])) * other;
                            const __nv_bfloat16 hi = __float2bfloat16_rn(r);
                            ph[0] = hi;
                            if (a.lo_rows) ph[lo_off] = __float2bfloat16_rn(r - __bfloat162float(hi));
                        }
                        ph += a.ldo;
                    }
                } else if (epi == EPI_STORE_BF16) {
                    const long long hrow = a.lo_rows ? (long long)(nt / HALF) * BN + (nt % HALF) : nt;
                    __nv_bfloat16* ph = a.out_bf16 + hrow * a.ldo + m;
                    const long long lo_off = (long long)HALF * a.ldo;
#pragma unroll
                    for (int j = 0; j < 16; ++j) {
                        if (j >= jn) break;
                        if (j < nvalid && m_ok) {
                            const __nv_bfloat16 hi = __float2bfloat16_rn(v[j]);
                            ph[0] = hi;
                            if (a.lo_rows) ph[lo_off] = __float2bfloat16_rn(v[j] - __bfloat162float(hi));
                        }
                        ph += a.ldo;
                    }
                } else if (epi == EPI_PARTIAL) {
                    float* pw = ws_tile + (size_t)(nt - ntok0) * BM + q * 32 + lane;
#pragma unroll
                    for (int j = 0; j < 16; ++j)
                        if (j < jn) pw[(size_t)j * BM] = v[j];
                } else {
                    float* pf = a.out_f32 + (long long)nt * a.ldo + m;
                    if (epi == EPI_ADD) {
#pragma unroll
                        for (int j = 0; j < 16; ++j)
                            if (j < jn && j < nvalid && m_ok) v[j] += pf[(long long)j * a.ldo];
                    }
#pragma unroll
                    for (int j = 0; j < 16; ++j) {
                        if (j >= jn) break;
                        if (j < nvalid && m_ok) {
                            pf[0] = v[j];
                        }
                        pf += a.ldo;
                    }
                }
            }
            if (!whole) {
                const int n_parts = stream_k_owner((long long)(mt + 1) * a.k_blocks - 1, units, gridDim.x) - first_owner + 1;
                const unsigned my_kb = (unsigned)(seg_end - seg_begin);
                __threadfence();
                named_sync(1, 32 * C::EPI_WARPS);
                if (threadIdx.x == 0) *s_reduce = atomicAdd(&a.part_cnt[tile_id], my_kb) + my_kb == (unsigned)a.k_blocks;
                named_sync(1, 32 * C::EPI_WARPS);
                if (*s_reduce) {
                    __threadfence();
                    const float* base = a.part_ws + tile_id * a.part_slots * BN * BM;
                    constexpr int NT = 32 * C::EPI_WARPS, PER = 16;
                    const int n_el = n_cols * BM;
                    for (int i0 = 0; i0 < n_el; i0 += NT * PER) {
                        float sum[PER];
#pragma unroll
                        for (int e = 0; e < PER; ++e) sum[e] = 0.f;
                        for (int p = 0; p < n_parts; ++p) {
                            const long long c = first_owner + p;
                            if (units * (c + 1) / gridDim.x == units * c / gridDim.x) continue;
                            const float* slot = base + (size_t)p * BN * BM;
#pragma unroll
                            for (int e = 0; e < PER; ++e) {
                                const int i = i0 + threadIdx.x + e * NT;
                                if (i < n_el) sum[e] += __ldcg(slot + i);
                            }
                        }
#pragma unroll
                        for (int e = 0; e < PER; ++e) {
                            const int i = i0 + threadIdx.x + e * NT;
                            const int tcol = i / BM, r = i - tcol * BM, mm = mt * BM + r, tok = ntok0 + tcol;
                            if (i < n_el && tok < a.N && mm < a.M) a.out_f32[(long long)tok * a.ldo + mm] += sum[e];
                        }
                    }
                    if (threadIdx.x == 0) a.part_cnt[tile_id] = 0;
                }
            }
        }
    }
}

struct SplitArgs {
    int M, N, K;
    int k_blocks, stages;
    float* h;
    const float* gain;
    __nv_bfloat16* xn;
    float* ss;
    const float* rstd_ss;
    int rstd_parts;
    float rstd_inv_h, rstd_eps;
};

__device__ __forceinline__ uint32_t cluster_ctarank() { uint32_t r; asm volatile("mov.u32 %0, %%cluster_ctarank;" : "=r"(r)); return r; }
__device__ __forceinline__ uint32_t cluster_nctarank() { uint32_t r; asm volatile("mov.u32 %0, %%cluster_nctarank;" : "=r"(r)); return r; }
__device__ __forceinline__ void cluster_sync_all() {
    asm volatile("barrier.cluster.arrive.release.aligned;" ::: "memory");
    asm volatile("barrier.cluster.wait.acquire.aligned;" ::: "memory");
}
__device__ __forceinline__ uint32_t map_to_rank(uint32_t saddr, uint32_t rank) {
    uint32_t r;
    asm volatile("mapa.shared::cluster.u32 %0, %1, %2;" : "=r"(r) : "r"(saddr), "r"(rank));
    return r;
}
__device__ __forceinline__ void st_cluster_f4(uint32_t addr, float a, float b, float c, float d) {
    asm volatile("st.shared::cluster.v4.f32 [%0], {%1, %2, %3, %4};" ::"r"(addr), "f"(a), "f"(b), "f"(c), "f"(d) : "memory");
}

constexpr int SPLIT_MAX_CLUSTER = 8;
struct SmemSplit {
    static constexpr int STAGE = Smem<16>::STAGE;
    static constexpr int PART_BYTES = BM * 8 * 4;
    static_assert(Smem<16>::ACC_BYTES <= STAGE, "the staged accumulator lives in ring stage 0");
    static size_t bytes(int stages, int cluster) { return (size_t)stages * STAGE + (size_t)(cluster - 1) * PART_BYTES + 512; }
};

#ifdef B2A_TC_GEMM_IMPL
__global__ void __launch_bounds__(THREADS, 2)
tc_gemm_splitk_kernel(const __grid_constant__ CUtensorMap tmA, const __grid_constant__ CUtensorMap tmB, SplitArgs a) {
    using S = Smem<16>;
    constexpr int BN = 16;
    extern __shared__ __align__(1024) uint8_t smem[];
    const uint32_t C = cluster_nctarank(), rank = cluster_ctarank();
    float* part = reinterpret_cast<float*>(smem + (size_t)a.stages * S::STAGE);
    float* sacc = reinterpret_cast<float*>(smem);
    uint64_t* full = reinterpret_cast<uint64_t*>(part + (size_t)(C - 1) * BM * 8);
    uint64_t* empty = full + a.stages;
    float* s_red = reinterpret_cast<float*>(empty + a.stages);

    const int warp = threadIdx.x >> 5, lane = threadIdx.x & 31;
    const int mt = blockIdx.x / C;
    const int kb0 = (int)((long long)a.k_blocks * rank / C), kb1 = (int)((long long)a.k_blocks * (rank + 1) / C);
    asm volatile("griddepcontrol.launch_dependents;" ::: "memory");

    check_smem_base(smem);
    if (threadIdx.x == 0) {
        tma_prefetch_desc(&tmA);
        tma_prefetch_desc(&tmB);
        for (int i = 0; i < a.stages; ++i) { mbar_init(&full[i], 1); mbar_init(&empty[i], 4); }
        fence_barrier_init();
    }
    __syncthreads();

    if (warp == 4) {
        if (lane == 0) {
            const int n = kb1 - kb0, npre = min(a.stages, n);
            for (int i = 0; i < npre; ++i) {
                mbar_arrive_expect_tx(&full[i], S::STAGE);
                tma_load_2d(smem + (size_t)i * S::STAGE, &tmA, &full[i], (kb0 + i) * BK, mt * BM);
            }
            asm volatile("griddepcontrol.wait;" ::: "memory");
            for (int i = 0; i < npre; ++i) tma_load_2d(smem + (size_t)i * S::STAGE + S::A_BYTES, &tmB, &full[i], (kb0 + i) * BK, 0);
            int stage = npre == a.stages ? 0 : npre;
            uint32_t phase = npre == a.stages ? 1 : 0;
            for (int i = npre; i < n; ++i) {
                mbar_wait(&empty[stage], phase ^ 1);
                uint8_t* sa = smem + (size_t)stage * S::STAGE;
                mbar_arrive_expect_tx(&full[stage], S::STAGE);
                tma_load_2d(sa, &tmA, &full[stage], (kb0 + i) * BK, mt * BM);
                tma_load_2d(sa + S::A_BYTES, &tmB, &full[stage], (kb0 + i) * BK, 0);
                if (++stage == a.stages) { stage = 0; phase ^= 1; }
            }
        }
    }
    float acc[8], hold[8];
    float g = 0.f;
    const int q = warp & 3, row = q * 32 + lane;
    const int m = mt * BM + row;
    const bool m_ok = m < a.M;
    if (warp < 4) {
        if (rank == 0) {
            asm volatile("griddepcontrol.wait;" ::: "memory");
            g = m_ok ? a.gain[m] : 0.f;
#pragma unroll
            for (int j = 0; j < 8; ++j) hold[j] = (j < a.N && m_ok) ? a.h[(long long)j * a.M + m] : 0.f;
        }
        float d[2][8];
#pragma unroll
        for (int rb = 0; rb < 2; ++rb)
#pragma unroll
            for (int i = 0; i < 8; ++i) d[rb][i] = 0.f;
        int stage = 0; uint32_t phase = 0;
        for (int kb = kb0; kb < kb1; ++kb) {
            mbar_wait(&full[stage], phase);
            const uint32_t sa = smem_u32(smem + (size_t)stage * S::STAGE);
            wg_fence();
#pragma unroll
            for (int k = 0; k < BK / UMMA_K; ++k) {
#pragma unroll
                for (int rb = 0; rb < 2; ++rb)
                    wgmma_bf16<BN>(d[rb], make_smem_desc(sa + (uint32_t)(rb * 64 * 128)) + (uint64_t)(2 * k),
                                   make_smem_desc(sa + S::A_BYTES) + (uint64_t)(2 * k), (kb == kb0 && k == 0) ? 0u : 1u);
            }
            wg_commit();
            wg_wait0();
            __syncwarp();
            if (lane == 0) mbar_arrive(&empty[stage]);
            if (++stage == a.stages) { stage = 0; phase ^= 1; }
        }
        named_sync(3, 128);
#pragma unroll
        for (int rb = 0; rb < 2; ++rb) {
            wg_fence_operand(d[rb]);
            store_frag<BN>(sacc, Cfg<BN>::LD, d[rb], rb * 64, 0);
        }
        named_sync(3, 128);
        float v[16];
        ld_acc16(sacc + (size_t)row * Cfg<BN>::LD, v);
#pragma unroll
        for (int j = 0; j < 8; ++j) acc[j] = v[j] + v[j + 8];
        if (rank != 0) {
            const uint32_t dst = map_to_rank(smem_u32(part + ((size_t)(rank - 1) * BM + row) * 8), 0);
            st_cluster_f4(dst, acc[0], acc[1], acc[2], acc[3]);
            st_cluster_f4(dst + 16, acc[4], acc[5], acc[6], acc[7]);
        }
    }
    __syncwarp();
    cluster_sync_all();
    if (rank == 0 && warp < 4) {
        for (uint32_t r = 1; r < C; ++r) {
// ... 59 lines not shown
```

Baseline: 29.96.

## Fuse QK-norm, RoPE and KV-cache append into the QKV GEMM epilogue

Moves the per-head q/k RMS norm, rotary embedding and KV-cache writes out of the attention kernel into a new EPI_QKV epilogue of the tensor-core QKV GEMM (and a standalone rope_append kernel on the unfused path). Attention now reads pre-rotated q from a separate buffer and the new k/v straight from the cache, and no longer zeroes the qkv buffer. This takes the serial per-block rope/norm prologue off the attention critical path and drops the qkv round trip through global memory. In exchange the GEMM epilogue gets heavier, with named barriers and sincos work, and the stream-K reduction path also has to apply the transform.

```diff
diff --git a/include/b200audio_internal.h b/include/b200audio_internal.h
--- a/include/b200audio_internal.h
+++ b/include/b200audio_internal.h
@@ -35,6 +35,11 @@
                          int32_t split, int32_t hilo, int32_t ctas, void* stream);
 int32_t b2a_tc_gemm_splitk_test(const void* W, const void* X, float* h, const float* gain, void* xn, float* ss, int32_t M, int32_t N,
                                 int32_t K, int32_t cluster, int32_t stages, void* stream);
+int32_t b2a_tc_gemm_qkv_test(const void* W, const void* X, const float* rstd_ss, int32_t rstd_parts, float rstd_eps, const int32_t* pos,
+                             const float* freqs, const float* qnorm, const float* knorm, float qk_eps, float* q, float* kcache,
+                             float* vcache, int32_t nq, int32_t nkv, int32_t max_ctx, int32_t N, int32_t K, int32_t ctas, void* stream);
+int32_t b2a_rope_append_test(const float* qkv, int32_t N, const int32_t* pos, const float* freqs, const float* qnorm, const float* knorm,
+                             float qk_eps, float* q, float* kcache, float* vcache, int32_t nq, int32_t nkv, int32_t max_ctx, void* stream);
 int32_t b2a_mha_tc_test(const float* qkv, void* out, int32_t B, int32_t T, int32_t nh, void* stream);
 int32_t b2a_conv_gemm_test(const float* w, int32_t M, int32_t K, const void* X, int32_t N, int32_t epi, const float* bias,
                            const float* alpha, const float* gamma, int32_t gelu, float* x, int32_t ldx, void* hl, int32_t ldh,
diff --git a/mlx-audio-swift_b200/_ffi.py b/mlx-audio-swift_b200/_ffi.py
--- a/mlx-audio-swift_b200/_ffi.py
+++ b/mlx-audio-swift_b200/_ffi.py
@@ -208,6 +208,9 @@
     "b2a_tc_gemm_epilogue_test": (C.c_int32, [_P, _P, _P] + [C.c_int32] * 8 + [_P, C.c_int32, C.c_int32, C.c_int32, _P, C.c_int32,
                                                                              C.c_float, C.c_int32, _P]),
     "b2a_tc_gemm_splitk_test": (C.c_int32, [_P, _P, _P, _P, _P, _P] + [C.c_int32] * 5 + [_P]),
+    "b2a_tc_gemm_qkv_test": (C.c_int32, [_P, _P, _P, C.c_int32, C.c_float, _P, _P, _P, _P, C.c_float, _P, _P, _P] + [C.c_int32] * 6
+                             + [_P]),
+    "b2a_rope_append_test": (C.c_int32, [_P, C.c_int32, _P, _P, _P, _P, C.c_float, _P, _P, _P] + [C.c_int32] * 3 + [_P]),
     "b2a_mha_tc_test": (C.c_int32, [_P, _P, C.c_int32, C.c_int32, C.c_int32, _P]),
     "b2a_conv_gemm_test": (C.c_int32, [_P, C.c_int32, C.c_int32, _P, C.c_int32, C.c_int32, _P, _P, _P, C.c_int32, _P, C.c_int32, _P,
                                        C.c_int32] + [C.c_int32] * 6 + [_P, C.c_uint64, C.c_int32, _P]),
diff --git a/mlx-audio-swift_b200/csrc/llama.cu b/mlx-audio-swift_b200/csrc/llama.cu
--- a/mlx-audio-swift_b200/csrc/llama.cu
+++ b/mlx-audio-swift_b200/csrc/llama.cu
@@ -190,25 +190,21 @@
 }
 
 constexpr int HD = 128, AT_THREADS = 256, MAXG = 8, AT_CAP = 64;
+static_assert(HD == tc::BM, "a 128-row tile of the q|k|v GEMM is one head (tc::qkv_rope_append)");
 constexpr int AT_SLOTS = 3;
 constexpr size_t attn_smem_bytes(int G) {
-    return ((size_t)AT_SLOTS * AT_CAP * HD + (size_t)G * HD + 2 * HD + (size_t)G * HD + 2 * MAXG) * sizeof(float) + 64;
+    return ((size_t)AT_SLOTS * AT_CAP * HD + (size_t)G * HD + (size_t)G * HD + 2 * MAXG) * sizeof(float) + 64;
 }
 static_assert((AT_THREADS / 32) * MAXG * HD <= AT_CAP * HD, "the warp-partial outputs must fit in one ring slot");
 
 struct AttnArgs {
-    const float* qkv;
+    const float* q;
     const int* pos;
-    const float* freqs;
     float* kcache;
     float* vcache;
     bf16* out;
     int nq, nkv, max_ctx;
     float scale;
-    const float* qnorm;
-    const float* knorm;
-    float qk_eps;
-    int zero_qkv;
 };
 
 template <int G>
@@ -221,8 +217,7 @@
     float* sKV = reinterpret_cast<float*>(at_smem);
     float* wpo = sKV;
     float* sq = sKV + (size_t)AT_SLOTS * AT_CAP * HD;
-    float* snew = sq + G * HD;
-    float* xo = snew + 2 * HD;
+    float* xo = sq + G * HD;
     float* xml = xo + G * HD;
     uint64_t* bars = reinterpret_cast<uint64_t*>(xml + 2 * MAXG);
     __shared__ float red_m[AT_THREADS / 32][MAXG], red_l[AT_THREADS / 32][MAXG];
@@ -234,10 +229,8 @@
     const int nch = p / AT_CAP + 1;
     const int n_my = nch > rank ? (nch - rank + 1) / 2 : 0;
     const bool owner = ((nch - 1) & 1) == rank;
-    const int qkv_ld = (a.nq + 2 * a.nkv) * HD;
-    const float* row = a.qkv + (long long)b * qkv_ld;
-    float* kc = a.kcache + (((long long)b * a.nkv + h) * a.max_ctx) * HD;
-    float* vc = a.vcache + (((long long)b * a.nkv + h) * a.max_ctx) * HD;
+    const float* kc = a.kcache + (((long long)b * a.nkv + h) * a.max_ctx) * HD;
+    const float* vc = a.vcache + (((long long)b * a.nkv + h) * a.max_ctx) * HD;
     const int n_mat = 2 * n_my;
     auto issue = [&](int j) {
         const int slot = j % AT_SLOTS, c = rank + 2 * (j >> 1);
@@ -258,46 +251,10 @@
         asm volatile("fence.proxy.async.shared::cta;" ::: "memory");
         for (int j = 0; j < min(n_mat, AT_SLOTS); ++j) issue(j);
     }
-    float sn = 0.f, cs = 1.f;
-    if (tid < HD / 2) sincosf((float)p / a.freqs[tid], &sn, &cs);
     pdl_wait();
-    const float* qsrc = row + (long long)h * G * HD;
-    const float* ksrc = row + (a.nq + h) * HD;
-    if (a.qnorm) {
-        for (int vec = tid >> 5; vec < G + 1; vec += AT_THREADS / 32) {
-            const float* src = vec < G ? qsrc + vec * HD : ksrc;
-            const float* w = vec < G ? a.qnorm : a.knorm;
-            const float4 x = reinterpret_cast<const float4*>(src)[tid & 31];
-            const float ss = warp_sum(x.x * x.x + x.y * x.y + x.z * x.z + x.w * x.w);
-            const float r = rsqrtf(ss * (1.0f / HD) + a.qk_eps);
-            const float4 g4 = reinterpret_cast<const float4*>(w)[tid & 31];
-            reinterpret_cast<float4*>(vec < G ? sq + vec * HD : snew)[tid & 31] =
-                make_float4(x.x * r * g4.x, x.y * r * g4.y, x.z * r * g4.z, x.w * r * g4.w);
-        }
-        __syncthreads();
-        qsrc = sq;
-        ksrc = snew;
-    }
-    if (tid < HD / 2) {
-        const int d = tid;
-        _Pragma("unroll") for (int g = 0; g < G; ++g) {
-            const float* q = qsrc + g * HD;
-            const float x1 = q[d], x2 = q[d + HD / 2];
-            sq[g * HD + d] = x1 * cs - x2 * sn;
-            sq[g * HD + d + HD / 2] = x2 * cs + x1 * sn;
-        }
-        const float* k = ksrc;
-        const float x1 = k[d], x2 = k[d + HD / 2];
-        const float k1 = x1 * cs - x2 * sn, k2 = x2 * cs + x1 * sn;
-        if (owner) { kc[(long long)p * HD + d] = k1; kc[(long long)p * HD + d + HD / 2] = k2; }
-        snew[d] = k1;
-        snew[d + HD / 2] = k2;
-    } else if (tid >= 128) {
-        const int d = tid - 128;
-        const float v = row[(a.nq + a.nkv + h) * HD + d];
-        if (owner) vc[(long long)p * HD + d] = v;
-        snew[HD + d] = v;
-    }
+    const float4* qsrc = reinterpret_cast<const float4*>(a.q + ((long long)b * a.nq + h * G) * HD);
+    for (int i = tid; i < G * HD / 4; i += AT_THREADS) reinterpret_cast<float4*>(sq)[i] = __ldcg(qsrc + i);
+    const float kv_new = owner ? __ldcg((tid < HD ? kc : vc) + (long long)p * HD + (tid & (HD - 1))) : 0.f;
     __syncthreads();
 
     const int lane = tid & 31, warp = tid >> 5;
@@ -313,7 +270,7 @@
         const int t0 = c * AT_CAP, nk = min(AT_CAP, p + 1 - t0);
         tc::mbar_wait(&bars[jk % AT_SLOTS], (uint32_t)((jk / AT_SLOTS) & 1));
         if (c == nch - 1) {
-            if (tid < HD) sK[(p - t0) * HD + tid] = snew[tid];
+            if (tid < HD) sK[(p - t0) * HD + tid] = kv_new;
             __syncthreads();
         }
         float sacc[G];
@@ -357,7 +314,7 @@
         }
         tc::mbar_wait(&bars[jv % AT_SLOTS], (uint32_t)((jv / AT_SLOTS) & 1));
         if (c == nch - 1) {
-            if (tid >= HD) sV[(p - t0) * HD + tid - HD] = snew[tid];
+            if (tid >= HD) sV[(p - t0) * HD + tid - HD] = kv_new;
             __syncthreads();
         }
 #pragma unroll
@@ -408,11 +365,6 @@
         }
     }
     cluster.sync();
-    if (a.zero_qkv && rank == 0) {
-        float* wrow = const_cast<float*>(row);
-        for (int i = tid; i < G * HD; i += AT_THREADS) wrow[(long long)h * G * HD + i] = 0.f;
-        if (tid < HD) { wrow[(a.nq + h) * HD + tid] = 0.f; wrow[(a.nq + a.nkv + h) * HD + tid] = 0.f; }
-    }
     if (rank == 0 && tid < HD) {
         _Pragma("unroll") for (int g = 0; g < G; ++g) {
             const float M1 = xml[g], L1 = xml[MAXG + g], O1 = xo[g * HD + tid];
@@ -422,6 +374,23 @@
             tc::store_hilo(a.out, (long long)a.nq * HD, b, (h * G + g) * HD + tid, O / L, LO_ROW);
         }
     }
+}
+
+__global__ void __launch_bounds__(HD) rope_append_kernel(const float* __restrict__ qkv, int N, const __grid_constant__ tc::QkvArgs a) {
+    __shared__ __align__(16) float xch[8 * HD + 8];
+    const int head = blockIdx.x, d = threadIdx.x, ld = (a.nq + 2 * a.nkv) * HD;
+    pdl_trigger();
+    pdl_wait();
+    float v[8];
+    int p[8];
+#pragma unroll
+    for (int j = 0; j < 8; ++j) {
+        v[j] = j < N ? qkv[(long long)j * ld + head * HD + d] : 0.f;
+        p[j] = j < N ? a.pos[j] : -1;
+    }
+    float cs[8], sn[8];
+    tc::rope_cos_sin(p, N, a, cs, sn);
+    tc::qkv_rope_append(v, p, cs, sn, head, N, a, xch);
 }
 
 constexpr int PF_HALF = 64;
@@ -820,7 +789,7 @@
     const bf16* lm_head = nullptr;
     DBuf<float> final_ln, freqs;
     DBuf<float> kcache, vcache;
-    DBuf<float> x, y, qkv, logits, probs;
+    DBuf<float> x, y, qkv, qbuf, logits, probs;
     DBuf<bf16> xn, attn, act;
     DBuf<float> sk_ws;
     DBuf<unsigned> sk_cnt;
@@ -906,6 +875,19 @@
         }
     }
 
+    tc::QkvArgs qkv_args(int l) {
+        const size_t kv_layer = (size_t)cfg.max_batch * cfg.num_key_value_heads * cfg.max_context * HD;
+        LayerW& Lw = layers[l];
+        return tc::QkvArgs{qbuf.p, kcache.p + l * kv_layer, vcache.p + l * kv_layer, pos.p, freqs.p, spec.qk_norm ? Lw.qnorm.p : nullptr,
+                           spec.qk_norm ? Lw.knorm.p : nullptr, cfg.rms_norm_eps, cfg.num_attention_heads, cfg.num_key_value_heads,
+                           cfg.max_context};
+    }
+    AttnArgs attn_args(int l) {
+        const size_t kv_layer = (size_t)cfg.max_batch * cfg.num_key_value_heads * cfg.max_context * HD;
+        return AttnArgs{qbuf.p, pos.p, kcache.p + l * kv_layer, vcache.p + l * kv_layer, attn.p, cfg.num_attention_heads,
+                        cfg.num_key_value_heads, cfg.max_context, 1.0f / sqrtf((float)HD)};
+    }
+
     void check_config() {
         const b2a_llama_config& c = cfg;
         B2A_CHECK(c.head_dim == HD, B2A_ERR_INVALID_INPUT, "llama: head_dim must be 128");
@@ -935,7 +917,7 @@
         B2A_CUDA(cudaMemset(kcache.p, 0, kv * sizeof(float)));
         B2A_CUDA(cudaMemset(vcache.p, 0, kv * sizeof(float)));
         const int B = 8, R16 = 16;
-        x.alloc((size_t)B * H); y.alloc((size_t)B * H); qkv.alloc((size_t)B * (NQ + 2 * NKV));
+        x.alloc((size_t)B * H); y.alloc((size_t)B * H); qkv.alloc((size_t)B * (NQ + 2 * NKV)); qbuf.alloc((size_t)B * NQ);
         logits.alloc((size_t)B * c.vocab_size); probs.alloc((size_t)B * c.vocab_size);
         xn.alloc((size_t)R16 * H); attn.alloc((size_t)R16 * NQ); act.alloc((size_t)R16 * I);
         B2A_CUDA(cudaMemset(xn.p, 0, (size_t)R16 * H * sizeof(bf16)));
@@ -1133,7 +1115,7 @@
     }
 
     void tc_gemm(const CUtensorMap& tmW, const CUtensorMap& tmX, int op, float* yout, bf16* actout, int B, int M, int K,
-                 cudaStream_t s, const float* rstd_ss = nullptr) {
+                 cudaStream_t s, const float* rstd_ss = nullptr, const tc::QkvArgs* qkv = nullptr) {
         tc::Args a{};
         a.rstd_ss = rstd_ss; a.rstd_parts = fused_parts; a.rstd_inv_h = 1.0f / (float)cfg.hidden_size; a.rstd_eps = cfg.rms_norm_eps;
         a.out_f32 = yout; a.out_bf16 = actout; a.M = M; a.N = B; a.K = K;
@@ -1153,6 +1135,7 @@
             a.ldo = M; a.epi_full = tc::EPI_STORE; a.epi_partial = tc::EPI_PARTIAL; a.lo_rows = 0;
             ctas = (int)std::min<long long>(num_sms, (long long)a.m_tiles * a.k_blocks);
             a.part_ws = sk_ws.p; a.part_cnt = sk_cnt.p; a.part_slots = sk_slots;
+            if (qkv) { a.epi_full = tc::EPI_QKV; a.qkv = *qkv; }
         }
         tc::launch<16>(tmW, tmX, a, ctas, 1, s);
     }
@@ -1193,19 +1176,17 @@
         tc::launch_splitk(tmW, tmX, a, cdiv(M, tc::BM), std::max(1, std::min(fused_cluster, a.k_blocks)), s);
     }
     void run_layers_fused(int B, cudaStream_t s) {
-        const int H = cfg.hidden_size, I = cfg.intermediate_size, nq = cfg.num_attention_heads, nkv = cfg.num_key_value_heads;
-        const int NQ = nq * HD, NKV = nkv * HD, L = cfg.num_hidden_layers;
+        const int H = cfg.hidden_size, I = cfg.intermediate_size, NQ = cfg.num_attention_heads * HD, L = cfg.num_hidden_layers;
+        const int NKV = cfg.num_key_value_heads * HD;
         if (x_ext) launch_pdl(ext_embed_kernel, dim3(B), dim3(256), 0, s, x_ext, x.p, y.p, H);
         else launch_pdl(embed_kernel, dim3(B), dim3(256), 0, s, tokens.p, embed.p, x.p, y.p, H, cfg.vocab_size);
         launch_pdl(add_rmsnorm_kernel, dim3(B), dim3(RN_THREADS), 0, s, x.p, (float*)nullptr, layers[0].ln1.p, xn.p, H, cfg.rms_norm_eps,
                    (float*)nullptr, (float*)nullptr, 0, LO_ROW, (float*)nullptr, ss_b.p, fused_parts);
-        const size_t kv_layer = (size_t)cfg.max_batch * nkv * cfg.max_context * HD;
         for (int l = 0; l < L; ++l) {
             LayerW& Lw = layers[l];
-            tc_gemm(tm_qkv[l], tmx_xn, OP_QKV, qkv.p, nullptr, B, NQ + 2 * NKV, H, s, ss_b.p);
-            AttnArgs aa{qkv.p, pos.p, freqs.p, kcache.p + l * kv_layer, vcache.p + l * kv_layer, attn.p, nq, nkv, cfg.max_context,
-                        1.0f / sqrtf((float)HD), spec.qk_norm ? Lw.qnorm.p : nullptr, spec.qk_norm ? Lw.knorm.p : nullptr, cfg.rms_norm_eps, 1};
-            attn_launch(aa, B, s);
+            const tc::QkvArgs qa = qkv_args(l);
+            tc_gemm(tm_qkv[l], tmx_xn, OP_QKV, nullptr, nullptr, B, NQ + 2 * NKV, H, s, ss_b.p, &qa);
+            attn_launch(attn_args(l), B, s);
             splitk_gemm(tm_o[l], tmx_attn, H, NQ, Lw.ln2.p, ss_a.p, B, s);
             tc_gemm(tm_gu_dec[l], tmx_xn, OP_GU, nullptr, act.p, B, 2 * I, H, s, ss_a.p);
             splitk_gemm(tm_down[l], tmx_act, H, I, l + 1 < L ? layers[l + 1].ln1.p : final_ln.p, ss_b.p, B, s);
@@ -1216,26 +1197,23 @@
     void run_layers(int B, cudaStream_t s) {
         if (fused && !trace_on) { run_layers_fused(B, s); return; }
         const int H = cfg.hidden_size, nq = cfg.num_attention_heads, nkv = cfg.num_key_value_heads;
-        const int QKV_N = (nq + 2 * nkv) * HD, G = nq / nkv;
+        const int QKV_N = (nq + 2 * nkv) * HD;
         if (x_ext) launch_pdl(ext_embed_kernel, dim3(B), dim3(256), 0, s, x_ext, x.p, y.p, H);
         else launch_pdl(embed_kernel, dim3(B), dim3(256), 0, s, tokens.p, embed.p, x.p, y.p, H, cfg.vocab_size);
-        const size_t kv_layer = (size_t)cfg.max_batch * nkv * cfg.max_context * HD;
         for (int l = 0; l < cfg.num_hidden_layers; ++l) {
             LayerW& L = layers[l];
             launch_pdl(add_rmsnorm_kernel, dim3(B), dim3(RN_THREADS), 0, s, x.p, l == 0 ? (float*)nullptr : y.p, L.ln1.p, xn.p, H,
                        cfg.rms_norm_eps, trace_on ? trace.p + (size_t)(2 * l) * 8 * H : (float*)nullptr, (float*)nullptr, 0, LO_ROW,
                        (float*)nullptr, (float*)nullptr, 0);
             gemm(OP_QKV, l, B, s);
-            AttnArgs aa{qkv.p, pos.p, freqs.p, kcache.p + l * kv_layer, vcache.p + l * kv_layer, attn.p, nq, nkv, cfg.max_context,
-                        1.0f / sqrtf((float)HD), spec.qk_norm ? L.qnorm.p : nullptr, spec.qk_norm ? L.knorm.p : nullptr, cfg.rms_norm_eps, 0};
-            attn_launch(aa, B, s);
+            launch_pdl(rope_append_kernel, dim3(nq + 2 * nkv), dim3(HD), 0, s, (const float*)qkv.p, B, qkv_args(l));
+            attn_launch(attn_args(l), B, s);
             gemm(OP_O, l, B, s);
             launch_pdl(add_rmsnorm_kernel, dim3(B), dim3(RN_THREADS), 0, s, x.p, y.p, L.ln2.p, xn.p, H, cfg.rms_norm_eps,
                        trace_on ? trace.p + (size_t)(2 * l + 1) * 8 * H : (float*)nullptr, qkv.p, QKV_N, LO_ROW, (float*)nullptr, (float*)nullptr, 0);
             gemm(OP_GU, l, B, s);
             gemm(OP_DOWN, l, B, s);
         }
-        (void)G;
     }
 
     void run_final_norm(int B, cudaStream_t s) {
@@ -1374,8 +1352,8 @@
         B2A_CUDA(cudaGraphInstantiate(&g_prefill, g, 0));
         cudaGraphDestroy(g);
         g_nb = B; g_args = sa; g_L = L;
-        launches_step = fused ? launches_layers_fused() + 1 + 1 : 1 + cfg.num_hidden_layers * 7 + 2 + 1;
-        launches_prefill = fused ? launches_layers_fused() + 1 : 1 + cfg.num_hidden_layers * 7 + 1;
+        launches_step = fused ? launches_layers_fused() + 1 + 1 : 1 + cfg.num_hidden_layers * 8 + 2 + 1;
+        launches_prefill = fused ? launches_layers_fused() + 1 : 1 + cfg.num_hidden_layers * 8 + 1;
     }
     int g_L = 0, launches_step = 0, launches_prefill = 0;
 };
@@ -1783,6 +1761,19 @@
     });
 }
 
+int32_t b2a_rope_append_test(const float* qkv, int32_t N, const int32_t* pos, const float* freqs, const float* qnorm, const float* knorm,
+                             float qk_eps, float* q, float* kcache, float* vcache, int32_t nq, int32_t nkv, int32_t max_ctx, void* stream) {
+    return guarded([&] {
+        B2A_CHECK(qkv && pos && freqs && q && kcache && vcache && N >= 1 && N <= 8 && nq >= 1 && nkv >= 1 && max_ctx >= 1,
+                  B2A_ERR_INVALID_INPUT, "b2a_rope_append_test: bad argument");
+        require_device(0);
+        launch_pdl(rope_append_kernel, dim3(nq + 2 * nkv), dim3(HD), 0, (cudaStream_t)stream, qkv, (int)N,
+                   tc::QkvArgs{q, kcache, vcache, pos, freqs, qnorm, knorm, qk_eps, nq, nkv, max_ctx});
+        B2A_CUDA(cudaGetLastError());
+        B2A_CUDA(cudaStreamSynchronize((cudaStream_t)stream));
+    });
+}
+
 int32_t b2a_tts_debug_trace(b2a_tts* h, int32_t enable, int32_t batch, float* out) {
     return guarded([&] {
         B2A_CHECK(h, B2A_ERR_INVALID_INPUT, "b2a_tts_debug_trace: null handle");
diff --git a/mlx-audio-swift_b200/csrc/tc_gemm.cu b/mlx-audio-swift_b200/csrc/tc_gemm.cu
--- a/mlx-audio-swift_b200/csrc/tc_gemm.cu
+++ b/mlx-audio-swift_b200/csrc/tc_gemm.cu
@@ -71,6 +71,8 @@
     B2A_CHECK(a.stages >= 1 && a.stages <= Smem<BN>::max_stages(), B2A_ERR_INVALID_INPUT, "tc_gemm: ring depth does not fit in shared memory");
     B2A_CHECK(a.epi_partial < 0 || (a.part_ws && a.part_cnt && a.part_slots >= stream_k_slots(a.m_tiles, a.k_blocks, ctas)),
               B2A_ERR_INVALID_INPUT, "tc_gemm: stream-K workspace missing or too small");
+    B2A_CHECK(a.epi_full != EPI_QKV || (BN == 16 && a.hilo && a.tile_rows == 0 && a.N <= 8 && a.M == (a.qkv.nq + 2 * a.qkv.nkv) * BM),
+              B2A_ERR_INVALID_INPUT, "tc_gemm: the q|k|v epilogue needs BN = 16 hi/lo inputs and one 128-row tile per head");
     launch_pdl(tc_gemm_kernel<BN>, dim3(ctas, n_tiles), dim3(Cfg<BN>::NTHREADS), Smem<BN>::bytes(a.stages), s, tmA, tmB, a);
 }
 template void launch<16>(const CUtensorMap&, const CUtensorMap&, const Args&, int, int, cudaStream_t);
@@ -189,3 +191,35 @@
         B2A_CUDA(cudaStreamSynchronize((cudaStream_t)stream));
     });
 }
+
+extern "C" int32_t b2a_tc_gemm_qkv_test(const void* W, const void* X, const float* rstd_ss, int32_t rstd_parts, float rstd_eps,
+                                        const int32_t* pos, const float* freqs, const float* qnorm, const float* knorm, float qk_eps, float* q,
+                                        float* kcache, float* vcache, int32_t nq, int32_t nkv, int32_t max_ctx, int32_t N, int32_t K,
+                                        int32_t ctas, void* stream) {
+    using namespace b2a;
+    using namespace b2a::tc;
+    return guarded([&] {
+        B2A_CHECK(W && X && pos && freqs && q && kcache && vcache && nq >= 1 && nkv >= 1 && max_ctx >= 1 && K > 0 && K % BK == 0 &&
+                      N >= 1 && N <= 8 && ctas >= 1 && (!rstd_ss || rstd_parts >= 1),
+                  B2A_ERR_INVALID_INPUT, "b2a_tc_gemm_qkv_test: bad argument");
+        require_device(0);
+        set_attributes();
+        const int M = (nq + 2 * nkv) * BM;
+        CUtensorMap ta = make_tmap_bf16(W, M, K, BM), tb = make_tmap_bf16(X, 16, K, 16);
+        Args a{};
+        a.M = M; a.N = N; a.K = K; a.ldo = M; a.m_tiles = M / BM; a.k_blocks = K / BK; a.stages = 6;
+        a.epi_full = EPI_QKV; a.epi_partial = EPI_PARTIAL; a.hilo = 1;
+        a.rstd_ss = rstd_ss; a.rstd_parts = rstd_parts; a.rstd_inv_h = 1.0f / (float)K; a.rstd_eps = rstd_eps;
+        a.qkv = QkvArgs{q, kcache, vcache, pos, freqs, qnorm, knorm, qk_eps, nq, nkv, max_ctx};
+        a.part_slots = stream_k_slots(a.m_tiles, a.k_blocks, ctas);
+        DBuf<float> ws;
+        DBuf<unsigned> cnt;
+        ws.alloc((size_t)a.m_tiles * a.part_slots * 16 * BM);
+        cnt.alloc((size_t)a.m_tiles);
+        B2A_CUDA(cudaMemset(cnt.p, 0, (size_t)a.m_tiles * sizeof(unsigned)));
+        a.part_ws = ws.p; a.part_cnt = cnt.p;
+        launch<16>(ta, tb, a, ctas, 1, (cudaStream_t)stream);
+        B2A_CUDA(cudaGetLastError());
+        B2A_CUDA(cudaStreamSynchronize((cudaStream_t)stream));
+    });
+}
diff --git a/mlx-audio-swift_b200/csrc/tc_gemm.cuh b/mlx-audio-swift_b200/csrc/tc_gemm.cuh
--- a/mlx-audio-swift_b200/csrc/tc_gemm.cuh
+++ b/mlx-audio-swift_b200/csrc/tc_gemm.cuh
@@ -9,8 +9,83 @@
 
 constexpr int BM = 128, BK = 64, UMMA_K = 16;
 constexpr int THREADS = 160;
-enum : int { EPI_STORE = 0, EPI_PARTIAL = 1, EPI_SWIGLU = 2, EPI_STORE_BF16 = 3, EPI_ADD = 4 };
+enum : int { EPI_STORE = 0, EPI_PARTIAL = 1, EPI_SWIGLU = 2, EPI_STORE_BF16 = 3, EPI_ADD = 4, EPI_QKV = 5 };
 enum : int { ACT_NONE = 0, ACT_GELU = 1 };
+
+struct QkvArgs {
+    float* q;
+    float* kcache;
+    float* vcache;
+    const int* pos;
+    const float* freqs;
+    const float* qnorm;
+    const float* knorm;
+    float qk_eps;
+    int nq, nkv, max_ctx;
+};
+
+#ifdef __CUDACC__
+__device__ __forceinline__ void named_sync(int id, int threads) { asm volatile("bar.sync %0, %1;" ::"r"(id), "r"(threads) : "memory"); }
+
+__device__ __forceinline__ void rope_cos_sin(const int (&p)[8], int N, const QkvArgs& a, float (&cs)[8], float (&sn)[8]) {
+    const float f = a.freqs[threadIdx.x & (BM / 2 - 1)];
+#pragma unroll
+    for (int j = 0; j < 8; ++j) {
+        cs[j] = 1.f; sn[j] = 0.f;
+        if (j < N) sincosf((float)p[j] / f, &sn[j], &cs[j]);
+    }
+}
+
+__device__ __forceinline__ void qkv_rope_append(float (&v)[8], const int (&p)[8], const float (&cs)[8], const float (&sn)[8], int head,
+                                                int N, const QkvArgs& a, float* xch) {
+    const int d = threadIdx.x & (BM - 1), lane = d & 31, w = d >> 5;
+    float* red = xch + 8 * BM;
+    const bool is_q = head < a.nq, is_k = !is_q && head < a.nq + a.nkv;
+    const float* gn = is_q ? a.qnorm : is_k ? a.knorm : nullptr;
+    named_sync(1, BM);
+    if (gn) {
+#pragma unroll
+        for (int j = 0; j < 8; ++j) xch[j * BM + d] = v[j];
+        named_sync(1, BM);
+        for (int j = w; j < 8; j += 4) {
+            const float4 x = reinterpret_cast<const float4*>(xch + j * BM)[lane];
+            const float ss = warp_sum(x.x * x.x + x.y * x.y + x.z * x.z + x.w * x.w);
+            if (lane == 0) red[j] = rsqrtf(ss * (1.0f / BM) + a.qk_eps);
+        }
+        named_sync(1, BM);
+        const float g = gn[d];
+#pragma unroll
+        for (int j = 0; j < 8; ++j) v[j] = v[j] * red[j] * g;
+        named_sync(1, BM);
+    }
+    if (is_q || is_k) {
+#pragma unroll
+        for (int j = 0; j < 8; ++j) xch[j * BM + d] = v[j];
+        named_sync(1, BM);
+        if (d < BM / 2) {
+#pragma unroll
+            for (int j = 0; j < 8; ++j) {
+                const float x1 = xch[j * BM + d], x2 = xch[j * BM + d + BM / 2];
+                xch[j * BM + d] = x1 * cs[j] - x2 * sn[j];
+                xch[j * BM + d + BM / 2] = x2 * cs[j] + x1 * sn[j];
+            }
+        }
+        named_sync(1, BM);
+#pragma unroll
+        for (int j = 0; j < 8; ++j) v[j] = xch[j * BM + d];
+    }
+#pragma unroll
+    for (int j = 0; j < 8; ++j) {
+        if (j >= N || p[j] < 0 || p[j] >= a.max_ctx) continue;
+        if (is_q) {
+            a.q[((long long)j * a.nq + head) * BM + d] = v[j];
+        } else {
+            const int kh = is_k ? head - a.nq : head - a.nq - a.nkv;
+            (is_k ? a.kcache : a.vcache)[(((long long)j * a.nkv + kh) * a.max_ctx + p[j]) * BM + d] = v[j];
+        }
+    }
+}
+#endif
 
 struct Args {
     float* out_f32;
@@ -32,6 +107,7 @@
     float* part_ws;
     unsigned* part_cnt;
     int part_slots;
+    QkvArgs qkv;
 };
 
 __host__ __device__ __forceinline__ int stream_k_owner(long long u, long long units, int ctas) {
@@ -170,8 +246,6 @@
         v[4 * i] = f.x; v[4 * i + 1] = f.y; v[4 * i + 2] = f.z; v[4 * i + 3] = f.w;
     }
 }
-__device__ __forceinline__ void named_sync(int id, int threads) { asm volatile("bar.sync %0, %1;" ::"r"(id), "r"(threads) : "memory"); }
-
 template <class I>
 __device__ __forceinline__ void store_hilo(__nv_bfloat16* base, long long ld, I t, long long col, float v, int half) {
     const __nv_bfloat16 hi = __float2bfloat16_rn(v);
@@ -291,6 +365,14 @@
 #pragma unroll
             for (int j = 0; j < 8; ++j) rstd[j] = __shfl_sync(0xffffffffu, rs, j);
             have_rstd = true;
+        }
+        int pos[8];
+        float rcs[8], rsn[8];
+        if (BN == 16 && a.epi_full == EPI_QKV) {
+            if (!have_rstd) asm volatile("griddepcontrol.wait;" ::: "memory");
+#pragma unroll
+            for (int j = 0; j < 8; ++j) pos[j] = j < a.N ? a.qkv.pos[j] : -1;
+            rope_cos_sin(pos, a.N, a.qkv, rcs, rsn);
         }
         while (u < u1) {
             const int mt = (int)(u / a.k_blocks);
@@ -369,6 +451,15 @@
                 }
                 const int nt = ntok0 + c0;
                 const int nvalid = min(jn, a.N - nt);
+                if constexpr (BN == 16) {
+                    if (epi == EPI_QKV) {
+                        float h8[8];
+#pragma unroll
+                        for (int j = 0; j < 8; ++j) h8[j] = v[j];
+                        qkv_rope_append(h8, pos, rcs, rsn, mt, a.N, a.qkv, sacc);
+                        continue;
+                    }
+                }
                 if (epi == EPI_SWIGLU) {
                     const long long hrow = a.lo_rows ? (long long)(nt / HALF) * BN + (nt % HALF) : nt;
                     __nv_bfloat16* ph = a.out_bf16 + hrow * a.ldo + (m >> 1);
@@ -447,6 +538,15 @@
                                 if (i < n_el) sum[e] += __ldcg(slot + i);
                             }
                         }
+                        if constexpr (BN == 16) {
+                            if (a.epi_full == EPI_QKV) {
+                                float h8[8];
+#pragma unroll
+                                for (int e = 0; e < 8; ++e) h8[e] = 0.f + sum[e];
+                                qkv_rope_append(h8, pos, rcs, rsn, mt, a.N, a.qkv, sacc);
+                                continue;
+                            }
+                        }
 #pragma unroll
                         for (int e = 0; e < PER; ++e) {
                             const int i = i0 + threadIdx.x + e * NT;
```

Result: no change. 29.74, median of 6 (-0.7%).
